# tavildar/Polar

Hardware: AMD Instinct MI355X
Metric: codewords/s (N=2048 K=1024 L=32 LLR-SCL) (higher is better)
Workload: dtype f64

## Files before the change

### include/polar_amd_debug.h

```cpp
#ifndef POLAR_AMD_DEBUG_H
#define POLAR_AMD_DEBUG_H
#include "polar_amd.h"
#ifdef __cplusplus
extern "C" {
#endif

int polar_debug_set(polar_code_t *h, const char *key, long value);
long polar_debug_get(const polar_code_t *h, const char *key);
long polar_debug_fallback_rows(polar_code_t *h, uint32_t *rows, long cap);
int polar_debug_comm_inits(void);
int polar_debug_weak_leaves(const polar_code_t *h);
void *polar_debug_scratch_ptr(polar_code_t *h);

#ifdef __cplusplus
}
#endif
#endif
```

### polar_amd/__init__.py

```python
import ctypes as C
import os

import numpy as np

try:
    import torch
except Exception:
    torch = None

_HERE = os.path.dirname(os.path.abspath(__file__))
LIB_PATH = os.environ.get("POLAR_AMD_LIB") or os.path.join(_HERE, "libpolar_amd.so")

_dp = C.POINTER(C.c_double)
_u8p = C.POINTER(C.c_uint8)
_u16p = C.POINTER(C.c_uint16)
_u64p = C.POINTER(C.c_uint64)


ASK4_GRAY, ASK8_GRAY, ASK16_GRAY, BPSK = 1, 2, 3, 4
ASK4_SP, ASK8_SP, ASK16_SP = 5, 6, 7
CONSTELLATION_NAMES = {"bpsk": BPSK, "ask4-gray": ASK4_GRAY, "ask8-gray": ASK8_GRAY, "ask16-gray": ASK16_GRAY,
                       "ask4-sp": ASK4_SP, "ask8-sp": ASK8_SP, "ask16-sp": ASK16_SP}
_NBITS = {BPSK: 1, ASK4_GRAY: 2, ASK4_SP: 2, ASK8_GRAY: 3, ASK8_SP: 3, ASK16_GRAY: 4, ASK16_SP: 4}
RX_MLC = 0x100
RECEIVERS = ("bicm", "mlc")


LLR_F64, LLR_F32, LLR_F16, LLR_BF16 = 0, 1, 2, 3
LLR_FORMATS = {"f64": LLR_F64, "f32": LLR_F32, "f16": LLR_F16, "bf16": LLR_BF16}
LS_RUN, LS_ERR, LS_MISS, LS_UNDET, LS_ML, LS_N = 0, 1, 2, 3, 4, 5
AD_RUN, AD_ERR, AD_UNDET, AD_STAGE0 = 0, 1, 2, 3
AD_MAX_STAGES = 8
FL_RUN, FL_ERR, FL_UNDET, FL_FIRST, FL_FLIPPED, FL_DECODES, FL_N = 0, 1, 2, 3, 4, 5, 6
FLIP_MAX = 64


def _llr_fmt_code(fmt):
    if isinstance(fmt, str):
        if fmt not in LLR_FORMATS:
            raise PolarError(f"unknown LLR format {fmt!r} (supported: {sorted(LLR_FORMATS)})")
        return LLR_FORMATS[fmt]
    return int(fmt)


def _llr_rows(llr, fmt):
    if fmt is not None:
        code = _llr_fmt_code(fmt)
        if code >= LLR_F16:
            ok = (np.uint16, np.float16) if code == LLR_F16 else (np.uint16,)
            if not (isinstance(llr, np.ndarray) and llr.dtype in ok):
                raise PolarError("fmt=%r takes the 16-bit patterns as a uint16 array%s" %
                                 (fmt, " (or the values as float16)" if code == LLR_F16 else ""))
            a = np.ascontiguousarray(llr)
        else:
            a = np.ascontiguousarray(llr, np.float32 if code == LLR_F32 else np.float64)
    elif isinstance(llr, np.ndarray) and llr.dtype == np.float32:
        code, a = LLR_F32, np.ascontiguousarray(llr)
    elif isinstance(llr, np.ndarray) and llr.dtype == np.float16:
        code, a = LLR_F16, np.ascontiguousarray(llr)
    else:
        code, a = LLR_F64, np.ascontiguousarray(llr, np.float64)
    return code, a


def _rx_flag(receiver):
    if receiver not in RECEIVERS:
        raise PolarError(f"unknown receiver {receiver!r} (supported: {RECEIVERS})")
    return RX_MLC if receiver == "mlc" else 0


def _constellation_id(c):
    if isinstance(c, str):
        if c not in CONSTELLATION_NAMES:
            raise PolarError(f"unsupported constellation {c!r} (supported: {sorted(CONSTELLATION_NAMES)})")
        return CONSTELLATION_NAMES[c]
    return int(c)


class PolarError(RuntimeError):
    pass


class PolarWeakLeavesWarning(UserWarning):
    """polar_create_explicit returned POLAR_W_WEAK_LEAVES (include/polar_amd.h)."""


POLAR_W_WEAK_LEAVES = 1


_lib = None


def lib():
    global _lib
    if _lib is None:
        if not os.path.exists(LIB_PATH):
            raise PolarError(
                f"{LIB_PATH} not found: build it with `python -m polar_amd.build` "
                "(the HIP extension is mandatory; there is no CPU fallback)")
        L = C.CDLL(LIB_PATH)
        L.polar_last_error.restype = C.c_char_p
        L.polar_snr_sqrt_linear.restype = C.c_double
        L.polar_snr_sqrt_linear.argtypes = [C.c_void_p, C.c_double]
        _lib = L
    return _lib


def use_library(path=None):
    global _lib, LIB_PATH
    LIB_PATH = path or os.environ.get("POLAR_AMD_LIB") or os.path.join(_HERE, "libpolar_amd.so")
    _lib = None
    return lib()


def _check(rc):
    if rc < 0:
        raise PolarError(f"polar_amd error {rc}: {lib().polar_last_error().decode()}")
    return rc


def _p(a, t):
    return a.ctypes.data_as(t)


def _stream_ptr(stream):
    if stream is None:
        if torch is not None and torch.cuda.is_available():
            return C.c_void_p(torch.cuda.current_stream().cuda_stream)
        return C.c_void_p(0)
    if hasattr(stream, "cuda_stream"):
        return C.c_void_p(stream.cuda_stream)
    return C.c_void_p(int(stream))


class Constellation:

    def __init__(self, name):
        self.id = _constellation_id(name)
        if self.id not in _NBITS:
            raise PolarError(f"unknown constellation {name!r} (supported: {sorted(CONSTELLATION_NAMES)})")
        self.name = name if isinstance(name, str) else {v: k for k, v in CONSTELLATION_NAMES.items()}[self.id]
        self.n_bits = _NBITS[self.id]
        self.n_sym = 1 << self.n_bits
        labels = ((np.arange(self.n_sym)[:, None] >> np.arange(self.n_bits)[None, :]) & 1).astype(np.uint8)
        self.points = self.modulate(labels.reshape(-1))

    def modulate(self, bits):
        a = np.ascontiguousarray(bits, np.uint8)
        if a.ndim not in (1, 2) or a.shape[-1] < 1:
            raise PolarError(f"modulate: bits must be [N] or [B][N], got shape {a.shape}")
        single = a.ndim == 1
        a2 = a.reshape(1, -1) if single else a
        out = np.zeros((a2.shape[0], a2.shape[1] // self.n_bits), np.float64)
        _check(lib().polar_modulate(C.c_int(self.id), _p(a2, _u8p), C.c_int(a2.shape[1]), C.c_long(a2.shape[0]), _p(out, _dp)))
        return out[0] if single else out

    def compute_llr_bicm(self, y, n0, block_length=None):
        f32 = isinstance(y, np.ndarray) and y.dtype == np.float32
        a = np.ascontiguousarray(y) if f32 else np.ascontiguousarray(y, np.float64)
        if a.ndim not in (1, 2):
            raise PolarError(f"compute_llr_bicm: y must be [M] or [B][M], got shape {a.shape}")
        single = a.ndim == 1
        a2 = a.reshape(1, -1) if single else a
        B, M = a2.shape
        N = M * self.n_bits if block_length is None else int(block_length)
        if N < 1 or N // self.n_bits != M:
            raise PolarError(f"compute_llr_bicm: rows of {M} symbols do not make rows of {N} positions at {self.n_bits} bits per symbol")
        p1, llr = np.zeros((B, N)), np.zeros((B, N))
        f = lib().polar_demap_bicm_f32 if f32 else lib().polar_demap_bicm
        _check(f(C.c_int(self.id), _p(a2, C.POINTER(C.c_float) if f32 else _dp), C.c_int(N), C.c_long(B), C.c_double(n0),
                 _p(llr, _dp), _p(p1, _dp)))
        return (p1[0], llr[0]) if single else (p1, llr)

    def compute_llr_bicm_dev(self, y_ptr, block_length, B, n0, llr_ptr=0, p1_ptr=0, stream=None, f32=False):
        f = lib().polar_demap_bicm_dev_f32 if f32 else lib().polar_demap_bicm_dev
        _check(f(C.c_int(self.id), C.c_void_p(y_ptr), C.c_int(block_length), C.c_long(B), C.c_double(n0),
                 C.c_void_p(llr_ptr), C.c_void_p(p1_ptr), _stream_ptr(stream)))


class PolarCode:

    def __init__(self, num_layers, info_length, epsilon, crc_size=0, _handle=None):
        L = self._L = lib()
        self._h = C.c_void_p()
        if _handle is not None:
            self._h = _handle
        else:
            self._chk(L.polar_create(C.c_int(num_layers), C.c_int(info_length), C.c_double(epsilon),
                                  C.c_int(crc_size), C.byref(self._h)))
        n, N, K, crc = C.c_int(), C.c_int(), C.c_int(), C.c_int()
        self._chk(L.polar_get_params(self._h, C.byref(n), C.byref(N), C.byref(K), C.byref(crc)))
        self.n, self.block_length, self.info_length, self.crc_size = n.value, N.value, K.value, crc.value
        self.N, self.K = self.block_length, self.info_length

    @property
    def weak_leaves(self):
        return int(self._L.polar_get_weak_leaves(self._h))

    def debug_set(self, key, value):
        self._chk(self._L.polar_debug_set(self._h, key.encode(), C.c_long(int(value))))

    def debug_get(self, key):
        f = self._L.polar_debug_get
        f.restype = C.c_long
        return int(f(self._h, key.encode()))

    def debug_fallback_rows(self):
        f = self._L.polar_debug_fallback_rows
        f.restype = C.c_long
        f.argtypes = [C.c_void_p, C.POINTER(C.c_uint32), C.c_long]
        n = int(f(self._h, None, 0))
        if n == -1:
            return None
        if n < 0:
            raise PolarError(f"polar_debug_fallback_rows: HIP status {-n - 1}")
        rows = np.zeros(max(n, 1), np.uint32)
        if int(f(self._h, _p(rows, C.POINTER(C.c_uint32)), n)) != n:
            raise PolarError("polar_debug_fallback_rows: the count changed between two reads")
        return np.sort(rows[:n])

    @classmethod
    def from_block_length(cls, block_length, info_length, design_epsilon, crc_size=0):
        n = int(round(np.log2(block_length)))
        if (1 << n) != block_length:
            raise PolarError("block_length must be a power of two")
        return cls(n, info_length, design_epsilon, crc_size)

    @classmethod
    def from_tables(cls, num_layers, info_length, crc_size, frozen, order, crc_matrix=None):
        frozen = np.ascontiguousarray(frozen, np.uint8)
        order = np.ascontiguousarray(order, np.uint16)
        N = 1 << num_layers
        if frozen.shape != (N,) or order.shape != (N,):
            raise PolarError("frozen/order must have N entries")
        cm = None
        if crc_size:
            cm = np.ascontiguousarray(crc_matrix, np.uint8)
            if cm.shape != (crc_size, info_length):
                raise PolarError("crc_matrix must be crc x K")
        h = C.c_void_p()
        status = _check(lib().polar_create_explicit(C.c_int(num_layers), C.c_int(info_length), C.c_int(crc_size),
                                                    _p(frozen, _u8p), _p(order, _u16p),
                                                    _p(cm, _u8p) if cm is not None else None, C.byref(h)))
        code = cls(num_layers, info_length, float("nan"), crc_size, _handle=h)
        if status == POLAR_W_WEAK_LEAVES:
            import warnings
            warnings.warn(f"polar_amd: {lib().polar_last_error().decode()}", PolarWeakLeavesWarning, stacklevel=2)
        return code

    @classmethod
    def from_construction_file(cls, path, info_length, crc_size=0, crc_matrix=None):
        return cls.from_counts(np.loadtxt(path).reshape(-1), info_length, crc_size, crc_matrix)

    @classmethod
    def from_counts(cls, counts, info_length, crc_size=0, crc_matrix=None):
        counts = np.asarray(counts).reshape(-1)
        N = counts.size
        n = int(round(np.log2(N)))
        if (1 << n) != N:
            raise PolarError("the count table must hold a power-of-two number of entries")
        order = np.argsort(counts, kind="stable").astype(np.uint16)
        frozen = np.ones(N, np.uint8)
        frozen[order[: info_length + crc_size]] = 0
        return cls.from_tables(n, info_length, crc_size, frozen, order, crc_matrix)

    @classmethod
    def from_monte_carlo(cls, block_length, info_length, design_snr_db, crc_size=0, num_runs=100000,
                         constellation_name="bpsk", receiver_algo="bicm", seed=1, crc_matrix=None, data_dir=None):
        _rx_flag(receiver_algo)
        path = None
        if data_dir is not None:
            path = os.path.join(data_dir, "MC_block_length_" + construction_unique_string(
                block_length, info_length + crc_size, design_snr_db, constellation_name, receiver_algo, num_runs) + ".txt")
        if path is not None and os.path.exists(path):
            counts = np.loadtxt(path).reshape(-1)
        else:
            n = int(round(np.log2(block_length)))
            if (1 << n) != block_length:
                raise PolarError("block_length must be a power of two")
            counts = mc_construction(n, design_snr_db, num_runs, constellation_name, seed=seed, receiver=receiver_algo)
            if path is not None:
                write_construction_file(path, counts)
        if crc_size and crc_matrix is None:
            crc_matrix = np.random.default_rng(seed).integers(0, 2, (crc_size, info_length)).astype(np.uint8)
        code = cls.from_counts(counts, info_length, crc_size, crc_matrix)
        code.construction_counts = np.asarray(counts)
        code.bler_estimate = float(np.sort(np.asarray(counts, np.float64), kind="stable")[: info_length + crc_size].sum() / num_runs)
        return code

    def monte_carlo_code_construction(self, design_snr_db, num_runs=100000, constellation_name="bpsk",
                                      receiver_algo="bicm", seed=1, data_dir=None):
        cm = self.crc_matrix if self.crc_size else None
        new = PolarCode.from_monte_carlo(self.block_length, self.info_length, design_snr_db, self.crc_size, num_runs,
                                         constellation_name, receiver_algo, seed, cm, data_dir)
        self.close()
        self._h, new._h = new._h, None
        self.construction_counts, self.bler_estimate = new.construction_counts, new.bler_estimate
        return self.bler_estimate

    @classmethod
    def from_gauss_approx(cls, block_length, info_length, design_snr_db, constellation_name="bpsk", receiver_algo="bicm",
                          crc_size=0, crc_matrix=None, phi_dx=1e-5, seed=1, capacity=None):
        n = int(round(np.log2(block_length)))
        if (1 << n) != block_length:
            raise PolarError("block_length must be a power of two")
        cap = None if capacity is None else np.asarray(capacity, np.float64).reshape(1, -1)
        ch, order, pre = ga_construction(n, [design_snr_db], constellation_name, receiver_algo, phi_dx, seed, cap)
        k = info_length + crc_size
        if not 0 < k <= block_length:
            raise PolarError("info_length + crc_size must lie in [1, block_length]")
        frozen = np.ones(block_length, np.uint8)
        frozen[order[0, :k]] = 0
        if crc_size and crc_matrix is None:
            crc_matrix = np.random.default_rng(seed).integers(0, 2, (crc_size, info_length)).astype(np.uint8)
        code = cls.from_tables(n, info_length, crc_size, frozen, order[0], crc_matrix)
        code.channels = ch[0]
        code.bler_estimate = float(pre[0, k - 1])
        return code

    def ga_code_construction(self, design_snr_db, constellation_name="bpsk", receiver_algo="bicm", phi_dx=1e-5, seed=1,
                             capacity=None):
        cm = self.crc_matrix if self.crc_size else None
        new = PolarCode.from_gauss_approx(self.block_length, self.info_length, design_snr_db, constellation_name,
                                          receiver_algo, self.crc_size, cm, phi_dx, seed, capacity)
        self.close()
        self._h, new._h = new._h, None
        self.channels, self.bler_estimate = new.channels, new.bler_estimate
        return self.bler_estimate

    def _chk(self, rc):
        if rc < 0:
            raise PolarError(f"polar_amd error {rc}: {self._L.polar_last_error().decode()}")
        return rc

    def close(self):
        if getattr(self, "_h", None):
            self._L.polar_destroy(self._h)
            self._h = None

    def __del__(self):
        try:
            self.close()
        except Exception:
            pass

    @property
    def frozen_bits(self):
        a = np.zeros(self.N, np.uint8)
        self._chk(self._L.polar_get_frozen(self._h, _p(a, _u8p)))
        return a

    @property
    def channel_order_descending(self):
        a = np.zeros(self.N, np.uint16)
        self._chk(self._L.polar_get_order(self._h, _p(a, _u16p)))
        return a

    @property
    def bit_rev_order(self):
        a = np.zeros(self.N, np.uint16)
        self._chk(self._L.polar_get_bitrev(self._h, _p(a, _u16p)))
        return a

    @property
    def crc_matrix(self):
        a = np.zeros((self.crc_size, self.K), np.uint8)
        if self.crc_size:
            self._chk(self._L.polar_get_crc_matrix(self._h, _p(a, _u8p)))
        return a

    @crc_matrix.setter
    def crc_matrix(self, m):
        m = np.ascontiguousarray(m, np.uint8)
        if m.shape != (self.crc_size, self.K):
            raise PolarError("crc_matrix must be crc x K")
        if self.crc_size:
            self._chk(self._L.polar_set_crc_matrix(self._h, _p(m, _u8p)))

    def reserve(self, B, list_size):
        self._chk(self._L.polar_reserve(self._h, C.c_long(B), C.c_int(list_size)))

    def set_tuning(self, waves_per_cu=0, lds_log=0):
        self._chk(self._L.polar_set_tuning(self._h, C.c_int(waves_per_cu), C.c_int(lds_log)))

    def set_mode(self, mode=0):
        self._chk(self._L.polar_set_mode(self._h, C.c_int(mode)))

    def snr_sqrt_linear(self, ebno_db):
        return self._L.polar_snr_sqrt_linear(self._h, C.c_double(ebno_db))

    def encode(self, info_bits):
        info = np.ascontiguousarray(info_bits, np.uint8)
        single = info.ndim == 1
        info2 = info.reshape(-1, self.K)
        out = np.zeros((info2.shape[0], self.N), np.uint8)
        self._chk(self._L.polar_encode_batch(self._h, _p(info2, _u8p), C.c_long(info2.shape[0]), _p(out, _u8p)))
        return out[0] if single else out

    def decode_scl_llr(self, llr, list_size, out=None, fmt=None):
        code, a = _llr_rows(llr, fmt)
        single = a.ndim == 1
        a2 = a.reshape(-1, self.N)
        if out is None:
            out = np.zeros((a2.shape[0], self.K), np.uint8)
        elif out.dtype != np.uint8 or out.shape != (a2.shape[0], self.K) or not out.flags.c_contiguous:
            raise PolarError("out must be a C-contiguous uint8 array of shape [B, K]")
        self._chk(self._L.polar_decode_scl_llr_batch_fmt(self._h, C.c_void_p(a2.ctypes.data), C.c_int(code), C.c_long(a2.shape[0]),
                                                    C.c_int(list_size), _p(out, _u8p)))
        return out[0] if single else out

    def decode_scl_llr_list(self, llr, list_size, fmt=None):
        code, a = _llr_rows(llr, fmt)
        a2 = a.reshape(-1, self.N)
        B, L = a2.shape[0], int(list_size)
        if not 1 <= L <= 64:
            raise PolarError("list size %d out of range [1, 64]" % L)
        cand = np.zeros((B, L, self.K), np.uint8)
        pm = np.zeros((B, L), np.float64)
        crc_ok = np.zeros((B, L), np.uint8)
        n_active = np.zeros(B, np.int32)
        winner = np.zeros(B, np.int32)
        self._chk(self._L.polar_decode_scl_llr_list_batch(
            self._h, C.c_void_p(a2.ctypes.data), C.c_int(code), C.c_long(B), C.c_int(L), C.c_void_p(cand.ctypes.data),
            C.c_void_p(pm.ctypes.data), C.c_void_p(crc_ok.ctypes.data), C.c_void_p(n_active.ctypes.data),
            C.c_void_p(winner.ctypes.data)))
        return cand, pm, crc_ok, n_active, winner

    def decode_scl_llr_list_dev(self, llr_ptr, fmt, B, list_size, cand_ptr, pm_ptr=0, crc_ok_ptr=0, n_active_ptr=0, winner_ptr=0,
                                stream=None):
        self._chk(self._L.polar_decode_scl_llr_list_batch_dev(
            self._h, C.c_void_p(llr_ptr), C.c_int(_llr_fmt_code(fmt)), C.c_long(B), C.c_int(list_size), C.c_void_p(cand_ptr),
            C.c_void_p(pm_ptr), C.c_void_p(crc_ok_ptr), C.c_void_p(n_active_ptr), C.c_void_p(winner_ptr), _stream_ptr(stream)))

    def list_find_dev(self, cand_ptr, n_active_ptr, info_ptr, B, list_size, rank_ptr, stream=None):
        self._chk(self._L.polar_list_find_dev(self._h, C.c_void_p(cand_ptr), C.c_void_p(n_active_ptr), C.c_void_p(info_ptr),
                                              C.c_long(B), C.c_int(list_size), C.c_void_p(rank_ptr), _stream_ptr(stream)))

    def path_metric(self, llr, info, fmt=None):
        code, a = _llr_rows(llr, fmt)
        a2 = a.reshape(-1, self.N)
        B = a2.shape[0]
        w = np.ascontiguousarray(info, np.uint8)
        if w.ndim == 1 and B == 1:
            w = w.reshape(1, -1)
        if w.ndim not in (2, 3) or w.shape[0] != B or w.shape[-1] != self.K:
            raise PolarError(f"path_metric: info must be [B, K] or [B, R, K] with B = {B}, K = {self.K}, got shape {w.shape}")
        R = 1 if w.ndim == 2 else w.shape[1]
        if not 1 <= R <= 64:
            raise PolarError("path_metric: %d words per row out of range [1, 64]" % R)
        pm = np.zeros((B,) if w.ndim == 2 else (B, R), np.float64)
        self._chk(self._L.polar_path_metric_batch(self._h, C.c_void_p(a2.ctypes.data), C.c_int(code), C.c_void_p(w.ctypes.data),
                                                  C.c_long(B), C.c_int(R), C.c_void_p(pm.ctypes.data)))
        return pm

    def path_metric_dev(self, llr_ptr, fmt, info_ptr, B, R, pm_ptr, stream=None):
        self._chk(self._L.polar_path_metric_batch_dev(self._h, C.c_void_p(llr_ptr), C.c_int(_llr_fmt_code(fmt)), C.c_void_p(info_ptr),
                                                      C.c_long(B), C.c_int(R), C.c_void_p(pm_ptr), _stream_ptr(stream)))

    def mc_batch_list(self, seed, t0, T, stride, axis, list_size_vec, enabled, stats, constellation=0):
        Ls = np.ascontiguousarray(list_size_vec, np.uint8)
        self._mc_batch_cells(self._L.polar_mc_batch_list, seed, t0, T, stride, axis, Ls, enabled, stats, constellation, LS_N, True)

    def _mc_batch_cells(self, fn, seed, t0, T, stride, axis, Ls, enabled, stats, constellation, cols, per_L):
        ax = np.ascontiguousarray(axis, np.float64)
        enabled = np.ascontiguousarray(enabled, np.uint8)
        cells, txt = (len(Ls) * len(ax), ("len(L)", "len(axis)")) if per_L else (len(ax), ("len(axis)",))
        if stats.dtype != np.uint64 or stats.size != cells * cols or not stats.flags.c_contiguous:
            raise PolarError("stats must be a C-contiguous uint64 array [%s, %d]" % (", ".join(txt), cols))
        if enabled.size != cells:
            raise PolarError("enabled must have %s entries" % " * ".join(txt))
        self._chk(fn(self._h, C.c_int(_constellation_id(constellation)), C.c_uint64(seed), C.c_uint64(t0), C.c_long(T), C.c_long(stride),
                     _p(ax, _dp), C.c_int(len(ax)), _p(Ls, _u8p), C.c_int(len(Ls)), _p(enabled, _u8p), _p(stats, _u64p)))

    @staticmethod
    def _stat_rounds(who, batch_fn, stats, err_col, run_col, max_runs, max_err, batch):
        if max_runs < 1 or batch < 0:
            raise PolarError(who + ": max_runs must be positive and batch non-negative")
        done, step = 0, int(batch) if batch else max(256, 2 * int(max_err))
        while done < max_runs:
            enabled = ((stats[..., err_col] <= max_err) & (stats[..., run_col] < max_runs)).astype(np.uint8)
            if not enabled.any():
                break
            T = min(step, max_runs - done)
            batch_fn(done, T, enabled)
            done += T
            if not batch:
                step = min(2 * step, 262144)

    def list_stats(self, axis, list_size_vec, max_runs=1000, max_err=100, seed=0, batch=0, constellation=0):
        ax = np.ascontiguousarray(axis, np.float64)
        Ls = np.ascontiguousarray(list_size_vec, np.uint8)
        stats = np.zeros((len(Ls), len(ax), LS_N), np.uint64)
        self._stat_rounds("list_stats", lambda t0, T, enabled: self.mc_batch_list(seed, t0, T, 1, ax, Ls, enabled, stats, constellation),
                          stats, LS_ERR, LS_RUN, max_runs, max_err, batch)
        run = np.maximum(stats[:, :, LS_RUN], 1).astype(np.float64)
        res = {"stats": stats}
        for name, col in (("bler", LS_ERR), ("miss_rate", LS_MISS), ("undetected_rate", LS_UNDET), ("ml_bound", LS_ML)):
            res[name] = stats[:, :, col] / run
        return res

    @staticmethod
    def _schedule(schedule):
        v = [int(x) for x in np.atleast_1d(np.asarray(schedule)).tolist()]
        if any(not 0 <= x <= 255 for x in v):
            raise PolarError("list size out of range [1, 64] in schedule %r" % (v,))
        return np.array(v, np.uint8)

    def decode_scl_llr_adaptive(self, llr, schedule=(1, 4, 32), fmt=None):
        code, a = _llr_rows(llr, fmt)
        a2 = a.reshape(-1, self.N)
        B, Ls = a2.shape[0], self._schedule(schedule)
        out = np.zeros((B, self.K), np.uint8)
        pm = np.zeros(B, np.float64)
        stage = np.zeros(B, np.uint8)
        crc_ok = np.zeros(B, np.uint8)
        self._chk(self._L.polar_decode_scl_llr_adaptive_batch(
            self._h, C.c_void_p(a2.ctypes.data), C.c_int(code), C.c_long(B), _p(Ls, _u8p), C.c_int(len(Ls)), _p(out, _u8p),
            C.c_void_p(pm.ctypes.data), C.c_void_p(stage.ctypes.data), C.c_void_p(crc_ok.ctypes.data)))
        return out, pm, stage, crc_ok

    def decode_scl_llr_adaptive_dev(self, llr_ptr, fmt, B, schedule, out_ptr, pm_ptr=0, stage_ptr=0, crc_ok_ptr=0, stream=None):
        Ls = self._schedule(schedule)
# ... 469 lines not shown
```

### polar_amd/build.py

```python
import os
import shutil
import subprocess
import sys

HERE = os.path.dirname(os.path.abspath(__file__))
ROOT = os.path.dirname(HERE)
CSRC = os.path.join(HERE, "csrc")
INC = os.path.join(ROOT, "include")
LIB = os.path.join(HERE, "libpolar_amd.so")
BUILD = os.path.join(HERE, "_build")
FLAGS_LIST32 = ["-mllvm", "-amdgpu-sched-strategy=max-memory-clause", "-mllvm", "-amdgpu-use-amdgpu-trackers"] + \
               os.environ.get("POLAR_LIST32_FLAGS", "").split()
FLAGS_LAT = os.environ.get("POLAR_LAT_FLAGS", "").split()
SOURCES = [("polar_kernels.hip", ["POLAR_ED_TU=0"], "", []), ("polar_kernels.hip", ["POLAR_ED_TU=1"], ".ed", []),
           ("polar_kernels.hip", ["POLAR_ED_TU=2"], ".ed32", FLAGS_LIST32), ("polar_kernels.hip", ["POLAR_ED_TU=3"], ".lat", FLAGS_LAT),
           ("polar_kernels.hip", ["POLAR_ED_TU=4"], ".list", []),
           ("polar_kernels.hip", ["POLAR_ED_TU=5"], ".headA", []), ("polar_kernels.hip", ["POLAR_ED_TU=6"], ".headB", FLAGS_LIST32),
           ("polar_kernels.hip", ["POLAR_ED_TU=7"], ".adapt", []),
           ("polar_kernels_sc.hip", [], "", []), ("polar_kernels_p1.hip", [], "", []), ("polar_channel.hip", [], "", []),
           ("polar_construct.hip", [], "", []), ("polar_kernels_mlc.hip", [], "", []), ("polar_kernels_ga.hip", [], "", []),
           ("polar_kernels_metric.hip", [], "", []), ("polar_kernels_adapt.hip", [], "", []),
           ("polar_kernels_flip.hip", [], "", [])] + \
          [(f, [], "", []) for f in ("polar_handle.cpp", "polar_decode.cpp", "polar_hostpipe.cpp", "polar_montecarlo.cpp", "polar_multi.cpp",
                                     "polar_debug.cpp", "polar_ga.cpp", "polar_bicm.cpp", "polar_list.cpp", "polar_mlc.cpp", "polar_adaptive.cpp", "polar_flip.cpp")]
TEST_HOOK_SOURCES = ("polar_montecarlo.cpp", "polar_debug.cpp")
LIB_TEST = os.path.join(HERE, "libpolar_amd_test.so")
KNOWN_DEFS = {"POLAR_MARGIN", "POLAR_SLOTHIST", "SCLAT_PROF", "POLAR_DEV_GS32", "POLAR_DEV_ONE", "POLAR_NO_FIXED_N",
              "POLAR_NO_GUARD_INT", "POLAR_NO_COLD_HINTS", "OCC", "ED_NR"}
ARCH = os.environ.get("POLAR_ARCH", "gfx950")
_flags_ok = {}


def _probe_flags(flags):
    key = tuple(flags)
    if key not in _flags_ok:
        import tempfile
        ok = list(flags)
        with tempfile.TemporaryDirectory() as d:
            src = os.path.join(d, "probe.hip")
            open(src, "w").write("#include <hip/hip_runtime.h>\n__global__ void probe_kernel() {}\n")
            pairs = [flags[i:i + 2] for i in range(0, len(flags), 2)]
            ok = []
            for pr in pairs:
                r = subprocess.run([_hipcc(), "--offload-arch=" + ARCH, "-c", src, "-o", os.path.join(d, "probe.o")] + pr,
                                   stdout=subprocess.DEVNULL, stderr=subprocess.PIPE, text=True)
                if r.returncode == 0 or "Unknown command line argument" not in r.stderr:
                    ok += pr
                else:
                    print("polar_amd.build: this compiler rejects %s (%s); building without it" %
                          (" ".join(pr), (r.stderr.strip().splitlines() or ["?"])[-1][:120]), file=sys.stderr)
        _flags_ok[key] = ok
    return _flags_ok[key]


def _hipcc():
    return shutil.which("hipcc") or "/opt/rocm/bin/hipcc"


def _torch_lib():
    try:
        import torch
        d = os.path.join(os.path.dirname(torch.__file__), "lib")
        if os.path.exists(os.path.join(d, "libamdhip64.so")):
            return d
    except Exception:
        pass
    return None


def _newer(target, deps):
    if not os.path.exists(target):
        return True
    t = os.path.getmtime(target)
    return any((not os.path.exists(d)) or os.path.getmtime(d) > t for d in deps)


def _fingerprint(cmd, files):
    import hashlib
    root = os.path.realpath(ROOT)

    def rel(x):
        rx = os.path.realpath(x) if os.path.isabs(x) else x
        return "<root>" + rx[len(root):] if os.path.isabs(rx) and rx.startswith(root) else x
    h = hashlib.sha256(" ".join(rel(c) for c in cmd[1:]).encode())
    for f in sorted(set(files), key=rel):
        try:
            h.update(rel(f).encode()); h.update(open(f, "rb").read())
        except OSError:
            h.update(b"<missing>")
    return h.hexdigest()


def _deps(obj, fallback):
    d = obj + ".d"
    if not os.path.exists(d):
        return fallback
    txt = open(d).read().replace("\\\n", " ")
    parts = txt.split(":", 1)
    if len(parts) < 2:
        return fallback
    out = []
    for x in parts[1].split():
        for anchor in ("/polar_amd/csrc/", "/include/"):
            k = x.rfind(anchor)
            if k >= 0 and not x.startswith("/opt/") and not x.startswith("/usr/"):
                cand = os.path.join(ROOT, x[k + 1:])
                if os.path.exists(cand):
                    out.append(cand)
                break
    return out


def build(force=False, verbose=False, profile=False, bless=False, test_hooks=False):
    global LIB
    os.makedirs(BUILD, exist_ok=True)
    lib_out = os.path.join(HERE, "libpolar_amd_prof.so") if profile else (LIB_TEST if test_hooks else LIB)
    tag = ".prof" if profile else ""
    if os.environ.get("POLAR_BUILD_TAG"):
        tag = "." + os.environ["POLAR_BUILD_TAG"]
        lib_out = os.path.join(HERE, "libpolar_amd_%s%s.so" % (os.environ["POLAR_BUILD_TAG"], "_test" if test_hooks else ""))
    extra_defs = os.environ.get("POLAR_DEFS", "").split()
    dev_build = profile or bool(extra_defs)
    if extra_defs:
        unknown = [d for d in extra_defs if d.split("=")[0] not in KNOWN_DEFS]
        if unknown:
            raise SystemExit("polar_amd.build: POLAR_DEFS names unknown macro(s) %s (known: %s)" % (unknown, sorted(KNOWN_DEFS)))
        if not os.environ.get("POLAR_BUILD_TAG"):
            raise SystemExit("polar_amd.build: POLAR_DEFS=%r without POLAR_BUILD_TAG: development builds never take the product "
                             "library's name (libpolar_amd.so)" % os.environ["POLAR_DEFS"])
    headers = [os.path.join(INC, f) for f in os.listdir(INC)] + \
              [os.path.join(CSRC, f) for f in os.listdir(CSRC) if f.endswith((".h", ".inc"))]
    objs = []
    jobs = []
    for s, defs, otag, xflags in SOURCES:
        src = os.path.join(CSRC, s)
        if test_hooks and s in TEST_HOOK_SOURCES:
            defs, otag = defs + ["POLAR_TEST_HOOKS"], otag + ".th"
        obj = os.path.join(BUILD, s + otag + tag + ".o")
        objs.append(obj)
        cmd = [_hipcc(), "--offload-arch=" + ARCH, "-O3", "-std=c++17", "-fPIC", "-ffp-contract=off",
               "-Wall", "-Wno-unused-function", "-x", "hip", "-I", INC, "-I", CSRC, "-MD", "-MF", obj + ".d",
               "-c", src, "-o", obj]
        if profile:
            cmd.insert(1, "-DPOLAR_PROFILE")
        for d in defs + extra_defs + (["POLAR_DEV_BUILD"] if dev_build else []):
            cmd.insert(1, "-D" + d)
        cmd[1:1] = (_probe_flags(xflags) if xflags else []) + os.environ.get("POLAR_HIPCC_FLAGS", "").split()
        fp = _fingerprint(cmd, [src] + _deps(obj, headers))
        stamp = obj + ".sha"
        have = open(stamp).read().strip() if os.path.exists(stamp) and os.path.exists(obj) else None
        if bless and os.path.exists(obj):
            if have != fp:
                print("polar_amd.build --bless: WARNING: stamping %s as current WITHOUT compiling it; use only on a tree "
                      "whose objects you know to be built from these sources" % os.path.basename(obj), file=sys.stderr)
            open(stamp, "w").write(fp)
            continue
        if force or have != fp:
            if verbose:
                print(" ".join(cmd))
            jobs.append((cmd, stamp, obj, src, headers))
    if jobs:
        from concurrent.futures import ThreadPoolExecutor

        def run(job):
            cmd, stamp, obj, src, hdrs = job
            subprocess.check_call(cmd)
            open(stamp, "w").write(_fingerprint(cmd, [src] + _deps(obj, hdrs)))
        with ThreadPoolExecutor(max_workers=min(len(jobs), os.cpu_count() or 1)) as ex:
            list(ex.map(run, jobs))
    import hashlib
    link_fp = hashlib.sha256("".join(open(o + ".sha").read() if os.path.exists(o + ".sha") else "?" for o in objs).encode()).hexdigest()
    link_stamp = os.path.join(BUILD, os.path.basename(lib_out) + ".sha")
    have_link = open(link_stamp).read().strip() if os.path.exists(link_stamp) and os.path.exists(lib_out) else None
    if bless and os.path.exists(lib_out):
        open(link_stamp, "w").write(link_fp)
        have_link = link_fp
    if force or jobs or have_link != link_fp:
        tl = _torch_lib()
        vs = os.path.join(BUILD, "exports.map")
        open(vs, "w").write("{ global: polar_*; local: *; };\n")
        cmd = [_hipcc(), "-shared", "-fPIC", "-Wl,--version-script=" + vs, "-o", lib_out] + objs
        if tl:
            clang = "/opt/rocm/lib/llvm/bin/clang++"
            cmd = [clang, "-shared", "-fPIC", "-Wl,--version-script=" + vs, "-o", lib_out] + objs + \
                  ["-L" + tl, "-lamdhip64", "-Wl,-rpath," + tl, "-Wl,-rpath,/opt/rocm/lib", "-lstdc++", "-lm"]
        if verbose:
            print(" ".join(cmd))
        subprocess.check_call(cmd)
        open(link_stamp, "w").write(link_fp)
    return lib_out


def build_test(force=False):
    return build(force=force, test_hooks=True)


def build_cli(force=False):
    lib = build()
    exe = os.path.join(BUILD, "polar_main")
    src = os.path.join(HERE, "cpp", "main.cpp")
    hdr = os.path.join(HERE, "cpp", "PolarCode.hpp")
    if force or _newer(exe, [src, hdr, lib]):
        subprocess.check_call(["g++", "-std=c++17", "-O2", "-I", INC, "-I", os.path.join(HERE, "cpp"), src, "-o", exe,
                               "-L", HERE, "-lpolar_amd", "-Wl,-rpath," + HERE,
                               "-Wl,-rpath," + (_torch_lib() or "/opt/rocm/lib"), "-Wl,-rpath,/opt/rocm/lib"])
    return exe


if __name__ == "__main__":
    if "--bless" in sys.argv and not os.environ.get("POLAR_DEV"):
        raise SystemExit("polar_amd.build: --bless stamps existing objects as current without compiling them; it is a "
                         "development aid and needs POLAR_DEV=1 in the environment")
    print(build(force="--force" in sys.argv, verbose=True, profile="--profile" in sys.argv, bless="--bless" in sys.argv))
```

### polar_amd/csrc/polar_debug.cpp

```cpp
#include "polar_multi.h"
#include "polar_amd_debug.h"
#ifdef POLAR_TEST_HOOKS
#include "polar_head_plan.h"
#endif

extern "C" {

int polar_debug_weak_leaves(const polar_code_t *h) { return polar_get_weak_leaves(h); }

int polar_debug_set(polar_code_t *h, const char *key, long value) {
    if (!h || !key) return fail(POLAR_E_ARG, "NULL argument");
    polar_code::Knobs &k = h->knobs;
    const std::string s(key);
    if (s == "mode_override") { if (value < -1 || value > 2) return fail(POLAR_E_ARG, "mode_override must be -1 (none), 0, 1 or 2"); k.mode_override = (int)value; }
    else if (s == "sc_no_fold") k.sc_no_fold = value != 0;
    else if (s == "no_tables") k.no_tables = value != 0;
    else if (s == "no_head") k.no_head = value != 0;
    else if (s == "head_min_b") { if (value < 0) return fail(POLAR_E_ARG, "head_min_b must be >= 0 (0 = default)"); k.head_min_b = value; }
    else if (s == "no_fuse_front") k.no_fuse_front = value != 0;
    else if (s == "no_prefix") h->prefix_on = (value == 0);
    else if (s == "no_rccl") { k.no_rccl = value != 0; multi_release(h, false); }
    else if (s == "force_rccl") { k.force_rccl = value != 0; multi_release(h, false); }
#ifdef POLAR_TEST_HOOKS
    else if (s == "host_fail_alloc") k.host_fail_alloc = value;
    else if (s == "share_device") { k.share_device = value != 0; multi_release(h, false); }
    else if (s == "fail_device") k.fail_device = (int)value;
    else if (s == "fail_collective") k.fail_collective = (int)value;
#endif
    else if (s == "lat_max_b") k.lat_max_b = value;
    else if (s == "lat_grid") { if (value < 0) return fail(POLAR_E_ARG, "lat_grid must be >= 0 (0 = default)"); k.lat_grid = value; }
    else if (s == "lane_grid") { if (value < 0) return fail(POLAR_E_ARG, "lane_grid must be >= 0 (0 = default)"); k.lane_grid = value; }
    else if (s == "list_chunk_cw") { if (value < 0) return fail(POLAR_E_ARG, "list_chunk_cw must be >= 0"); k.list_chunk_cw = value; }
    else if (s == "host_pipe_min_bytes") k.host_pipe_min_bytes = value;
    else if (s == "host_chunk_bytes") k.host_chunk_bytes = value;
    else if (s == "host_lanes") { if (value < 0 || value > HostPipe::kMaxLanes) return fail(POLAR_E_ARG, "host_lanes must be 0 (default) or 1 .. %d", HostPipe::kMaxLanes); k.host_lanes = value; }
    else if (s == "host_ramp") k.host_ramp = value;
    else if (s == "host_prefault") { if (value < -1 || value > 16) return fail(POLAR_E_ARG, "host_prefault must be -1 (none), 0 (default) or 1 .. 16 threads"); k.host_prefault = value; }
    else if (s == "host_threads") { if (value < 0) return fail(POLAR_E_ARG, "host_threads must be >= 0"); k.host_threads = value; }
    else if (s == "multi_grace_s") { if (value < 0) return fail(POLAR_E_ARG, "multi_grace_s must be >= 0"); k.multi_grace_s = value; }
#ifdef POLAR_TEST_HOOKS
    else if (s == "force_workers") { k.force_workers = value != 0; multi_release(h, false); }
    else if (s == "stall_device") k.stall_device = (int)value;
    else if (s == "stall_ms") { if (value < 0) return fail(POLAR_E_ARG, "stall_ms must be >= 0"); k.stall_ms = value; }
#endif
    else if (s == "multi_timeout_s") { if (value < 0) return fail(POLAR_E_ARG, "multi_timeout_s must be >= 0 (0 = no watchdog)"); k.multi_timeout_s = value; }
    else return fail(POLAR_E_ARG, "polar_debug_set: unknown key '%s'", key);
    drop_clones(h);
    return POLAR_OK;
}
void *polar_debug_scratch_ptr(polar_code_t *h) { return h ? (void *)h->d_llr_scr.p : nullptr; }
long polar_debug_get(const polar_code_t *h, const char *key) {
    if (!key) return -1;
    const std::string s(key);
    if (s == "allocs") return (long)g_allocs.load();
    if (s == "comm_inits") return (long)polar_debug_comm_inits();
    if (!h) return -1;
    if (s == "test_hooks") {
#ifdef POLAR_TEST_HOOKS
        return 1;
#else
        return 0;
#endif
    }
    if (s == "weak_leaves") return h->weak_leaves;
    if (s == "mode_override") return h->knobs.mode_override;
    if (s == "head_phi") return h->last_head_phi;
    if (s == "lat_waves") return h->last_lat_waves;
    if (s == "lane_waves") return h->last_lane_waves;
#ifdef POLAR_TEST_HOOKS
    if (s == "head_check") {
        if (!h->last_head_phi || h->last_head_b <= 0 || !h->d_head_rec.p) return -2;
        int P = 0;
        while (P < h->N && h->frozen[P]) ++P;
        const int Q = P >= 256 ? 256 : (P < 33 ? 0 : (P < 64 ? 64 : (P < 128 ? 128 : 256)));
        const HeadPlan hp = head_plan(h->frozen.data(), h->n, Q, std::min(P, Q), h->N / 2);
        if (hp.phi_h != h->last_head_phi) return -3;
        std::vector<unsigned long long> rows2((size_t)h->last_head_b * 4);
        const size_t pitch = hp.record_words() * sizeof(unsigned long long);
        if (hipMemcpy2D(rows2.data(), 32, h->d_head_rec.p + 2 * 4, pitch, 32, (size_t)h->last_head_b, hipMemcpyDeviceToHost) != hipSuccess) return -4;
        long bad = 0;
        for (long b = 0; b < h->last_head_b; ++b) {
            unsigned long long r[4];
            for (int a = 0; a < 4; ++a) r[a] = rows2[(size_t)b * 4 + a];
            bad += head_record_ok(hp, r) ? 0 : 1;
        }
        return bad;
    }
#endif
    if (s == "last_rounds") return h->last_rounds;
    if (s == "last_round_max_per_device") return h->last_round_max_per_device;
    if (s == "worker_threads_started") return h->worker_threads_started;
    if (s.compare(0, 9, "round_us_") == 0) {
        if (h->round_us.empty()) return 0;
        std::vector<long> v(h->round_us);
        if (s == "round_us_count") return (long)v.size();
        if (s == "round_us_first") return v.front();
        std::sort(v.begin(), v.end());
        if (s == "round_us_min") return v.front();
        if (s == "round_us_max") return v.back();
        if (s == "round_us_median") return v[v.size() / 2];
        return -1;
    }
    if (s == "multi_poisoned") return h->multi_poisoned ? 1 : 0;
    if (s == "host_chunks") return h->hpipe ? h->hpipe->last_chunks : 0;
    if (s == "host_chunk_cw") return h->hpipe ? h->hpipe->last_chunk_cw : 0;
    if (s == "host_lanes") return h->hpipe ? h->hpipe->last_lanes : 0;
    if (s == "host_threads") return h->hpipe ? h->hpipe->last_threads : 0;
    if (s == "host_us_copy_in") return h->hpipe ? h->hpipe->us_copy_in : 0;
    if (s == "host_us_wait") return h->hpipe ? h->hpipe->us_wait : 0;
    if (s == "host_us_copy_out") return h->hpipe ? h->hpipe->us_copy_out : 0;
    if (s == "host_us_total") return h->hpipe ? h->hpipe->us_total : 0;
    return -1;
}
int polar_debug_comm_inits(void) { return g_comm_inits.load(); }

long polar_debug_fallback_rows(polar_code_t *h, uint32_t *rows, long cap) {
    if (!h || !h->fb_count) return -1;
    DevGuard dg_;
    if (ensure_device(h, dg_)) return -1;
    hipError_t e = hipStreamSynchronize((hipStream_t)h->fb_stream);
    unsigned int count = 0;
    if (e == hipSuccess) e = hipMemcpy(&count, h->fb_count, sizeof count, hipMemcpyDeviceToHost);
    if (e == hipSuccess && (long)count > h->fb_b) return -(long)hipErrorInvalidValue - 1;
    const long n = std::min<long>(count, cap);
    if (e == hipSuccess && rows && n > 0) e = hipMemcpy(rows, h->fb_list, (size_t)n * sizeof(uint32_t), hipMemcpyDeviceToHost);
    return e == hipSuccess ? (long)count : -(long)e - 1;
}

}
```

### polar_amd/csrc/polar_decode.cpp

```cpp
#include "polar_host.h"
#include "polar_head_plan.h"

namespace {

int effective_mode(const polar_code *h) { return h->knobs.mode_override >= 0 ? h->knobs.mode_override : h->mode; }
long lat_resident(const polar_code *h, int gs) {
    const size_t lds = polar_decode_lat_lds_bytes(h->N, gs, h->W);
    return lds <= h->lds_per_block ? (long)h->num_cu * std::min<long>(4, (long)(h->lds_per_block / lds)) : 0;
}
bool use_sc_lat(const polar_code *h, long B) {
    return h->n <= polar_sc_lat_max_log() && polar_sc_lat_lds_bytes(h->N, (int)h->sc_lat_ops.size()) <= h->lds_per_block &&
           h->knobs.lat_max_b >= 0 && B <= (h->knobs.lat_max_b ? h->knobs.lat_max_b : 2048);
}

struct Call {
    polar_code *h;
    const void *d_llr; int llr_fmt; long B; const unsigned int *n_dev; int L; uint8_t *d_out; double *d_pm;
    hipStream_t st; void *ev_start, *ev_stop; int phase; Deferred *deferred;
    BatchGeometry g; PolarDecodeParams p;
};

int batch_setup(polar_code *h, long B, int L, BatchGeometry &g) {
    if (!batch_geometry(h, B, L, true, g)) return fail(POLAR_E_ARG, "lds_log %d does not fit the LDS", g.lds_log);
    if ((size_t)g.grid * g.big * 64 + 64 > h->d_llr_scr.cap) {
        const size_t per_wave = g.big * 64 * sizeof(double) + 1;
        const long cap = (long)(scratch_budget(h) / per_wave);
        if (g.grid > cap) g.grid = (int)std::max<long>(g.wpb, (cap / g.wpb) * g.wpb);
    }
    return ensure_batch_scratch(h, g);
}

int fallback_pass(const PolarDecodeParams &p, const BatchGeometry &g, const uint32_t *list, const unsigned int *count, unsigned int *work, int max_grid, hipStream_t st) {
    PolarDecodeParams pf = p;
    pf.prefix_q = 0; pf.prefix_len = 0; pf.pre = nullptr;
    if (work) pf.work = work;
    else HIP_TRY(hipMemsetAsync(pf.work, 0, sizeof(unsigned int), st));
    pf.cw_list = list; pf.cw_count = count; pf.n_dev = nullptr;
    HIP_TRY(polar_launch_decode_llr(pf, g.gs, g.lds_log, g.pipe, std::min(g.grid, max_grid), false, st));
    return POLAR_OK;
}

int decode_sc8(Call &c, bool lat) {
    polar_code *h = c.h; const BatchGeometry &g = c.g;
    const long B = c.B;
    int rc;
    const int sgrid = (int)std::min<long>((B + 7) / 8, (long)h->num_cu * polar_sc8_waves_per_cu(h->N));
    const bool in_place = lat || (h->sc_fold && !h->knobs.sc_no_fold && ((uintptr_t)c.d_llr & 15u) == 0);
    if (!in_place && (rc = h->d_ech.ensure((size_t)B * h->N))) return rc;
    if ((rc = h->d_list.ensure((size_t)B))) return rc;
    const size_t nfw = (size_t)(B + 31) / 32 + 1;
    if ((rc = h->d_flag_words.ensure(4 + nfw))) return rc;
    unsigned int *ctrl = h->d_flag_words.p, *fwords = h->d_flag_words.p + 4;
    if ((rc = h->d_llr_scr.ensure(std::max((size_t)sgrid * polar_sc8_scratch_doubles_per_wave(h->N) + 64, (size_t)g.grid * g.big * 64 + 64)))) return rc;
    c.p.llr_scr = h->d_llr_scr.p;
    if (c.phase != 2) {
        HIP_TRY(hipMemsetAsync(ctrl, 0, (4 + nfw) * sizeof(unsigned int), c.st));
        if (!in_place) HIP_TRY(polar_launch_sc8_front(c.d_llr, c.llr_fmt, h->d_ech.p, fwords, h->d_tabs.p, h->n, B, c.n_dev, c.st));
        PolarScParams sp;
        sp.n = h->n; sp.N = h->N; sp.K = h->K; sp.B = B;
        sp.llr = in_place ? c.d_llr : nullptr; sp.llr_fmt = c.llr_fmt;
        sp.ech_t = in_place ? nullptr : h->d_ech.p; sp.out = c.d_out;
        sp.ops = lat ? h->d_sc_lat_ops.p : h->d_sc_ops.p; sp.n_ops = (int)(lat ? h->sc_lat_ops.size() : h->sc_ops.size());
        sp.order = h->d_order.p; sp.tabs = h->d_tabs.p; sp.a_scr = h->d_llr_scr.p;
        sp.flag_words = fwords; sp.work = ctrl; sp.n_dev = c.n_dev;
        sp.flag_bytes = lat ? h->lat_flag_bytes : nullptr;
        if (c.ev_start) HIP_TRY(hipEventRecord((hipEvent_t)c.ev_start, c.st));
        HIP_TRY(lat ? polar_launch_sc_lat(sp, lat_grid(h, std::min<long>(B, (long)h->num_cu * 4)), c.st) : polar_launch_sc8_decode(sp, sgrid, c.st));
        if (c.ev_stop) HIP_TRY(hipEventRecord((hipEvent_t)c.ev_stop, c.st));
        if (c.phase == 1 && lat && c.deferred) { *c.deferred = Deferred::FlagWords; return POLAR_OK; }
    }
    HIP_TRY(polar_launch_sc_collect(fwords, B, c.n_dev, h->d_list.p, ctrl + 1, c.st));
    h->note_fallback(ctrl + 1, h->d_list.p, c.st, B);
    return fallback_pass(c.p, g, h->d_list.p, ctrl + 1, ctrl + 2, 16 * g.wpb, c.st);
}

int decode_list_lat(const Call &c) {
    polar_code *h = c.h;
    const int gs = pow2ceil(c.L);
    const bool ed = effective_mode(h) != 1 && !(gs == 2 && c.d_pm);
    const long resident = lat_resident(h, gs);
    int rc;
    if (ed) {
        const size_t cap = (size_t)std::max<long>(c.B, 2 * resident);
        if ((rc = h->d_flags.ensure(cap))) return rc;
        if ((rc = h->d_list.ensure(cap))) return rc;
        if ((rc = h->d_count.ensure(1))) return rc;
    }
    const PolarDecodeParams &p = c.p;
    if (c.phase != 2) {
        PolarDecodeParams pl = p;
        if (ed) pl.flags = h->d_flags.p;
        HIP_TRY(hipMemsetAsync(p.work, 0, sizeof(unsigned int), c.st));
        if (c.ev_start) HIP_TRY(hipEventRecord((hipEvent_t)c.ev_start, c.st));
        HIP_TRY(polar_launch_decode_lat(pl, gs, ed, lat_grid(h, std::min<long>(c.B, resident)), c.st));
        if (c.ev_stop) HIP_TRY(hipEventRecord((hipEvent_t)c.ev_stop, c.st));
        if (ed && c.phase == 1 && c.deferred) { *c.deferred = Deferred::FlagBytes; return POLAR_OK; }
    }
    if (!ed) return POLAR_OK;
    HIP_TRY(hipMemsetAsync(h->d_count.p, 0, sizeof(unsigned int), c.st));
    HIP_TRY(polar_launch_ed_collect(h->d_flags.p, c.B, c.n_dev, h->d_list.p, h->d_count.p, c.st));
    h->note_fallback(h->d_count.p, h->d_list.p, c.st, c.B);
    return fallback_pass(p, c.g, h->d_list.p, h->d_count.p, nullptr, 64 * c.g.wpb, c.st);
}

int decode_batch_llr(Call &c) {
    polar_code *h = c.h; const BatchGeometry &g = c.g;
    PolarDecodeParams &p = c.p;
    if (int rc = prefix_params(h, g.gs, p)) return rc;
    HIP_TRY(hipMemsetAsync(p.work, 0, sizeof(unsigned int), c.st));
    if (p.prefix_q) HIP_TRY(polar_launch_prefix(p, false, nullptr, c.st));
    if (c.ev_start) HIP_TRY(hipEventRecord((hipEvent_t)c.ev_start, c.st));
    HIP_TRY(polar_launch_decode_llr(p, g.gs, g.lds_log, g.pipe, g.grid, false, c.st));
    if (c.ev_stop) HIP_TRY(hipEventRecord((hipEvent_t)c.ev_stop, c.st));
    return POLAR_OK;
}

int decode_batch_ed(Call &c) {
    polar_code *h = c.h; const BatchGeometry &g = c.g;
    PolarDecodeParams &p = c.p;
    const long B = c.B;
    int rc;
    if ((rc = prefix_params(h, g.gs, p))) return rc;
    HIP_TRY(hipMemsetAsync(p.work, 0, 2 * sizeof(unsigned int), c.st));
    if ((rc = h->d_ech.ensure((size_t)B * h->N))) return rc;
    if ((rc = h->d_flags.ensure((size_t)B))) return rc;
    if ((rc = h->d_list.ensure((size_t)B))) return rc;
    if ((rc = h->d_count.ensure(1))) return rc;
    HIP_TRY(hipMemsetAsync(h->d_count.p, 0, sizeof(unsigned int), c.st));
    const bool fuse_front = p.prefix_q > 0 && polar_prefix_is_staged(h->N) && !h->knobs.no_fuse_front;
    if (!fuse_front) HIP_TRY(polar_launch_ed_front(c.d_llr, c.llr_fmt, h->d_ech.p, h->d_flags.p, h->d_tabs.p, h->N, B, c.n_dev, c.st));
    PolarDecodeParams pe = p;
    pe.llr = h->d_ech.p; pe.llr_fmt = POLAR_LLR_F64; pe.flags = h->d_flags.p;
    if (g.gs == 32 && !g.pipe && h->N >= 1024 && p.prefix_q > 0 && !h->knobs.no_tables) {
        if ((rc = h->d_tab_scr.ensure((size_t)g.grid * g.G * 3 * h->N + 64))) return rc;
        if ((rc = h->d_var_scr.ensure((size_t)g.grid * (h->N / 32) * 64 + 64))) return rc;
        pe.tab_scr = h->d_tab_scr.p; pe.var_scr = h->d_var_scr.p;
    }
    if (pe.prefix_q && fuse_front) {
        PolarDecodeParams pp = pe;
        pp.llr = (const double *)c.d_llr; pp.llr_fmt = c.llr_fmt;
        HIP_TRY(polar_launch_prefix(pp, true, h->d_ech.p, c.st));
    } else if (pe.prefix_q) HIP_TRY(polar_launch_prefix(pe, true, nullptr, c.st));
    HeadPlan hp;
    if (g.gs == 32 && p.prefix_q > 0) hp = head_plan(h->frozen.data(), h->n, p.prefix_q, p.prefix_len, h->N / 2);
    const long head_min_b = h->knobs.head_min_b ? h->knobs.head_min_b : (long)h->num_cu * 16 * 16;
    const bool two_phase = head_use(hp, g.lds_log == 3 && !g.pipe, B, head_min_b, h->knobs.no_head);
    h->last_head_phi = two_phase ? hp.phi_h : 0;
    h->last_head_b = two_phase && !c.n_dev ? B : 0;
    PolarHeadParams ph;
    if (two_phase) {
        if ((rc = h->d_head_rec.ensure((size_t)B * hp.record_words()))) return rc;
        static_cast<PolarDecodeParams &>(ph) = pe;
        ph.head_rec = h->d_head_rec.p; ph.head_phi = hp.phi_h; ph.head_t = hp.t; ph.head_rows = hp.rows();
        ph.head_llr_mask = hp.llr_mask; ph.head_c_mask = hp.c_mask;
    }
    if (c.ev_start) HIP_TRY(hipEventRecord((hipEvent_t)c.ev_start, c.st));
    if (two_phase) {
        PolarHeadParams pa = ph;
        pa.L = HeadPlan::kPaths; pa.work = p.work + 1; pa.tab_scr = nullptr; pa.var_scr = nullptr; pa.out = nullptr; pa.pm_out = nullptr;
        const long waves_a = (B + 15) / 16;
        const int grid_a = (int)std::min<long>(g.grid, ((waves_a + g.wpb - 1) / g.wpb) * g.wpb);
        HIP_TRY(polar_launch_decode_head_export(pa, grid_a, c.st));
        HIP_TRY(polar_launch_decode_head_import(ph, g.grid, c.st));
    } else
    HIP_TRY(polar_launch_decode_llr(pe, g.gs, g.lds_log, g.pipe, g.grid, true, c.st));
    if (c.ev_stop) HIP_TRY(hipEventRecord((hipEvent_t)c.ev_stop, c.st));
    HIP_TRY(polar_launch_ed_collect(h->d_flags.p, B, c.n_dev, h->d_list.p, h->d_count.p, c.st));
    h->note_fallback(h->d_count.p, h->d_list.p, c.st, B);
    return fallback_pass(p, g, h->d_list.p, h->d_count.p, nullptr, h->weak_leaves ? g.grid : 64 * g.wpb, c.st);
}

}

Family polar_host::choose_family(const polar_code *h, long B, int L, bool want_pm) {
    const int mode = effective_mode(h), gs = pow2ceil(L);
    if (L == 1 && mode != 1 && !want_pm) return use_sc_lat(h, B) ? Family::ScLat : Family::Sc8;
    const bool ed = gs >= 4 && mode != 1;
    const long resident = lat_resident(h, gs);
    if ((gs == 2 || (ed && (gs == 4 || gs == 8))) && h->knobs.lat_max_b >= 0 && resident > 0 &&
        B <= (h->knobs.lat_max_b ? h->knobs.lat_max_b : 2 * resident)) return Family::ListLat;
    return ed ? Family::BatchEd : Family::BatchLlr;
}

int polar_host::prefix_params(polar_code *h, int gs, PolarDecodeParams &p) {
    int P = 0;
    while (P < h->N && h->frozen[P]) ++P;
    int Q = 0;
    if (gs >= 4 && h->prefix_on) {
        if (P >= 256) Q = 256;
        else { Q = 64; while (Q <= P) Q <<= 1; if (P < 33) Q = 0; }
        if (Q > h->N / 2) Q = 0;
    }
    p.prefix_q = Q; p.prefix_len = Q ? std::min(P, Q) : 0;
    if (!Q) return POLAR_OK;
    if (int rc = h->d_pre.ensure((size_t)p.B * (size_t)(h->N - Q + 1))) return rc;
    p.pre = h->d_pre.p;
    return POLAR_OK;
}

bool polar_host::batch_geometry(const polar_code *h, long B, int L, bool tuned, BatchGeometry &g) {
    g.gs = pow2ceil(L); g.G = 64 / g.gs;
    const long groups = (B + g.G - 1) / g.G;
    g.wpc = tuned && h->waves_per_cu ? h->waves_per_cu : 16;
    int lds_log = tuned ? h->lds_log : 3;
    if (tuned && !h->waves_per_cu && !h->lds_log && g.gs >= 16 && groups <= (long)h->num_cu * 4 &&
        polar_decode_lds_bytes(5, 1) <= h->lds_per_block) { g.wpc = 4; lds_log = 5; }
    g.pipe = (g.wpc > 8) ? 0 : 1;
    g.lds_log = lds_log ? lds_log : (g.pipe ? 4 : 3);
    g.wpb = polar_decode_waves_per_block(g.pipe);
    const int max_blocks_by_lds = (int)(h->lds_per_block / polar_decode_lds_bytes(g.lds_log, g.pipe));
    if (max_blocks_by_lds < 1) return false;
    if (g.wpc > max_blocks_by_lds * g.wpb) g.wpc = max_blocks_by_lds * g.wpb;
    g.grid = (int)std::min(groups, (long)h->num_cu * g.wpc);
    g.grid = ((g.grid + g.wpb - 1) / g.wpb) * g.wpb;
    g.big = polar_decode_big(h->N, g.lds_log);
    g.cwords = polar_decode_cwords(h->N);
    return true;
}

int polar_host::ensure_batch_scratch(polar_code *h, const BatchGeometry &g) {
    int rc;
    if ((rc = h->d_llr_scr.ensure((size_t)g.grid * g.big * 64 + 64))) return rc;
    if ((rc = h->d_c_scr.ensure((size_t)g.grid * 2 * g.cwords * 64 + 64))) return rc;
    return h->d_hist_scr.ensure((size_t)g.grid * 3 * h->W * 64 + 64);
}

int polar_host::default_scratch(polar_code *h, BatchGeometry *g, int n) {
    BatchGeometry gm = *std::max_element(g, g + n, [](const BatchGeometry &a, const BatchGeometry &b) { return a.grid < b.grid; });
    int rc;
    while ((rc = ensure_batch_scratch(h, gm)) == POLAR_E_NOMEM && gm.grid > gm.wpb) {
        (void)hipGetLastError();
        gm.grid = std::max(gm.wpb, (gm.grid / 2 / gm.wpb) * gm.wpb);
    }
    for (int s = 0; s < n && !rc; ++s) g[s].grid = std::min(g[s].grid, gm.grid);
    return rc;
}

void polar_host::base_params(const polar_code *h, int L, long B, PolarDecodeParams &p) {
    p.n = h->n; p.N = h->N; p.K = h->K; p.crc = h->crc; p.L = L; p.W = h->W; p.B = B;
    p.prefix_q = 0; p.prefix_len = 0; p.pre = nullptr;
    p.llr = nullptr; p.llr_fmt = POLAR_LLR_F64; p.p0 = nullptr; p.out = nullptr; p.pm_out = nullptr;
    p.frozen = h->d_frozen.p; p.info_rank = h->d_info_rank.p; p.crc_mask = h->d_crc_mask.p; p.tabs = h->d_tabs.p;
    p.ctl = h->d_ctl.p; p.work = h->d_work.p; p.llr_scr = h->d_llr_scr.p; p.c_scr = h->d_c_scr.p; p.hist_scr = h->d_hist_scr.p;
    p.flags = nullptr; p.cw_list = nullptr; p.cw_count = nullptr; p.n_dev = nullptr; p.tab_scr = nullptr; p.var_scr = nullptr;
}

void polar_host::fill_enc(const polar_code *h, PolarEncodeParams &p) {
    memset(&p, 0, sizeof p);
    p.n = h->n; p.N = h->N; p.K = h->K; p.crc = h->crc;
    p.order = h->d_order.p; p.crcm = h->d_crcm.p;
    p.stride = 1;
    p.info_block_div = 100;
}

int polar_host::decode_impl(polar_code *h, const void *d_llr, int llr_fmt, long B, const unsigned int *n_dev, int L, uint8_t *d_out,
                            double *d_pm, void *stream, void *ev_start, void *ev_stop, int phase, Deferred *deferred) {
    if (deferred) *deferred = Deferred::None;
    int rc = check_args(h && d_llr && d_out, L, B);
    if (rc || B == 0) return rc;
    DevGuard dg_;
    if ((rc = ensure_device(h, dg_))) return rc;
    if ((rc = h->d_work.ensure(2))) return rc;
    h->last_head_phi = 0; h->last_head_b = 0;
    if (phase != 2) h->last_lane_waves = 0;
    if (phase != 2) h->last_lat_waves = 0;
    if (phase != 2) h->note_fallback(nullptr, nullptr, nullptr, 0);
    const Family fam = choose_family(h, B, L, d_pm != nullptr);
    Call c{h, d_llr, llr_fmt, B, n_dev, L, d_out, d_pm, (hipStream_t)stream, ev_start, ev_stop, phase, deferred, {}, {}};
    if (!(fam == Family::ListLat && effective_mode(h) == 1) && (rc = batch_setup(h, B, L, c.g))) return rc;
    base_params(h, L, B, c.p);
    c.p.llr = (const double *)d_llr; c.p.llr_fmt = llr_fmt; c.p.out = d_out; c.p.pm_out = d_pm; c.p.n_dev = n_dev;
    switch (fam) {
        case Family::Sc8: case Family::ScLat: return decode_sc8(c, fam == Family::ScLat);
        case Family::ListLat: return decode_list_lat(c);
        case Family::BatchLlr: return decode_batch_llr(c);
        case Family::BatchEd: break;
    }
    return decode_batch_ed(c);
}

extern "C" {

int polar_decode_scl_llr_batch_dev(polar_code_t *h, const double *d_llr, long B, int L, uint8_t *d_out,
                                   double *d_pm, void *stream) {
    return polar_decode_scl_llr_batch_dev_fmt(h, d_llr, POLAR_LLR_F64, B, L, d_out, d_pm, stream);
}

int polar_decode_scl_llr_batch_dev_ev(polar_code_t *h, const double *d_llr, long B, int L, uint8_t *d_out,
                                      double *d_pm, void *stream, void *ev_start, void *ev_stop) {
    return decode_impl(h, d_llr, 0, B, nullptr, L, d_out, d_pm, stream, ev_start, ev_stop);
}

int polar_decode_scl_llr_batch_dev_f32(polar_code_t *h, const float *d_llr, long B, int L, uint8_t *d_out,
                                       double *d_pm, void *stream) {
    return polar_decode_scl_llr_batch_dev_fmt(h, d_llr, POLAR_LLR_F32, B, L, d_out, d_pm, stream);
}
int polar_decode_scl_llr_batch_dev_fmt(polar_code_t *h, const void *d_llr, int fmt, long B, int L, uint8_t *d_out,
                                       double *d_pm, void *stream) {
    int rc = llr_fmt_check(fmt, d_llr);
    if (rc) return rc;
    return decode_impl(h, d_llr, fmt, B, nullptr, L, d_out, d_pm, stream, nullptr, nullptr);
}

int polar_decode_scl_p1_batch(polar_code_t *h, const double *p1, const double *p0, long B, int L, uint8_t *out) {
    int rc = check_args(h && p1 && p0 && out, L, B);
    if (rc || B == 0) return rc;
    DevGuard dg_;
    if ((rc = ensure_device(h, dg_))) return rc;
    const int N = h->N;
    const int gs = pow2ceil(L), G = 64 / gs;
    long groups = (B + G - 1) / G;
    if ((rc = h->d_in.ensure((size_t)B * N * 2))) return rc;
    if ((rc = h->d_out.ensure((size_t)B * h->K))) return rc;
    int grid = 1;
    h->last_lat_waves = 0; h->last_lane_waves = 0;
    rc = grid_that_fits(h, lane_grid(h, std::min<long>(groups, (long)h->num_cu * 16)), (size_t)N * 64 * 2 * sizeof(double), [&](int g) {
        int r = h->d_llr_scr.ensure((size_t)g * N * 64 * 2 + 64);
        if (!r) r = h->d_c_scr.ensure((size_t)g * 2 * polar_decode_cwords(N) * 64 + 64);
        if (!r) r = h->d_hist_scr.ensure((size_t)g * h->W * 64 + 64);
        return r;
    }, &grid);
    if (rc) return rc;
    HIP_TRY(hipMemcpy(h->d_in.p, p1, (size_t)B * N * sizeof(double), hipMemcpyHostToDevice));
    HIP_TRY(hipMemcpy(h->d_in.p + (size_t)B * N, p0, (size_t)B * N * sizeof(double), hipMemcpyHostToDevice));
    PolarDecodeParams p;
    base_params(h, L, B, p);
    p.ctl = nullptr; p.work = nullptr;
    p.llr = h->d_in.p; p.p0 = h->d_in.p + (size_t)B * N; p.out = h->d_out.p;
    HIP_TRY(polar_launch_decode_p1(p, gs, grid, nullptr));
    h->last_lane_waves = grid;
    HIP_TRY(hipDeviceSynchronize());
    HIP_TRY(hipMemcpy(out, h->d_out.p, (size_t)B * h->K, hipMemcpyDeviceToHost));
    return POLAR_OK;
}
int polar_decode_scl_p1(polar_code_t *h, const double *p1, const double *p0, int L, uint8_t *out) {
    return polar_decode_scl_p1_batch(h, p1, p0, 1, L, out);
}

int polar_decode_sc_p1_batch(polar_code_t *h, const double *p1, long B, double *out) {
    int rc = check_args(h && p1 && out, kNoList, B);
    if (rc || B == 0) return rc;
    DevGuard dg_;
    if ((rc = ensure_device(h, dg_))) return rc;
    const int N = h->N;
    h->last_lat_waves = 0; h->last_lane_waves = 0;
    if ((rc = h->d_in.ensure((size_t)B * N + (size_t)B * h->K))) return rc;
    PolarScP1Params p;
    p.n = h->n; p.N = N; p.K = h->K; p.B = B;
    p.p1 = h->d_in.p; p.out = h->d_in.p + (size_t)B * N;
    p.frozen = h->d_frozen.p; p.order = h->d_order.p; p.scr = nullptr;
    HIP_TRY(hipMemcpy(h->d_in.p, p1, (size_t)B * N * sizeof(double), hipMemcpyHostToDevice));
    const long lat_waves = polar_sc_p1_lat_lds_bytes(N) <= h->lds_per_block ? (long)h->num_cu * std::max<long>(1, (long)(h->lds_per_block / polar_sc_p1_lat_lds_bytes(N))) : 0;
    const long lat_max = h->knobs.lat_max_b < 0 ? 0 : (h->knobs.lat_max_b ? h->knobs.lat_max_b : lat_waves * 4);
    if (lat_waves > 0 && B <= lat_max) {
        HIP_TRY(polar_launch_sc_p1_lat(p, lat_grid(h, std::min<long>(B, lat_waves)), nullptr));
    } else {
        int grid = 1;
        rc = grid_that_fits(h, lane_grid(h, std::min<long>((B + 63) / 64, (long)h->num_cu * 16)), (size_t)N * 64 * 4 * sizeof(double),
                            [&](int g) { return h->d_llr_scr.ensure((size_t)g * 4 * N * 64 + 64); }, &grid);
        if (rc) return rc;
        p.scr = h->d_llr_scr.p;
        HIP_TRY(polar_launch_sc_p1(p, grid, nullptr));
        h->last_lane_waves = grid;
    }
    HIP_TRY(hipDeviceSynchronize());
    HIP_TRY(hipMemcpy(out, p.out, (size_t)B * h->K * sizeof(double), hipMemcpyDeviceToHost));
    return POLAR_OK;
}
int polar_decode_sc_p1(polar_code_t *h, const double *p1, double *out) { return polar_decode_sc_p1_batch(h, p1, 1, out); }

int polar_encode_batch_dev(polar_code_t *h, const uint8_t *d_info, long B, uint8_t *d_coded, void *stream) {
    int rc = check_args(h && d_info && d_coded, kNoList, B);
    if (rc || B == 0) return rc;
    DevGuard dg_;
    if ((rc = ensure_device(h, dg_))) return rc;
    PolarEncodeParams p;
    fill_enc(h, p);
    p.B = B; p.info = d_info; p.coded = d_coded;
    HIP_TRY(polar_launch_encode(p, (hipStream_t)stream));
    return POLAR_OK;
}

int polar_encode_batch(polar_code_t *h, const uint8_t *info, long B, uint8_t *coded) {
    int rc = check_args(h && info && coded, kNoList, B);
    if (rc || B == 0) return rc;
    DevGuard dg_;
    if ((rc = ensure_device(h, dg_))) return rc;
    if ((rc = h->d_bytes_a.ensure((size_t)B * h->K))) return rc;
    if ((rc = h->d_bytes_b.ensure((size_t)B * h->N))) return rc;
    HIP_TRY(hipMemcpy(h->d_bytes_a.p, info, (size_t)B * h->K, hipMemcpyHostToDevice));
    if ((rc = polar_encode_batch_dev(h, h->d_bytes_a.p, B, h->d_bytes_b.p, nullptr))) return rc;
    HIP_TRY(hipDeviceSynchronize());
    HIP_TRY(hipMemcpy(coded, h->d_bytes_b.p, (size_t)B * h->N, hipMemcpyDeviceToHost));
    return POLAR_OK;
}
int polar_encode(polar_code_t *h, const uint8_t *info, uint8_t *coded) { return polar_encode_batch(h, info, 1, coded); }

int polar_synth_llr_dev(polar_code_t *h, uint64_t seed, uint64_t trial0, long B, double s,
                        double *d_llr, uint8_t *d_info, void *stream) {
    int rc = check_args(h && d_llr, kNoList, B);
    if (rc || B == 0) return rc;
    DevGuard dg_;
    if ((rc = ensure_device(h, dg_))) return rc;
    PolarEncodeParams p;
    fill_enc(h, p);
    p.B = B; p.seed = seed; p.trial0 = trial0; p.s = s; p.llr = d_llr; p.info_out = d_info;
    HIP_TRY(polar_launch_synth(p, (hipStream_t)stream));
    return POLAR_OK;
}

int polar_reserve(polar_code_t *h, long B, int L) {
    if (!h) return fail(POLAR_E_ARG, "NULL handle");
    int rc = check_args(true, L, B);
    if (rc || B == 0) return rc;
    DevGuard dg_;
    if ((rc = ensure_device(h, dg_))) return rc;
    DevBuf<double> llr, pm;
    DevBuf<uint8_t> out;
    if ((rc = llr.ensure((size_t)B * h->N + 1)) || (rc = out.ensure((size_t)B * h->K)) || (rc = pm.ensure((size_t)B))) { llr.release(); out.release(); pm.release(); return rc; }
    rc = polar_synth_llr_dev(h, 1, 0, B, polar_snr_sqrt_linear(h, 2.0), llr.p, nullptr, nullptr);
    const int top = std::min(pow2ceil(L), POLAR_MAX_LIST);
    for (int l = 1; l <= top && !rc; l <<= 1) {
        rc = polar_decode_scl_llr_batch_dev(h, llr.p, B, l, out.p, nullptr, nullptr);
        if (!rc && l <= 8) rc = polar_decode_scl_llr_batch_dev(h, llr.p, 1, l, out.p, nullptr, nullptr);
        if (!rc && l == 1) rc = polar_decode_scl_llr_batch_dev(h, llr.p, B, l, out.p, pm.p, nullptr);
        if (!rc && l == 1) rc = polar_decode_scl_llr_batch_dev(h, llr.p + 1, B, l, out.p, nullptr, nullptr);
    }
    if (!rc && top >= 32) {
        PolarDecodeParams pp;
        base_params(h, 32, B, pp);
        if (!(rc = prefix_params(h, 32, pp)) && pp.prefix_q > 0) {
            const HeadPlan hp = head_plan(h->frozen.data(), h->n, pp.prefix_q, pp.prefix_len, h->N / 2);
            if (hp.phi_h > 0 && hp.window >= kHeadMinWindow) rc = h->d_head_rec.ensure((size_t)B * hp.record_words());
        }
    }
    hipError_t e = hipDeviceSynchronize();
    llr.release(); out.release(); pm.release();
    if (!rc && e != hipSuccess) return fail(POLAR_E_DEVICE, "polar_reserve: %s", hipGetErrorString(e));
    return rc;
}

int polar_count_errors_dev(polar_code_t *h, const uint8_t *d_a, const uint8_t *d_b, long B,
                           unsigned long long *d_err_count, void *stream) {
    int rc = check_args(h && d_a && d_b && d_err_count, kNoList, B);
    if (rc || B == 0) return rc;
    DevGuard dg_;
    if ((rc = ensure_device(h, dg_))) return rc;
    HIP_TRY(polar_launch_count_errors(d_a, d_b, B, h->K, d_err_count, nullptr, (hipStream_t)stream));
    return POLAR_OK;
}

}
```

### polar_amd/csrc/polar_handle.cpp

```cpp
#include "polar_host.h"

namespace polar_host {

thread_local std::string g_err;

int fail(int code, const char *fmt, ...) {
    char buf[512];
    va_list ap;
    va_start(ap, fmt);
    vsnprintf(buf, sizeof buf, fmt, ap);
    va_end(ap);
    g_err = buf;
    return code;
}

std::atomic<unsigned long> g_allocs{0};

int usable_cpus() {
    int n = (int)std::thread::hardware_concurrency();
    cpu_set_t set;
    if (sched_getaffinity(0, sizeof set, &set) == 0) n = CPU_COUNT(&set);
    if (FILE *f = fopen("/sys/fs/cgroup/cpu.max", "r")) {
        char q[32]; long per = 0;
        if (fscanf(f, "%31s %ld", q, &per) == 2 && strcmp(q, "max") != 0 && per > 0) n = std::min<long>(n, std::max<long>(1, atol(q) / per));
        fclose(f);
    }
    return std::max(1, n);
}

void make_bitrev(polar_code *h) {
    h->bitrev.resize(h->N);
    for (int i = 0; i < h->N; ++i) {
        unsigned r = 0;
        for (int b = 0; b < h->n; ++b) r |= ((unsigned(i) >> b) & 1u) << (h->n - 1 - b);
        h->bitrev[i] = (uint16_t)r;
    }
}

int derive_tables(polar_code *h) {
    const int N = h->N, K = h->K, crc = h->crc, E = K + crc;
    std::vector<int> rank(N, -1);
    int t = 0;
    for (int i = 0; i < N; ++i) if (!h->frozen[i]) rank[i] = t++;
    if (t != E) return fail(POLAR_E_ARG, "frozen mask has %d unfrozen positions, expected K+crc = %d", t, E);
    std::vector<uint8_t> seen(N, 0);
    h->info_rank.assign(E, 0);
    for (int b = 0; b < E; ++b) {
        int pos = h->order[b];
        if (pos >= N || rank[pos] < 0 || seen[pos])
            return fail(POLAR_E_ARG, "order[%d] = %d is frozen, duplicate or out of range", b, pos);
        seen[pos] = 1;
        h->info_rank[b] = (uint16_t)rank[pos];
    }
    h->W = (E + 31) / 32;
    if (h->W == 0) h->W = 1;
    h->sched.assign(N, 0);
    if (h->n >= 4) {
        for (int phi = 0; phi < N;) {
            auto allf = [&](int z) { if (phi % z || phi + z > N) return false; for (int i = 0; i < z; ++i) if (!h->frozen[phi + i]) return false; return true; };
            if (allf(8)) { h->sched[phi] = 3; phi += 8; }
            else if (allf(4)) { h->sched[phi] = 2; phi += 4; }
            else ++phi;
        }
    }
    h->sc_ops.clear();
    {
        auto emit = [&](int type, int S, int base) {
            int sh = 0; while ((1 << sh) < S) ++sh;
            h->sc_ops.push_back((uint32_t)type | ((uint32_t)sh << 3) | ((uint32_t)base << 8));
        };
        struct Rec {
            polar_code *h; decltype(emit) &em; int N;
            void go(int lo, int S) {
                bool allf = true, nonef = true;
                for (int i = lo; i < lo + S; ++i) { if (h->frozen[i]) nonef = false; else allf = false; }
                if (allf) { if (S < N) em(6, S, lo); }
                else if (nonef) em(3, S, lo);
                else {
                    const int hS = S / 2;
                    em(0, hS, lo); go(lo, hS);
                    em(1, hS, lo); go(lo + hS, hS);
                    em(4, hS, lo);
                }
            }
        } rec{h, emit, N};
        rec.go(0, N);
        h->sc_lat_ops.clear();
        {
            auto emit2 = [&](int type, int S, int base, uint32_t hi) {
                int sh = 0; while ((1 << sh) < S) ++sh;
                h->sc_lat_ops.push_back((uint32_t)type | ((uint32_t)sh << 3) | ((uint32_t)base << 8) | (hi << 24));
            };
            struct Rec2 {
                polar_code *h; decltype(emit2) &em; int N;
                void go(int lo, int S) {
                    bool allf = true, nonef = true;
                    for (int i = lo; i < lo + S; ++i) { if (h->frozen[i]) nonef = false; else allf = false; }
                    if (allf) { if (S < N) em(6, S, lo, 0u); }
                    else if (nonef) em(3, S, lo, 0u);
                    else if (S == 8) {
                        uint32_t pat = 0;
                        for (int i = 0; i < 8; ++i) pat |= (uint32_t)(h->frozen[lo + i] ? 1u : 0u) << i;
                        em(7, S, lo, pat);
                    } else {
                        const int hS = S / 2;
                        em(0, hS, lo, 0u); go(lo, hS);
                        em(1, hS, lo, 0u); go(lo + hS, hS);
                        uint32_t &last = h->sc_lat_ops.back();
                        if ((last & 7u) == 7u) last += 1u << 3;
                        else last += 1u << 24;
                    }
                }
            } rec2{h, emit2, N};
            rec2.go(0, N);
            for (uint32_t &w : h->sc_lat_ops) if ((w & 7u) == 7u) w -= 3u << 3;
        }
        std::vector<uint32_t> fused;
        for (size_t i = 0; i < h->sc_ops.size(); ++i) {
            uint32_t op = h->sc_ops[i];
            const int type = (int)(op & 7u), sh = (int)((op >> 3) & 15u);
            if (type <= 1 && N <= 65536) {
                int extra = 0;
                while (extra < 2 && i + 1 < h->sc_ops.size()) {
                    const uint32_t nx = h->sc_ops[i + 1];
                    if ((nx & 7u) != 0u || (int)((nx >> 3) & 15u) != sh - 1 - extra || sh - 1 - extra < polar_sc8_min_global_log() - 1 || sh - extra < polar_sc8_min_global_log()) break;
                    ++extra; ++i;
                }
                op |= (uint32_t)extra << 24;
            }
            fused.push_back(op);
        }
        h->sc_ops.swap(fused);
        h->sc_fold = h->n >= polar_sc8_fold_min_log();
        for (uint32_t op : h->sc_ops) {
            const int type = (int)(op & 7u), sh = (int)((op >> 3) & 15u), extra = (int)((op >> 24) & 3u);
            if (sh == h->n) h->sc_fold = false;
            if (type <= 1 && sh == h->n - 1 && extra != 2) h->sc_fold = false;
        }
    }
    h->ctl.resize(N);
    for (int i = 0; i < N; ++i) h->ctl[i] = (uint32_t)(h->frozen[i] ? 1u : 0u) | ((uint32_t)h->sched[i] << 1);
    h->weak_leaves = 0;
    {
        std::vector<double> z(1, 0.5), om(1, 0.5), z2, om2;
        for (int l = 0; l < h->n; ++l) {
            z2.resize(2 * z.size()); om2.resize(2 * z.size());
            for (size_t i = 0; i < z.size(); ++i) {
                z2[2 * i] = 2 * z[i] - z[i] * z[i]; om2[2 * i] = om[i] * om[i];
                z2[2 * i + 1] = z[i] * z[i];        om2[2 * i + 1] = om[i] * (1.0 + z[i]);
            }
            z.swap(z2); om.swap(om2);
        }
        for (int i = 0; i < N; ++i)
            if (!h->frozen[i] && om[i] < 1e-3) { h->ctl[i] |= 0x100u; ++h->weak_leaves; }
    }
    h->crc_mask.assign((size_t)crc * h->W, 0u);
    for (int i = 0; i < crc; ++i) {
        uint32_t *m = &h->crc_mask[(size_t)i * h->W];
        for (int j = 0; j < K; ++j)
            if (h->crcm[(size_t)i * K + j] & 1) m[h->info_rank[j] >> 5] ^= 1u << (h->info_rank[j] & 31);
        int r = h->info_rank[K + i];
        m[r >> 5] ^= 1u << (r & 31);
    }
    return POLAR_OK;
}

int ensure_device(polar_code *h, DevGuard &dg) {
    if (h->ctx_stuck) return fail(POLAR_E_DEVICE, "an earlier multi-device round of this handle never returned: the handle accepts no further calls (create a new one)");
    int cur = -1;
    if (hipGetDevice(&cur) == hipSuccess && h->device >= 0 && cur != h->device) dg.prev = cur;
    if (h->dev_ready) {
        HIP_TRY(hipSetDevice(h->device));
        return POLAR_OK;
    }
    int cnt = 0;
    hipError_t e = hipGetDeviceCount(&cnt);
    if (e != hipSuccess || cnt <= 0)
        return fail(POLAR_E_DEVICE, "no HIP device available (%s); this library has no CPU decode path",
                    e == hipSuccess ? "device count 0" : hipGetErrorString(e));
    if (h->device < 0) HIP_TRY(hipGetDevice(&h->device));
    HIP_TRY(hipSetDevice(h->device));
    hipDeviceProp_t prop;
    HIP_TRY(hipGetDeviceProperties(&prop, h->device));
    h->num_cu = prop.multiProcessorCount;
    {
        int v = 0;
        h->lds_per_block = (hipDeviceGetAttribute(&v, hipDeviceAttributeMaxSharedMemoryPerBlock, h->device) == hipSuccess && v > 0) ? (size_t)v : (size_t)64 * 1024;
    }
    int rc;
    if ((rc = upload(h->d_frozen, h->frozen))) return rc;
    if ((rc = upload(h->d_ctl, h->ctl))) return rc;
    if ((rc = upload(h->d_sc_ops, h->sc_ops))) return rc;
    if ((rc = upload(h->d_sc_lat_ops, h->sc_lat_ops))) return rc;
    if ((rc = upload(h->d_order, h->order))) return rc;
    if ((rc = upload(h->d_info_rank, h->info_rank))) return rc;
    if ((rc = upload(h->d_crc_mask, h->crc_mask))) return rc;
    if ((rc = upload(h->d_crcm, h->crcm))) return rc;
    {
        std::vector<double> t(322);
        for (int j = 0; j < 64; ++j) t[j] = j ? 2.0 * std::exp2(-(double)(64 - j) / 64.0) : 1.0;
        for (int j = 0; j <= 128; ++j) {
            t[64 + j] = 1.0 / (1.0 + (double)j / 128.0);
            t[64 + 129 + j] = std::log1p((double)j / 128.0);
        }
        if ((rc = upload(h->d_tabs, t))) return rc;
    }
    h->dev_ready = true;
    return POLAR_OK;
}

int read_env_knobs(polar_code *h) {
    auto on = [](const char *name) { const char *e = getenv(name); return e && *e && strcmp(e, "0") != 0; };
    if (const char *e = getenv("POLAR_MODE")) {
        if (!(e[0] >= '0' && e[0] <= '2' && e[1] == 0)) return fail(POLAR_E_ARG, "POLAR_MODE=%s: must be 0, 1 or 2", e);
        h->knobs.mode_override = e[0] - '0';
    }
    h->knobs.sc_no_fold = on("POLAR_SC_NO_FOLD");
    h->knobs.no_tables = on("POLAR_NO_TABLES");
    h->knobs.no_head = on("POLAR_NO_HEAD");
    h->knobs.no_rccl = on("POLAR_NO_RCCL");
    h->knobs.force_rccl = on("POLAR_FORCE_RCCL");
    return POLAR_OK;
}

void drop_clones(polar_code *h) {
    if (h->multi_poisoned) return;
    for (polar_code *c : h->clones) polar_destroy(c);
    h->clones.clear();
    if (h->hpipe) for (polar_code *&c : h->hpipe->ctx) if (c) { polar_destroy(c); c = nullptr; }
}

}

extern "C" {

const char *polar_last_error(void) { return g_err.c_str(); }
int polar_version(void) { return 200; }

int polar_create(int n, int K, double eps, int crc, polar_code_t **out) {
    if (!out) return fail(POLAR_E_ARG, "out is NULL");
    if (n < 1 || n > POLAR_MAX_N_LOG2) return fail(POLAR_E_ARG, "n = %d out of range [1, %d]", n, POLAR_MAX_N_LOG2);
    const int N = 1 << n;
    if (K < 1 || crc < 0 || crc > POLAR_MAX_CRC || K + crc > N)
        return fail(POLAR_E_ARG, "need 1 <= K, 0 <= crc <= %d, K + crc <= N (K=%d crc=%d N=%d)", POLAR_MAX_CRC, K, crc, N);
    polar_code *h = new polar_code;
    h->n = n; h->N = N; h->K = K; h->crc = crc; h->eps = eps;
    make_bitrev(h);
    std::vector<double> z(N, eps);
    for (int it = 0; it < n; ++it) {
        const int inc = 1 << it;
        for (int j = 0; j < inc; ++j)
            for (int i = 0; i < N; i += 2 * inc) {
                double c1 = z[i + j], c2 = z[i + j + inc];
                z[i + j] = c1 + c2 - c1 * c2;
                z[i + j + inc] = c1 * c2;
            }
    }
    h->order.resize(N);
    std::iota(h->order.begin(), h->order.end(), (uint16_t)0);
    const std::vector<uint16_t> &br = h->bitrev;
    std::sort(h->order.begin(), h->order.end(), [&](int i1, int i2) { return z[br[i1]] < z[br[i2]]; });
    h->frozen.assign(N, 1);
    for (int i = 0; i < K + crc; ++i) h->frozen[h->order[i]] = 0;
    h->crcm.resize((size_t)crc * K);
    for (int b = 0; b < crc; ++b)
        for (int j = 0; j < K; ++j) h->crcm[(size_t)b * K + j] = (uint8_t)(rand() % 2);
    int rc = derive_tables(h);
    if (!rc) rc = read_env_knobs(h);
    if (rc) { delete h; return rc; }
    (void)hipGetDevice(&h->device);
    *out = h;
    return POLAR_OK;
}

int polar_create_explicit(int n, int K, int crc, const uint8_t *frozen, const uint16_t *order,
                          const uint8_t *crc_matrix, polar_code_t **out) {
    if (!out || !frozen || !order) return fail(POLAR_E_ARG, "NULL argument");
    if (n < 1 || n > POLAR_MAX_N_LOG2) return fail(POLAR_E_ARG, "n = %d out of range", n);
    const int N = 1 << n;
    if (K < 1 || crc < 0 || crc > POLAR_MAX_CRC || K + crc > N) return fail(POLAR_E_ARG, "bad K/crc");
    if (crc > 0 && !crc_matrix) return fail(POLAR_E_ARG, "crc_matrix is NULL with crc = %d", crc);
    polar_code *h = new polar_code;
    h->n = n; h->N = N; h->K = K; h->crc = crc; h->eps = NAN;
    make_bitrev(h);
    h->frozen.assign(frozen, frozen + N);
    h->order.assign(order, order + N);
    h->crcm.assign((size_t)crc * K, 0);
    if (crc) memcpy(h->crcm.data(), crc_matrix, (size_t)crc * K);
    int rc = derive_tables(h);
    if (!rc) rc = read_env_knobs(h);
    if (rc) { delete h; return rc; }
    (void)hipGetDevice(&h->device);
    *out = h;
    if (h->weak_leaves) { g_err = "explicit table leaves " + std::to_string(h->weak_leaves) + " unfrozen leaves in channels of BEC(1/2) capacity below 1e-3"; return POLAR_W_WEAK_LEAVES; }
    return POLAR_OK;
}

void polar_destroy(polar_code_t *h) {
    if (!h) return;
    if (h->multi_poisoned) return;
    multi_release(h, false);
    for (polar_code *c : h->clones) polar_destroy(c);
    h->clones.clear();
    hostpipe_release(h);
    DevGuard dg_;
    {
        int cur = -1;
        if (h->dev_ready && hipGetDevice(&cur) == hipSuccess && cur != h->device) dg_.prev = cur;
    }
    if (h->dev_ready) (void)hipSetDevice(h->device);
    h->d_frozen.release(); h->d_ctl.release(); h->d_crcm.release(); h->d_order.release(); h->d_info_rank.release();
    h->d_crc_mask.release(); h->d_tabs.release(); h->d_pre.release(); h->d_llr_scr.release(); h->d_c_scr.release(); h->d_hist_scr.release();
    h->d_in.release(); h->d_f32.release(); h->d_out.release(); h->d_bytes_a.release(); h->d_bytes_b.release();
    h->d_counter.release(); h->d_sel.release(); h->d_work.release();
    h->d_ech.release(); h->d_flags.release(); h->d_list.release(); h->d_count.release(); h->d_bicm_llr.release(); h->d_list_out.release(); h->d_metric_scr.release(); h->d_adapt_ctl.release();
    h->d_alive[0].release(); h->d_alive[1].release(); h->d_nalive.release(); h->d_mc_ctr.release();
    for (auto &sl : h->mc_slots) { sl.list[0].release(); sl.list[1].release(); }
    h->d_slot_n.release();
    if (h->pin_in) (void)hipHostFree(h->pin_in);
    if (h->pin_out) (void)hipHostFree(h->pin_out);
    h->d_flip_ops.release(); h->d_flip_i32.release(); h->d_sc_ops.release(); h->d_sc_lat_ops.release(); h->d_flag_words.release(); h->d_var_scr.release(); h->d_tab_scr.release(); h->d_head_rec.release();
    delete h;
}

int polar_get_params(const polar_code_t *h, int *n, int *N, int *K, int *crc) {
    if (!h) return fail(POLAR_E_ARG, "NULL handle");
    if (n) *n = h->n;
    if (N) *N = h->N;
    if (K) *K = h->K;
    if (crc) *crc = h->crc;
    return POLAR_OK;
}
int polar_get_frozen(const polar_code_t *h, uint8_t *o) {
    if (!h || !o) return fail(POLAR_E_ARG, "NULL argument");
    memcpy(o, h->frozen.data(), h->N); return POLAR_OK;
}
int polar_get_order(const polar_code_t *h, uint16_t *o) {
    if (!h || !o) return fail(POLAR_E_ARG, "NULL argument");
    memcpy(o, h->order.data(), 2 * (size_t)h->N); return POLAR_OK;
}
int polar_get_bitrev(const polar_code_t *h, uint16_t *o) {
    if (!h || !o) return fail(POLAR_E_ARG, "NULL argument");
    memcpy(o, h->bitrev.data(), 2 * (size_t)h->N); return POLAR_OK;
}
int polar_get_weak_leaves(const polar_code_t *h) { return h ? h->weak_leaves : -1; }
int polar_get_crc_matrix(const polar_code_t *h, uint8_t *m) {
    if (!h || (!m && h->crc)) return fail(POLAR_E_ARG, "NULL argument");
    if (h->crc) memcpy(m, h->crcm.data(), (size_t)h->crc * h->K);
    return POLAR_OK;
}

int polar_set_crc_matrix(polar_code_t *h, const uint8_t *m) {
    if (!h || (!m && h->crc)) return fail(POLAR_E_ARG, "NULL argument");
    drop_clones(h);
    if (h->crc) memcpy(h->crcm.data(), m, (size_t)h->crc * h->K);
    int rc = derive_tables(h);
    if (rc) return rc;
    if (h->dev_ready) {
        if ((rc = upload(h->d_crc_mask, h->crc_mask))) return rc;
        if ((rc = upload(h->d_crcm, h->crcm))) return rc;
    }
    return POLAR_OK;
}

int polar_set_tuning(polar_code_t *h, int waves_per_cu, int lds_log) {
    if (!h) return fail(POLAR_E_ARG, "NULL handle");
    if (waves_per_cu < 0 || waves_per_cu > 32) return fail(POLAR_E_ARG, "waves_per_cu out of range");
    if (lds_log != 0 && (lds_log < 2 || lds_log > 5)) return fail(POLAR_E_ARG, "lds_log must be 0 or 2..5");
    if (lds_log == 2 && waves_per_cu != 0 && waves_per_cu <= 8)
        return fail(POLAR_E_ARG, "lds_log = 2 exists only for the 4-wave-block kernels (waves_per_cu > 8)");
    h->waves_per_cu = waves_per_cu;
    h->lds_log = lds_log;
    drop_clones(h);
    return POLAR_OK;
}

int polar_set_mode(polar_code_t *h, int mode) {
    if (!h) return fail(POLAR_E_ARG, "NULL handle");
    if (mode < 0 || mode > 2) return fail(POLAR_E_ARG, "mode must be 0 (auto), 1 (LLR-domain) or 2 (exp-domain)");
    h->mode = mode;
    drop_clones(h);
    return POLAR_OK;
}

double polar_snr_sqrt_linear(const polar_code_t *h, double ebno_db) {
    if (!h) return NAN;
    return std::pow(10.0f, ebno_db / 20) * std::sqrt(((double)h->K) / ((double)h->N));
}

}
```

### polar_amd/csrc/polar_host.h

```cpp
#pragma once
#include <hip/hip_runtime.h>

#include <dlfcn.h>
#include <sched.h>
#include <sys/mman.h>
#include <unistd.h>

#include <algorithm>
#include <atomic>
#include <chrono>
#include <condition_variable>
#include <memory>
#include <mutex>
#include <thread>
#include <cmath>
#include <cstdarg>
#include <cstdio>
#include <cstdlib>
#include <cstring>
#include <functional>
#include <numeric>
#include <string>
#include <vector>

#include "polar_amd.h"
#include "polar_kernels.h"
#include "polar_synth.h"

namespace polar_host {

extern thread_local std::string g_err;
int fail(int code, const char *fmt, ...);

#define HIP_TRY(expr)                                                                      \
    do {                                                                                   \
        hipError_t e_ = (expr);                                                            \
        if (e_ != hipSuccess)                                                              \
            return fail(POLAR_E_DEVICE, "%s failed: %s (%s:%d)", #expr, hipGetErrorString(e_), __FILE__, __LINE__); \
    } while (0)

extern std::atomic<unsigned long> g_allocs;

template <typename T>
struct DevBuf {
    T *p = nullptr;
    size_t cap = 0;
    int ensure(size_t n) {
        if (n <= cap) return POLAR_OK;
        if (p) (void)hipFree(p);
        p = nullptr; cap = 0;
        ++g_allocs;
        hipError_t e = hipMalloc((void **)&p, n * sizeof(T));
        if (e != hipSuccess) return fail(POLAR_E_NOMEM, "hipMalloc(%zu bytes) failed: %s", n * sizeof(T), hipGetErrorString(e));
        cap = n;
        return POLAR_OK;
    }
    void release() { if (p) (void)hipFree(p); p = nullptr; cap = 0; }
};

int usable_cpus();

struct CopyPool {
    std::vector<std::thread> threads;
    std::mutex m;
    std::condition_variable cv_job, cv_done;
    unsigned gen = 0;
    bool quit = false;
    char *dst = nullptr; const char *src = nullptr; size_t bytes = 0;
    std::atomic<size_t> next{0};
    int pending = 0;
    static constexpr size_t kSlice = (size_t)1 << 20;
    void work() {
        for (;;) {
            const size_t off = next.fetch_add(kSlice);
            if (off >= bytes) return;
            memcpy(dst + off, src + off, std::min(kSlice, bytes - off));
        }
    }
    void start(int n) {
        for (int i = 0; i < n; ++i)
            threads.emplace_back([this] {
                unsigned seen = 0;
                for (;;) {
                    {
                        std::unique_lock<std::mutex> lk(m);
                        cv_job.wait(lk, [&] { return quit || gen != seen; });
                        if (quit) return;
                        seen = gen;
                    }
                    work();
                    std::lock_guard<std::mutex> lk(m);
                    if (--pending == 0) cv_done.notify_all();
                }
            });
    }
    void copy(void *d, const void *s, size_t n) {
        if (threads.empty() || n < 2 * kSlice) { memcpy(d, s, n); return; }
        {
            std::lock_guard<std::mutex> lk(m);
            dst = (char *)d; src = (const char *)s; bytes = n; next = 0; pending = (int)threads.size(); ++gen;
        }
        cv_job.notify_all();
        work();
        std::unique_lock<std::mutex> lk(m);
        cv_done.wait(lk, [&] { return pending == 0; });
    }
    ~CopyPool() {
        { std::lock_guard<std::mutex> lk(m); quit = true; }
        cv_job.notify_all();
        for (auto &t : threads) t.join();
    }
};

struct PrefaultPool {
    std::vector<std::thread> threads;
    std::mutex m;
    std::condition_variable cv_job, cv_done;
    unsigned gen = 0;
    bool quit = false;
    uintptr_t lo = 0, hi = 0, pg = 4096;
    std::atomic<uintptr_t> next{0};
    int pending = 0;
    static constexpr uintptr_t kStep = (uintptr_t)2 << 20;
    void work() {
        for (;;) {
            const uintptr_t q = next.fetch_add(kStep);
            if (q >= hi) return;
            const size_t len = (size_t)std::min(kStep, hi - q);
#ifdef MADV_POPULATE_WRITE
            if (madvise((void *)q, len, MADV_POPULATE_WRITE) == 0) continue;
#endif
            for (uintptr_t r = q; r < q + len; r += pg) __atomic_fetch_add((volatile unsigned char *)r, (unsigned char)0, __ATOMIC_RELAXED);
        }
    }
    void start_threads(int n) {
        pg = (uintptr_t)sysconf(_SC_PAGESIZE);
        for (int i = 0; i < n; ++i)
            threads.emplace_back([this] {
                unsigned seen = 0;
                for (;;) {
                    {
                        std::unique_lock<std::mutex> lk(m);
                        cv_job.wait(lk, [&] { return quit || gen != seen; });
                        if (quit) return;
                        seen = gen;
                    }
                    work();
                    std::lock_guard<std::mutex> lk(m);
                    if (--pending == 0) cv_done.notify_all();
                }
            });
    }
    void start(void *p, size_t bytes) {
        const uintptr_t a = ((uintptr_t)p + pg - 1) & ~(pg - 1), b = ((uintptr_t)p + bytes) & ~(pg - 1);
        if (threads.empty() || b <= a + 64 * pg) return;
        {
            std::lock_guard<std::mutex> lk(m);
            lo = a; hi = b; next = a; pending = (int)threads.size(); ++gen;
        }
        cv_job.notify_all();
    }
    void wait() {
        std::unique_lock<std::mutex> lk(m);
        cv_done.wait(lk, [&] { return pending == 0; });
    }
    ~PrefaultPool() {
        { std::lock_guard<std::mutex> lk(m); quit = true; }
        cv_job.notify_all();
        for (auto &t : threads) t.join();
    }
};

}
using namespace polar_host;

struct HostPipe {
    static constexpr int kMaxLanes = 8, kMaxSlots = kMaxLanes + 2;
    int R = 0;
    hipStream_t copy = nullptr, lane[kMaxLanes] = {};
    hipEvent_t h2d[kMaxSlots] = {}, done[kMaxSlots] = {};
    void *pin_in[kMaxSlots] = {}; uint8_t *pin_out[kMaxSlots] = {};
    void *d_in[kMaxSlots] = {}; uint8_t *d_out[kMaxSlots] = {};
    size_t in_cap = 0, out_cap = 0;
    polar_code *ctx[kMaxLanes] = {};
    std::unique_ptr<CopyPool> pool;
    std::unique_ptr<PrefaultPool> prefault;
    long last_chunks = 0, last_chunk_cw = 0, last_lanes = 0, last_threads = 0;
    long us_copy_in = 0, us_wait = 0, us_copy_out = 0, us_total = 0;
};

struct polar_code {
    int n = 0, N = 0, K = 0, crc = 0;
    double eps = 0.0;
    std::vector<uint8_t> frozen;
    std::vector<uint16_t> order;
    std::vector<uint16_t> bitrev;
    std::vector<uint8_t> crcm;
    int W = 0;
    std::vector<uint16_t> info_rank;
    std::vector<uint32_t> crc_mask;
    std::vector<uint8_t> sched;
    std::vector<uint32_t> ctl;
    int weak_leaves = 0;
    std::vector<uint32_t> sc_ops;
    std::vector<uint32_t> sc_lat_ops;
    bool sc_fold = false;
    bool dev_ready = false;
    int device = -1, num_cu = 0;
    size_t lds_per_block = 0;
    DevBuf<uint8_t> d_frozen, d_crcm;
    DevBuf<uint16_t> d_order, d_info_rank;
    DevBuf<uint32_t> d_crc_mask, d_ctl, d_sc_ops, d_sc_lat_ops, d_var_scr;
    DevBuf<double> d_tab_scr;
    DevBuf<unsigned long long> d_head_rec;
    int last_head_phi = 0;
    long last_head_b = 0;
    long last_lat_waves = 0;
    long last_lane_waves = 0;
    const unsigned int *fb_count = nullptr;
    const uint32_t *fb_list = nullptr;
    void *fb_stream = nullptr;
    long fb_b = 0;
    void note_fallback(const unsigned int *count, const uint32_t *list, void *st, long B) { fb_count = count; fb_list = list; fb_stream = st; fb_b = B; }
    DevBuf<unsigned int> d_flag_words;
    DevBuf<double> d_llr_scr, d_tabs, d_pre;
    DevBuf<uint32_t> d_c_scr, d_hist_scr;
    DevBuf<double> d_in;
    DevBuf<float> d_f32;
    DevBuf<uint8_t> d_out, d_bytes_a, d_bytes_b;
    DevBuf<unsigned long long> d_counter;
    DevBuf<unsigned int> d_work;
    DevBuf<uint64_t> d_sel;
    DevBuf<double> d_ech;
    DevBuf<uint8_t> d_flags;
    DevBuf<uint32_t> d_list;
    DevBuf<unsigned int> d_count;
    DevBuf<double> d_list_out;
    DevBuf<double> d_metric_scr;
    DevBuf<unsigned int> d_adapt_ctl;
    std::vector<uint32_t> flip_ops;
    DevBuf<uint32_t> d_flip_ops;
    DevBuf<int32_t> d_flip_i32;
    DevBuf<double> d_bicm_llr;
    int mode = 0;
    struct Knobs {
        int mode_override = -1;
        bool sc_no_fold = false;
        bool no_tables = false;
        bool no_head = false;
        long head_min_b = 0;
        bool no_fuse_front = false;
        bool no_rccl = false;
        bool force_rccl = false;
        bool share_device = false;
        int fail_device = -1;
        int fail_collective = -1;
        long multi_timeout_s = 1800;
        long multi_grace_s = 10;
        bool force_workers = false;
        int stall_device = -1;
        long stall_ms = 0;
        long lat_max_b = 0;
        long host_pipe_min_bytes = 0;
        long host_chunk_bytes = 0;
        long host_lanes = 0;
        long host_threads = 0;
        long host_ramp = 0;
        long host_fail_alloc = 0;
        long lat_grid = 0;
        long lane_grid = 0;
        long list_chunk_cw = 0;
        long host_prefault = 0;
    } knobs;
    DevBuf<uint64_t> d_alive[2];
    DevBuf<unsigned int> d_nalive;
    DevBuf<unsigned long long> d_mc_ctr;
    struct McSlot { DevBuf<uint64_t> list[2]; int cur = 0; long cnt = 0; };
    std::vector<McSlot> mc_slots;
    DevBuf<unsigned int> d_slot_n;
    std::vector<unsigned int> h_slot_n;
    std::vector<polar_code *> clones;
    struct MultiCtx *multi = nullptr;
    bool multi_poisoned = false;
    bool ctx_stuck = false;
    void *pin_in = nullptr, *pin_in_dev = nullptr;
    uint8_t *pin_out = nullptr, *pin_out_dev = nullptr;
    size_t pin_in_cap = 0, pin_out_cap = 0;
    uint8_t *lat_flag_bytes = nullptr;
    struct HostPipe *hpipe = nullptr;
    long last_rounds = 0, last_round_max_per_device = 0, worker_threads_started = 0;
    std::vector<long> round_us;
    int waves_per_cu = 0, lds_log = 0, pipe = -1;
    bool prefix_on = true;
};

namespace polar_host {

struct DevGuard {
    int prev = -1;
    ~DevGuard() { if (prev >= 0) (void)hipSetDevice(prev); }
};

inline int pow2ceil(int v) { int p = 1; while (p < v) p <<= 1; return p; }
inline bool is_ask_constellation(int c) { return c >= POLAR_CONST_ASK4_GRAY && c <= POLAR_CONST_ASK16_SP; }
inline bool is_ask_not_bpsk(int c) { return is_ask_constellation(c) && c != POLAR_CONST_BPSK; }
inline double sigma_of_snr_db(double snr_db) { return std::sqrt(1.0 / 2) * std::pow(10.0, -snr_db / 20); }

int derive_tables(polar_code *h);
int ensure_device(polar_code *h, DevGuard &dg);
void drop_clones(polar_code *h);
template <typename T>
int upload(DevBuf<T> &d, const std::vector<T> &v) {
    size_t n = v.size() ? v.size() : 1;
    int rc = d.ensure(n);
    if (rc) return rc;
    if (v.size()) HIP_TRY(hipMemcpy(d.p, v.data(), v.size() * sizeof(T), hipMemcpyHostToDevice));
    return POLAR_OK;
}
inline int stage_rows(polar_code *h, const void *rows, int fmt, long B) {
    const size_t bytes = (size_t)B * h->N * polar_llr_esz(fmt);
    if (int rc = h->d_in.ensure((bytes + 7) / 8)) return rc;
    HIP_TRY(hipMemcpy(h->d_in.p, rows, bytes, hipMemcpyHostToDevice));
    return POLAR_OK;
}
template <typename T>
int copy_back(T *dst, size_t at, const T *d_src, size_t n) {
    if (dst) HIP_TRY(hipMemcpy(dst + at, d_src, n * sizeof(T), hipMemcpyDeviceToHost));
    return POLAR_OK;
}
inline int lat_grid(polar_code *h, long grid) {
    if (h->knobs.lat_grid > 0) grid = std::min<long>(grid, h->knobs.lat_grid);
    h->last_lat_waves = grid;
    return (int)grid;
}
inline long lane_grid(const polar_code *h, long want) {
    return h->knobs.lane_grid > 0 ? std::min<long>(want, h->knobs.lane_grid) : want;
}
inline long chunk_len(const polar_code *h, long T, size_t budget, size_t per) {
    return std::min<long>(T, h->knobs.list_chunk_cw > 0 ? h->knobs.list_chunk_cw : std::max<long>(1, (long)(budget / per)));
}
constexpr int kNoList = 1;
inline int check_args(bool ptrs_set, int L, long B, const std::function<int()> &mid = nullptr) {
    if (!ptrs_set) return fail(POLAR_E_ARG, "NULL argument");
    if (int rc = mid ? mid() : POLAR_OK) return rc;
    if (L < 1 || L > POLAR_MAX_LIST) return fail(POLAR_E_ARG, "list size %d out of range [1, %d]", L, POLAR_MAX_LIST);
    return B < 0 ? fail(POLAR_E_ARG, "negative batch") : POLAR_OK;
}
inline size_t scratch_budget(const polar_code *h) {
    size_t budget = (size_t)24 << 30, free_b = 0, total_b = 0;
    if (hipMemGetInfo(&free_b, &total_b) == hipSuccess) budget = std::min(budget, (free_b + h->d_llr_scr.cap * sizeof(double)) / 2);
    return std::max(budget, (size_t)64 << 20);
}
template <typename Ensure>
int grid_that_fits(const polar_code *h, long want, size_t per_wave, Ensure ensure, int *grid_out) {
    long grid = want;
    if ((size_t)want * per_wave > h->d_llr_scr.cap * sizeof(double)) grid = std::max<long>(1, std::min<long>(want, (long)(scratch_budget(h) / per_wave)));
    for (;;) {
        const int rc = ensure((int)grid);
        if (rc != POLAR_E_NOMEM || grid <= 64) { *grid_out = (int)grid; return rc; }
        (void)hipGetLastError();
        grid /= 2;
    }
}

enum class Family { Sc8, ScLat, ListLat, BatchLlr, BatchEd };
Family choose_family(const polar_code *h, long B, int L, bool want_pm);
enum class Deferred { None, FlagWords, FlagBytes };
int decode_impl(polar_code *h, const void *d_llr, int llr_fmt, long B, const unsigned int *n_dev, int L, uint8_t *d_out,
                double *d_pm, void *stream, void *ev_start, void *ev_stop, int phase = 0, Deferred *deferred = nullptr);
struct BatchGeometry { int gs, G, wpc, lds_log, pipe, wpb, grid; size_t big, cwords; };
bool batch_geometry(const polar_code *h, long B, int L, bool tuned, BatchGeometry &g);
int ensure_batch_scratch(polar_code *h, const BatchGeometry &g);
int default_scratch(polar_code *h, BatchGeometry *g, int n);
void base_params(const polar_code *h, int L, long B, PolarDecodeParams &p);
int prefix_params(polar_code *h, int gs, PolarDecodeParams &p);
static_assert(POLAR_LLR_F64 == 0 && POLAR_LLR_F32 == 1 && POLAR_LLR_F16 == 2 && POLAR_LLR_BF16 == 3, "POLAR_LLR_* codes");
int llr_fmt_check(int fmt, const void *rows);
void fill_enc(const polar_code *h, PolarEncodeParams &p);
int mlc_check(const polar_code *h, int constellation, int *cid);
void fill_mlc(const polar_code *h, int cid, double snr_db, PolarMlcParams &p);
int mlc_decode_launch(polar_code *h, int cid, const double *d_y, double n0, long B, const unsigned int *n_dev, double *d_out,
                      uint8_t *d_out_bytes, hipStream_t st);
int bicm_check(int constellation, double n0);
void fill_demap(int cid, int N, double n0, PolarDemapParams &p);
int bicm_front(polar_code *c, int cid, double n0, const void *d_y, int y_f32, long B, hipStream_t st, const double **d_llr);
void fill_channel(const polar_code *h, PolarEncodeParams &p, int constellation, double snr_point);
struct Sweep { polar_code *h; int cid; uint64_t seed, t0; long T, stride; const double *axis; uint64_t *stats; DevGuard dg; };
struct SweepCell { int point; long chunk; size_t ctr; int width; };
int sweep_begin(Sweep &sw, polar_code *h, bool ptrs_set, const char *what, int constellation, uint64_t seed, uint64_t t0, long T,
                long stride, const double *axis, bool sizes_ok, uint64_t *stats, const std::function<int()> &own);
int sweep_walk(Sweep &sw, const std::vector<SweepCell> &cells, size_t n_ctr, const std::function<int(const SweepCell &, long)> &body);
struct SymRows { int cid, M; double n0; };
int host_decode(polar_code *h, const void *rows, int rows_fmt, const SymRows *sym, long B, int L, uint8_t *out);
void hostpipe_release(polar_code *h);
void multi_release(polar_code *h, bool abort_comms);
polar_code *copy_ctx(polar_code *h, int dev);
polar_code *clone_on_device(polar_code *h, int dev, bool fresh = false);

}
```

### polar_amd/csrc/polar_kernels.hip

```cpp
#include <hip/hip_runtime.h>
#include <stdint.h>
#include <type_traits>

#include "polar_kernels.h"
#include "polar_device.h"
#include "polar_edom.h"

#ifdef POLAR_PROFILE
#define PROF_DECL u64 prof_acc[24] = {0,0,0,0,0,0,0,0,0,0,0,0,0,0,0,0,0,0,0,0,0,0,0,0}; u64 prof_t = __builtin_readcyclecounter();
#define PROF(i) { u64 t_ = __builtin_readcyclecounter(); prof_acc[i] += t_ - prof_t; prof_t = t_; }
#define PROF_OUT if (lane == 0 && p.pm_out) { for (int i_ = 0; i_ < 24; ++i_) atomicAdd((u64 *)p.pm_out + i_, prof_acc[i_]); }
#define PROF_CNT(i, v) { prof_acc[i] += (u64)(v); }
#define PROF_HEAD_DECL const int prof_head_phi = p.pm_out ? (int)((const u64 *)p.pm_out)[32] : 0; const u64 prof_head_t0 = prof_t; bool prof_head_open = prof_head_phi > 0;
#define PROF_HEAD(phi_) if (prof_head_open && (phi_) >= prof_head_phi) { prof_acc[22] += __builtin_readcyclecounter() - prof_head_t0; prof_head_open = false; }
#define PROF_HEAD_END prof_acc[23] += __builtin_readcyclecounter() - prof_head_t0;
#else
#define PROF_HEAD_DECL
#define PROF_HEAD(phi_)
#define PROF_HEAD_END
#define PROF_DECL
#define PROF(i)
#define PROF_CNT(i, v)
#define PROF_OUT
#endif

#include "polar_llr_nodes.h"

template <bool NARROW16>
__device__ __forceinline__ const double *ch_row(const PolarDecodeParams &p, size_t cw, int N) {
    if constexpr (NARROW16) {
        if (p.llr_fmt >= POLAR_LLR_F16) return reinterpret_cast<const double *>(reinterpret_cast<const uint16_t *>(p.llr) + cw * (size_t)N);
    }
    return p.llr_fmt ? reinterpret_cast<const double *>(reinterpret_cast<const float *>(p.llr) + cw * (size_t)N)
                     : p.llr + cw * (size_t)N;
}
template <bool NARROW16>
__device__ __forceinline__ double ch_narrow(const double *row, size_t i, int fmt) {
    if constexpr (NARROW16) return llr_load_narrow(row, i, fmt);
    else return (double)reinterpret_cast<const float *>(row)[i];
}
#define CH(row, i) (p.llr_fmt ? ch_narrow<CH_N16>(row, i, p.llr_fmt) : (row)[i])

#ifndef FU
#define FU 4
#endif
#ifndef POLAR_SKIP_L1
#define POLAR_SKIP_L1 1
#endif
#define POLAR_SADDR 1
#ifndef OCC
#define OCC 4
#endif
#define LANE_CTX                                   \
    const int lane = LAT ? lane_k : lane_id_opaque();    \
    const int lig = lane & (GS - 1);               \
    const int gbase = lane & ~(GS - 1);            \
    (void)lig; (void)gbase;
#if defined(POLAR_ED_TU) && POLAR_ED_TU == 4
#define POLAR_LIST_OUT 1
#define scl_decode_llr_kernel scl_decode_llr_list_kernel
#define POLAR_KPARAMS PolarListParams
#elif defined(POLAR_ED_TU) && POLAR_ED_TU == 7
#define POLAR_ADAPT_OUT 1
#define scl_decode_llr_kernel scl_decode_llr_adapt_kernel
#define POLAR_KPARAMS PolarAdaptParams
#elif defined(POLAR_ED_TU) && (POLAR_ED_TU == 5 || POLAR_ED_TU == 6)
#define POLAR_HEAD (POLAR_ED_TU == 5 ? 1 : 2)
#define scl_decode_llr_kernel scl_decode_llr_head_kernel
#define POLAR_KPARAMS PolarHeadParams
#else
#define POLAR_KPARAMS PolarDecodeParams
#endif
#ifndef POLAR_HEAD
#define POLAR_HEAD 0
#endif
template <int GS, int LDS_LOG, int PIPE, bool ED, int NL = 0, int LAT = 0>
__global__ __launch_bounds__(PIPE ? 64 : 256, PIPE ? 2 : OCC) void scl_decode_llr_kernel(POLAR_KPARAMS p) {
    constexpr int WPB = PIPE ? 1 : 4;
    constexpr bool CH_N16 = !ED;
    constexpr int G = LAT ? 1 : 64 / GS;
    constexpr int EL = 64 / GS;
    constexpr int CST = LAT ? GS : 64;
#define POLAR_CL (LAT ? lig : lane)
#define POLAR_CGB (LAT ? 0 : gbase)
    constexpr int SL = 1 << LDS_LOG;
    const int lane = threadIdx.x & 63;
    const int wib = __builtin_amdgcn_readfirstlane((int)(threadIdx.x >> 6));
    const int wave_id = blockIdx.x * WPB + wib;
    const int nwaves = gridDim.x * WPB;
    const int lane_k = lane;
    (void)lane_k;
    const int lig = lane & (GS - 1);
    const int gbase = lane & ~(GS - 1);
    const int grp = LAT ? 0 : lane / GS;
    const int n = NL ? NL : p.n, N = NL ? (1 << NL) : p.N, K = p.K, L = p.L;
    const u64 gmask = (GS == 64) ? ~0ull : ((1ull << GS) - 1ull);

    extern __shared__ __attribute__((aligned(16))) unsigned char smem[];
    double *tabs = reinterpret_cast<double *>(smem);
    constexpr size_t WAVE_LDS = (size_t)(2 * SL - 1) * 64 * 8 + 128 * 8 + 128;
    unsigned char *wbase = smem + 324 * 8 + (size_t)wib * WAVE_LDS;
    double *lds_llr = reinterpret_cast<double *>(wbase);
    double *sortbuf = lds_llr + (LAT ? 0 : (size_t)(2 * SL - 1) * 64);
    unsigned char *stackv = reinterpret_cast<unsigned char *>(sortbuf + 128);
    unsigned char *srcof = stackv + 64;
    for (int i = threadIdx.x; i < 322; i += WPB * 64) tabs[i] = p.tabs[i];
    if (WPB > 1) __syncthreads();
    const Tabs tb = {tabs, tabs + 64, tabs + 64 + 129};
    u64 guard = 0;
    double gacc = __builtin_inf();
    auto FN = [&](double a, double b) -> double {
        if constexpr (ED) return f_node_e_acc(a, b, gacc); else return f_node(a, b, tb);
    };
    auto GN = [&](double a, double b, uint32_t cw_, int bi) -> double {
        if constexpr (ED) return g_node_e(a, b, cw_ << (31 - bi), tb); else return g_node(a, b, (cw_ >> bi) & 1u);
    };
    const long Bv = p.cw_count ? (long)*p.cw_count : (p.n_dev ? ((long)*p.n_dev < p.B ? (long)*p.n_dev : p.B) : p.B);

    const size_t big_elems = (N > 2 * SL) ? (size_t)(N - 2 * SL) : 0;
    double *g_llr = LAT ? nullptr : p.llr_scr + (size_t)wave_id * big_elems * 64;
    const int cwords = (N >= 128) ? (N / 32 - 2) : 0;
    double *lat_ch = reinterpret_cast<double *>(stackv + 128);
    double *lat_a = lat_ch + N;
    uint32_t *lat_w = reinterpret_cast<uint32_t *>(lat_a + (size_t)N * GS);
    uint32_t *g_cl = LAT ? lat_w : p.c_scr + (size_t)wave_id * 2 * (size_t)cwords * 64;
    uint32_t *g_cr = g_cl + (size_t)cwords * CST;
    uint32_t *g_hist = LAT ? g_cr + (size_t)cwords * CST : p.hist_scr + (size_t)wave_id * 3 * (size_t)p.W * 64;
    uint32_t *g_horg = g_hist + (size_t)p.W * CST;
    uint32_t *g_tb = g_horg + (size_t)p.W * CST;
    const int S1 = N / 2, S2 = N / 4;
    const bool tbl = ED && !PIPE && GS == 32 && N >= 1024 && p.tab_scr != nullptr && p.prefix_q > 0;
    double *tab_w = tbl ? p.tab_scr + (size_t)wave_id * G * (size_t)(3 * N) : nullptr;
    uint32_t *g_v = tbl ? p.var_scr + (size_t)wave_id * (size_t)(S2 / 8) * 64 : nullptr;

    for (long g0 = (long)wave_id * G; g0 < Bv;) {
        const long cwi = g0 + grp;
        const bool valid = (cwi < Bv);
        const long cw = (p.cw_list && valid) ? (long)p.cw_list[cwi] : cwi;
        guard = 0;
        gacc = __builtin_inf();
        auto cw_of_lane = [&](int ln) -> size_t {
            const long i = g0 + (LAT ? 0 : ln / GS);
            return p.cw_list ? (size_t)p.cw_list[i < Bv ? i : Bv - 1] : (size_t)i;
        };
        auto FN2 = [&](double a0_, double b0_, double a1_, double b1_, double &r0_, double &r1_) {
            if constexpr (ED) { r0_ = f_node_e_acc(a0_, b0_, gacc); r1_ = f_node_e_acc(a1_, b1_, gacc); }
            else f_node2(a0_, b0_, a1_, b1_, tb, r0_, r1_);
        };

        bool active = valid && (lig == L - 1);
        u64 actw = __ballot(active);
        double pm = 0.0;
        int sp = L - 1;
        if (lig < L - 1) stackv[gbase + lig] = (unsigned char)lig;
        P16 pL = {0, 0};
        P16 pC = {0, 0};
        u64 clsmall = 0;
        uint32_t hword = 0;
        int origin = lig;
        unsigned t = 0;
        if constexpr (LAT) {
            bool any = false, sized = false;
            const size_t row = (size_t)(valid ? cw : 0) * (size_t)N;
            for (int i0 = 0; i0 < N; i0 += 64 * 8) {
                double x[8];
#pragma unroll
                for (int k = 0; k < 8; ++k) {
                    const int i = i0 + 64 * k + lane;
                    x[k] = (i < N) ? (p.llr_fmt ? llr_load_narrow(p.llr, row + i, p.llr_fmt) : p.llr[row + i]) : 1.0;
                }
#pragma unroll
                for (int k = 0; k < 8; ++k) {
                    const int i = i0 + 64 * k + lane;
                    double v = x[k];
                    if constexpr (ED) { bool f; v = ed_from_channel(x[k], tb, f); any |= f; sized |= i < N && fabs(x[k]) >= 0.1; }
                    if (i < N) lat_ch[__brev((unsigned)i) >> (32 - n)] = v;
                }
            }
            if constexpr (ED) { if (wave_any(any) || !wave_any(sized)) guard = ~0ull; }
        }
        wave_mem_fence();

        int phi_start = 0, forced_top = 0;
#if POLAR_HEAD == 2
        {
            static_assert(GS == 32 && ED && !LAT && !PIPE && LDS_LOG == 3, "import exists for the list of 32 in its default tuning");
            const int la = lig - (L - 4);
            const bool mine = valid && la >= 0 && lig < L;
            const u64 *rec = p.head_rec + (size_t)(valid ? cw : 0) * (size_t)p.head_rows * 4 + (mine ? la : 0);
            const u64 st_ = mine ? rec[8] : 0ull;
            active = (st_ >> 63) != 0;
            actw = __ballot(active);
            sp = L - __popcll((actw >> gbase) & gmask);
            if (active) {
                pm = __longlong_as_double((long long)rec[0]);
                clsmall = rec[4];
                hword = (uint32_t)st_;
                int r = 3;
                for (int s = 6; s < n; ++s) {
                    if (!((p.head_c_mask >> s) & 1u)) continue;
                    const int nwd = (1 << s) / 32;
                    uint32_t *dst = g_cl + (size_t)(nwd - 2) * 64 + lane;
#pragma unroll 1
                    for (int w = 0; w < nwd; w += 2) {
                        const u64 x0 = rec[(size_t)(r + w) * 4], x1 = rec[(size_t)(r + w + 1) * 4];
                        dst[(size_t)w * 64] = (uint32_t)x0; dst[(size_t)(w + 1) * 64] = (uint32_t)x1;
                    }
                    pC.set(s, lig);
                    r += nwd;
                }
                for (int s = 5; s < n; ++s) {
                    if (!((p.head_llr_mask >> s) & 1u)) continue;
                    const int T = 1 << s;
                    double *dst = g_llr + (size_t)(T - 2 * SL) * 64 + lane;
#pragma unroll 1
                    for (int j = 0; j < T; j += 4) {
                        u64 x[4];
#pragma unroll
                        for (int k = 0; k < 4; ++k) x[k] = rec[(size_t)(r + j + k) * 4];
#pragma unroll
                        for (int k = 0; k < 4; ++k) dst[(size_t)(j + k) * 64] = __longlong_as_double((long long)x[k]);
                    }
                    pL.set(s, lig);
                    r += T;
                }
            }
            t = (unsigned)p.head_t;
            wave_mem_fence();
            phi_start = p.head_phi;
        }
#else
        const double *pre_cw = nullptr;
        if (!LAT && p.prefix_q > 0) {
            const int Q = p.prefix_q, Pe = p.prefix_len;
            pre_cw = p.pre + (size_t)(valid ? cw : 0) * (size_t)(N - Q + 1);
            if (active) {
                pm = pre_cw[0];
                for (int S = 64; S <= Q && S <= N / 2; S <<= 1) {
                    uint32_t *cz = g_cl + (size_t)(S / 32 - 2) * 64 + lane;
                    for (int w = 0; w < S / 32; ++w) cz[(size_t)w * 64] = 0u;
                    pC.set(__builtin_ctz((unsigned)S), lig);
                }
            }
            wave_mem_fence();
            phi_start = Pe;
            if (Pe < Q) forced_top = n - __builtin_ctz((unsigned)Q) + 1;
        }
#endif

        PROF_DECL
        PROF_HEAD_DECL
#ifdef POLAR_MARGIN
        double mingap = __builtin_inf();
#endif
        typedef const uint32_t __attribute__((address_space(4))) *kconst_u32;
        const kconst_u32 ctlp = (kconst_u32)(uintptr_t)p.ctl;
        uint32_t ctlv = 0, ctlv_n = 0;
        double lat_x[4] = {0.0, 0.0, 0.0, 0.0}, lat_y0 = 0.0, lat_y1 = 0.0;
        bool lat_yv = false;
        (void)lat_x; (void)lat_y0; (void)lat_y1; (void)lat_yv;
        auto ctl_window = [&](int w0) -> uint32_t { const int i_ = w0 + lane_id_opaque(); return p.ctl[i_ < N ? i_ : 0]; };
        uint32_t ctl_next;
        if constexpr (LAT) {
            ctlv = ctl_window(phi_start & ~63);
            ctlv_n = ctl_window((phi_start & ~63) + 64);
            ctl_next = (uint32_t)__builtin_amdgcn_readlane((int)ctlv, phi_start & 63);
        } else ctl_next = ctlp[phi_start];
#if POLAR_HEAD == 1
        for (int phi = phi_start; phi < p.head_phi; ++phi) {
#else
        for (int phi = phi_start; phi < N; ++phi) {
#endif
            PROF_HEAD(phi)
            PROF(0)
            const uint32_t ctl = ctl_next;
            auto update_c = [&](int S, uint32_t X, int ph) {
                LANE_CTX
                if constexpr (LAT) {
                    if (S == 1 && N >= 128) {
                        uint32_t lo = (uint32_t)clsmall, hi = (uint32_t)(clsmall >> 32);
                        bool done = false;
                        auto level = [&](auto SC_) {
                            constexpr int Sc = decltype(SC_)::value;
                            if (done) return;
                            const uint32_t cl = (Sc == 16) ? (lo >> 16) : ((lo >> Sc) & ((1u << Sc) - 1u));
                            const uint32_t nw = (cl ^ X) | (X << Sc);
                            if (!((ph >> 1) & 1)) {
                                if constexpr (Sc == 16) hi = nw;
                                else if constexpr (Sc == 8) lo = (lo & 0x0000FFFFu) | (nw << 16);
                                else lo = (lo & ~(((1u << (2 * Sc)) - 1u) << (2 * Sc))) | (nw << (2 * Sc));
                                done = true;
                            } else { X = nw; ph >>= 1; }
                        };
                        level(std::integral_constant<int, 1>{}); level(std::integral_constant<int, 2>{}); level(std::integral_constant<int, 4>{});
                        level(std::integral_constant<int, 8>{}); level(std::integral_constant<int, 16>{});
                        if (done) {
                            if (active) clsmall = ((u64)hi << 32) | lo;
                            return;
                        }
                        S = 32;
                    }
                }
                for (;;) {
                    if (4 * S > N) break;
                    const int psi = ph >> 1;
                    const bool to_right = (psi & 1);
                    const int sh = __builtin_ctz((unsigned)S);
                    if (S <= 16) {
                        uint32_t cl = (uint32_t)(clsmall >> S) & ((1u << S) - 1u);
                        uint32_t nw = (cl ^ X) | (X << S);
                        if (!to_right) {
                            const int S2 = 2 * S;
                            const u64 m = ((S2 == 32) ? 0xFFFFFFFFull : ((1ull << S2) - 1ull)) << S2;
                            if (active) clsmall = (clsmall & ~m) | ((u64)nw << S2);
                        }
                        X = nw;
                    } else if (S == 32) {
                        uint32_t cl = (uint32_t)(clsmall >> 32);
                        uint32_t *dst = (to_right ? g_cr : g_cl) + (size_t)0 * CST + POLAR_CL;
                        if (active) { dst[0] = cl ^ X; dst[CST] = X; }
                        if (!to_right && active) pC.set(sh + 1, lig);
                    } else {
                        const int nwd = S / 32;
                        const uint32_t *cl = g_cl + (size_t)(nwd - 2) * CST + POLAR_CGB + pC.get(sh);
                        const uint32_t *cr = g_cr + (size_t)(nwd - 2) * CST + POLAR_CL;
                        uint32_t *dst = (to_right ? g_cr : g_cl) + (size_t)(2 * nwd - 2) * CST + POLAR_CL;
                        if (active) {
                            auto chunk = [&](auto CH_) {
                                constexpr int CH = decltype(CH_)::value;
                                for (int w = 0; w < nwd; w += CH) {
                                    uint32_t r[CH], l[CH];
#pragma unroll
                                    for (int i = 0; i < CH; ++i) { r[i] = cr[(size_t)(w + i) * CST]; l[i] = cl[(size_t)(w + i) * CST]; }
#pragma unroll
                                    for (int i = 0; i < CH; ++i) { dst[(size_t)(w + i) * CST] = l[i] ^ r[i]; dst[(size_t)(w + i + nwd) * CST] = r[i]; }
                                }
                            };
                            if (nwd >= 8) chunk(std::integral_constant<int, 8>{});
                            else if (nwd == 4) chunk(std::integral_constant<int, 4>{});
                            else chunk(std::integral_constant<int, 2>{});
                            if (!to_right) pC.set(sh + 1, lig);
                        }
                    }
                    wave_mem_fence();
                    if (!to_right) break;
                    S *= 2;
                    ph = psi;
                }
            };
            const int zb = (int)(ctl >> 1) & 0x7F;
            {
                const int nphi = phi + (1 << zb);
                if constexpr (LAT) {
                    if (POLAR_UNLIKELY2(((nphi ^ phi) & ~63) != 0)) { ctlv = ctlv_n; ctlv_n = ctl_window((nphi & ~63) + 64); }
                    ctl_next = (uint32_t)__builtin_amdgcn_readlane((int)ctlv, nphi & 63);
                } else ctl_next = ctlp[nphi < N ? nphi : 0];
            }
            const int lam_stop = n - zb;
#include "polar_scl_visits.inc"
#include "polar_scl_leaf.inc"
        }
        PROF_HEAD_END
        PROF_OUT

#if POLAR_HEAD == 1
        {
            static_assert(GS == 4 && ED && !LAT && !PIPE && LDS_LOG == 3, "export exists for the groups of 4 lanes in the default tuning");
            (void)K; (void)g_tb;
            if (valid) {
                u64 *rec = p.head_rec + (size_t)cw * (size_t)p.head_rows * 4 + lig;
                rec[0] = active ? (u64)__double_as_longlong(pm) : 0ull;
                rec[4] = clsmall;
                rec[8] = (u64)hword | ((u64)t << 32) | ((u64)(active ? 1 : 0) << 63);
                if (active) {
                    int r = 3;
                    for (int s = 6; s < n; ++s) {
                        if (!((p.head_c_mask >> s) & 1u)) continue;
                        const int nwd = (1 << s) / 32;
                        const uint32_t *src = g_cl + (size_t)(nwd - 2) * 64 + gbase + pC.get(s);
                        for (int w = 0; w < nwd; w += 2) {
                            const uint32_t x0 = src[(size_t)w * 64], x1 = src[(size_t)(w + 1) * 64];
                            rec[(size_t)(r + w) * 4] = x0; rec[(size_t)(r + w + 1) * 4] = x1;
                        }
                        r += nwd;
                    }
                    for (int s = 5; s < n; ++s) {
                        if (!((p.head_llr_mask >> s) & 1u)) continue;
                        const int T = 1 << s;
                        const double *src = g_llr + (size_t)(T - 2 * SL) * 64 + gbase + pL.get(s);
                        for (int j = 0; j < T; j += 8) {
                            double x[8];
#pragma unroll
                            for (int k = 0; k < 8; ++k) x[k] = src[(size_t)(j + k) * 64];
#pragma unroll
                            for (int k = 0; k < 8; ++k) rec[(size_t)(r + j + k) * 4] = (u64)__double_as_longlong(x[k]);
                        }
                        r += T;
                    }
                }
            }
            guard |= __ballot(gacc <= ED_GACC_FLAG);
            if (valid && lig == 0 && ((guard >> gbase) & gmask) != 0) p.flags[cw] = 1;
            wave_mem_fence();
        }
#else
#include "polar_scl_finish.inc"
#endif
        if (p.work) {
            unsigned nxt = 0;
            if (lane == 0) nxt = atomicAdd(p.work, 1u);
            g0 = ((long)nwaves + (long)__builtin_amdgcn_readfirstlane((int)nxt)) * G;
        } else {
            g0 += (long)nwaves * G;
        }
    }
}

template <bool ED>
__global__ __launch_bounds__(256) void prefix_kernel(PolarDecodeParams p, int staged, double *ech_out) {
    __shared__ double tabs[324];
    extern __shared__ double pstage[];

    for (int i = threadIdx.x; i < 322; i += 256) tabs[i] = p.tabs[i];
    __syncthreads();
    const Tabs tb = {tabs, tabs + 64, tabs + 64 + 129};
    u64 guard = 0;
    auto FN = [&](double a, double b) -> double {
        if constexpr (ED) return f_node_e(a, b, guard); else return f_node(a, b, tb);
    };
    auto GN0 = [&](double a, double b) -> double {
        if constexpr (ED) return g_node_e(a, b, 0u, tb); else return g_node(a, b, 0u);
    };
    constexpr bool CH_N16 = true;
    const int lane = threadIdx.x & 63, lig = lane & 31, gbase = lane & 32;
    const int n = p.n, N = p.N, Q = p.prefix_q, Pe = p.prefix_len;
    const int R = Q >> 5;
    const long per_block = 8;
    const long Bv = p.n_dev ? ((long)*p.n_dev < p.B ? (long)*p.n_dev : p.B) : p.B;
    for (long c0 = (long)blockIdx.x * per_block; c0 < Bv; c0 += (long)gridDim.x * per_block) {
        const long cw = c0 + (threadIdx.x >> 5);
        const bool valid = cw < Bv;
        const double *in0 = ch_row<CH_N16>(p, (size_t)(valid ? cw : 0), N);
        double *pre = const_cast<double *>(p.pre) + (size_t)(valid ? cw : 0) * (size_t)(N - Q + 1);
        double x[8] = {0, 0, 0, 0, 0, 0, 0, 0};
        bool bad_in = false;
        for (int S = N / 2; S >= Q; S >>= 1) {
            if (valid && staged && 2 * S == N) {
                double *stg = pstage + (size_t)(threadIdx.x >> 5) * (size_t)S;
                double *outp = pre + 1;
                if (ED && ech_out) {
                    double *erow = ech_out + (size_t)cw * (size_t)N;
                    bool any = false, sized = false;
                    int m = lig;
                    for (; m + 96 < S; m += 128) {
                        double x0[4], x1[4];
#pragma unroll
                        for (int k = 0; k < 4; ++k) { x0[k] = CH(in0, 2 * (m + 32 * k)); x1[k] = CH(in0, 2 * (m + 32 * k) + 1); }
#pragma unroll
                        for (int k = 0; k < 4; ++k) {
                            const int mk = m + 32 * k;
                            bool f0, f1;
                            const double a = ed_from_channel(x0[k], tb, f0), b = ed_from_channel(x1[k], tb, f1);
                            any |= f0 | f1;
                            sized |= (fabs(x0[k]) >= 0.1) | (fabs(x1[k]) >= 0.1);
                            erow[2 * mk] = a; erow[2 * mk + 1] = b;
                            stg[__brev((unsigned)mk) >> (33 - n)] = FN(a, b);
                        }
                    }
                    for (; m < S; m += 32) {
                        const double x0 = CH(in0, 2 * m), x1 = CH(in0, 2 * m + 1);
                        bool f0, f1;
                        const double a = ed_from_channel(x0, tb, f0), b = ed_from_channel(x1, tb, f1);
                        any |= f0 | f1;
                        sized |= (fabs(x0) >= 0.1) | (fabs(x1) >= 0.1);
                        erow[2 * m] = a; erow[2 * m + 1] = b;
                        stg[__brev((unsigned)m) >> (33 - n)] = FN(a, b);
                    }
                    const u64 m_any = __builtin_amdgcn_ballot_w64(any), m_sz = __builtin_amdgcn_ballot_w64(sized);
                    const u64 half = gbase ? 0xFFFFFFFF00000000ull : 0x00000000FFFFFFFFull;
                    bad_in = ((m_any & half) != 0) || ((m_sz & half) == 0);
                } else {
                    for (int m = lig; m < S; m += 32) {
                        const double r = FN(CH(in0, 2 * m), CH(in0, 2 * m + 1));
                        stg[__brev((unsigned)m) >> (33 - n)] = r;
                    }
                }
                wave_mem_fence();
                for (int j = lig; j < S; j += 32) {
                    const double r = stg[j];
                    outp[j] = r;
                    if (S == Q) {
#pragma unroll
                        for (int rr = 0; rr < 8; ++rr) if (rr == (j >> 5)) x[rr] = r;
                    }
                }
                wave_mem_fence();
            } else if (valid && staged) {
                double *stg = pstage + (size_t)(threadIdx.x >> 5) * (size_t)(N / 2);
                double *outp = pre + 1 + (size_t)(N - 2 * S);
                for (int j = lig; j < S; j += 32) {
                    const double r = FN(stg[j], stg[j + S]);
                    stg[j] = r;
                    outp[j] = r;
                    if (S == Q) {
#pragma unroll
                        for (int rr = 0; rr < 8; ++rr) if (rr == (j >> 5)) x[rr] = r;
                    }
                }
                wave_mem_fence();
            } else if (valid) {
                const bool from_ch = (2 * S == N);
                const double *inp = pre + 1 + (size_t)(N - 4 * S);
                double *outp = pre + 1 + (size_t)(N - 2 * S);
                int j = lig;
                for (; j + 96 < S; j += 128) {
                    double a[4], b[4];
#pragma unroll
                    for (int k = 0; k < 4; ++k) {
                        if (from_ch) {
                            const unsigned idx = __brev((unsigned)(j + 32 * k)) >> (32 - n);
                            a[k] = CH(in0, idx); b[k] = CH(in0, idx + 1);
                        } else {
                            a[k] = inp[j + 32 * k]; b[k] = inp[j + 32 * k + S];
                        }
                    }
#pragma unroll
                    for (int k = 0; k < 4; ++k) {
                        const double r = FN(a[k], b[k]);
                        outp[j + 32 * k] = r;
                        if (S == Q) {
#pragma unroll
                            for (int rr = 0; rr < 8; ++rr) if (rr == ((j + 32 * k) >> 5)) x[rr] = r;
                        }
                    }
                }
                for (; j < S; j += 32) {
                    double a, b;
                    if (from_ch) {
                        unsigned idx = __brev((unsigned)j) >> (32 - n);
                        a = CH(in0, idx); b = CH(in0, idx + 1);
                    } else {
                        a = inp[j]; b = inp[j + S];
                    }
                    const double r = FN(a, b);
                    outp[j] = r;
                    if (S == Q) {
#pragma unroll
                        for (int rr = 0; rr < 8; ++rr) if (rr == (j >> 5)) x[rr] = r;
                    }
                }
            }
            wave_mem_fence();
        }
        for (int h = Q / 2; h >= 1; h >>= 1) {
            if (h >= 32) {
                const int hr = h >> 5;
#pragma unroll
                for (int r = 0; r < 8; ++r) {
                    if (r < R && (r & hr) == 0) {
#pragma unroll
                        for (int r2 = 0; r2 < 8; ++r2) {
                            if (r2 == r + hr) {
                                const double lo = x[r], hi = x[r2];
                                x[r] = FN(lo, hi);
                                x[r2] = GN0(lo, hi);
                            }
                        }
                    }
                }
            } else {
#pragma unroll
                for (int r = 0; r < 8; ++r) {
                    if (r < R) {
                        const double mine = x[r];
                        const double other = shfl_d(mine, lane ^ h);
                        x[r] = (lig & h) ? GN0(other, mine) : FN(mine, other);
                    }
                }
            }
        }
        double acc = 0.0;
#pragma unroll
        for (int r = 0; r < 8; ++r) {
            if (r < R && r * 32 < Pe) {
                bool ng; double al, sneg, spos;
                leaf_terms<ED>(x[r], true, __builtin_amdgcn_ballot_w64(true), tb, ng, al, sneg, spos);
                const double spv = ng ? spos : sneg;
                const int cnt = (Pe - r * 32 < 32) ? (Pe - r * 32) : 32;
#pragma unroll
                for (int c = 0; c < 32; ++c) {
                    const double t = shfl_d(spv, gbase + c);
                    acc = (c < cnt) ? acc + t : acc;
                }
            }
        }
        if (valid && lig == 0) pre[0] = acc;
        if constexpr (ED) {
            const bool fl = ((guard >> gbase) & 0xFFFFFFFFull) != 0;
            if (ech_out) { if (valid && lig == 0) p.flags[cw] = (fl || bad_in) ? 1 : 0; }
            else if (valid && lig == 0 && fl) p.flags[cw] = 1;
            guard = 0;
        }
        wave_mem_fence();
    }
}

#ifndef POLAR_ED_TU
#define POLAR_ED_TU 0
#endif
#if POLAR_ED_TU < 2
#if POLAR_ED_TU
hipError_t polar_launch_prefix_ed1(const PolarDecodeParams &p, double *ech_out, hipStream_t st) {
#else
hipError_t polar_launch_prefix_ed0(const PolarDecodeParams &p, double *ech_out, hipStream_t st) {
#endif
    long blocks = (p.B + 7) / 8;
    if (blocks > 8192) blocks = 8192;
    const size_t stage = (size_t)8 * (size_t)(p.N / 2) * sizeof(double);
    const int staged = polar_prefix_is_staged(p.N);
    if (ech_out && !staged) return hipErrorInvalidValue;
    hipLaunchKernelGGL(prefix_kernel<POLAR_ED_TU != 0>, dim3((unsigned)blocks), dim3(256), staged ? stage : 0, st, p, staged, ech_out);
    return hipGetLastError();
}
#endif

#if !POLAR_ED_TU
int polar_prefix_is_staged(int N) { return (N >= 64 && (size_t)8 * (size_t)(N / 2) * sizeof(double) <= 64 * 1024) ? 1 : 0; }
hipError_t polar_launch_prefix(const PolarDecodeParams &p, bool ed, double *ech_out, hipStream_t st) {
    return ed ? polar_launch_prefix_ed1(p, ech_out, st) : polar_launch_prefix_ed0(p, nullptr, st);
}
template <typename TIN>
__global__ __launch_bounds__(256) void ed_front_kernel(const TIN *llr, double *ech, uint8_t *flags, const double *tabs_g, int N, long B, const unsigned *n_dev) {
    if (n_dev && (long)*n_dev < B) B = (long)*n_dev;
    __shared__ double tabs[324];
    for (int i = threadIdx.x; i < 322; i += 256) tabs[i] = tabs_g[i];
    __syncthreads();
    const Tabs tb = {tabs, tabs + 64, tabs + 64 + 129};
    const int lane = threadIdx.x & 63;
    for (long cw = (long)blockIdx.x * 4 + (threadIdx.x >> 6); cw < B; cw += (long)gridDim.x * 4) {
        const TIN *src = llr + (size_t)cw * N;
        double *dst = ech + (size_t)cw * N;
        bool any = false, sized = false;
        for (int i = lane; i < N; i += 64) {
            bool f;
            const double x = llr_widen(src[i]);
            dst[i] = ed_from_channel(x, tb, f);
            any |= f;
            sized |= fabs(x) >= 0.1;
        }
        const bool bad = wave_any(any) || !wave_any(sized);
        if (lane == 0) flags[cw] = bad ? 1 : 0;
    }
}
hipError_t polar_launch_ed_front(const void *llr, int llr_fmt, double *ech, uint8_t *flags, const double *tabs, int N, long B, const unsigned *n_dev, hipStream_t st) {
    long blocks = (B + 3) / 4;
    if (blocks > 16384) blocks = 16384;
    if (llr_fmt == POLAR_LLR_F32) hipLaunchKernelGGL(ed_front_kernel<float>, dim3((unsigned)blocks), dim3(256), 0, st, (const float *)llr, ech, flags, tabs, N, B, n_dev);
    else if (llr_fmt == POLAR_LLR_F16) hipLaunchKernelGGL(ed_front_kernel<polar_f16>, dim3((unsigned)blocks), dim3(256), 0, st, (const polar_f16 *)llr, ech, flags, tabs, N, B, n_dev);
    else if (llr_fmt == POLAR_LLR_BF16) hipLaunchKernelGGL(ed_front_kernel<polar_bf16>, dim3((unsigned)blocks), dim3(256), 0, st, (const polar_bf16 *)llr, ech, flags, tabs, N, B, n_dev);
    else hipLaunchKernelGGL(ed_front_kernel<double>, dim3((unsigned)blocks), dim3(256), 0, st, (const double *)llr, ech, flags, tabs, N, B, n_dev);
    return hipGetLastError();
}
__global__ __launch_bounds__(256) void ed_collect_kernel(const uint8_t *flags, long B, const unsigned *n_dev, uint32_t *list, unsigned *count) {
    if (n_dev && (long)*n_dev < B) B = (long)*n_dev;
    for (long cw = (long)blockIdx.x * 256 + threadIdx.x; cw < B; cw += (long)gridDim.x * 256)
        if (flags[cw]) list[atomicAdd(count, 1u)] = (uint32_t)cw;
}
hipError_t polar_launch_ed_collect(const uint8_t *flags, long B, const unsigned *n_dev, uint32_t *list, unsigned *count, hipStream_t st) {
    long blocks = (B + 255) / 256;
    if (blocks > 1024) blocks = 1024;
    hipLaunchKernelGGL(ed_collect_kernel, dim3((unsigned)blocks), dim3(256), 0, st, flags, B, n_dev, list, count);
    return hipGetLastError();
}

#endif

template <int GS, bool ED>
static hipError_t launch_gs(const PolarDecodeParams &p, int lds_log, int pipe, int grid, hipStream_t st) {
    size_t lds = polar_decode_lds_bytes(lds_log, pipe);
    const int wpb = polar_decode_waves_per_block(pipe);
#define POLAR_LAUNCH(LL, PP) hipLaunchKernelGGL((scl_decode_llr_kernel<GS, LL, PP, ED>), dim3(grid / wpb), dim3(64 * wpb), lds, st, p)
#ifndef POLAR_NO_FIXED_N
    if constexpr (GS == 32 && ED) {
        if (lds_log == 3 && !pipe && (p.n == 11 || p.n == 10)) {
            if (p.n == 11) hipLaunchKernelGGL((scl_decode_llr_kernel<GS, 3, 0, ED, 11>), dim3(grid / wpb), dim3(64 * wpb), lds, st, p);
            else hipLaunchKernelGGL((scl_decode_llr_kernel<GS, 3, 0, ED, 10>), dim3(grid / wpb), dim3(64 * wpb), lds, st, p);
            return hipGetLastError();
        }
    }
#endif
    switch (lds_log * 2 + (pipe ? 1 : 0)) {
        case 6: POLAR_LAUNCH(3, 0); break;
#ifndef POLAR_DEV_ONE
        case 4: POLAR_LAUNCH(2, 0); break;
        case 7: POLAR_LAUNCH(3, 1); break;
        case 8: POLAR_LAUNCH(4, 0); break;
        case 9: POLAR_LAUNCH(4, 1); break;
        case 10: POLAR_LAUNCH(5, 0); break;
        case 11: POLAR_LAUNCH(5, 1); break;
#endif
        default: return hipErrorInvalidValue;
    }
#undef POLAR_LAUNCH
    return hipGetLastError();
}

template <int GS, bool ED>
static hipError_t launch_lat(const PolarDecodeParams &p, int blocks, hipStream_t st) {
    const size_t lds = polar_decode_lat_lds_bytes(p.N, GS, p.W);
    const hipError_t e = hipFuncSetAttribute(reinterpret_cast<const void *>(&scl_decode_llr_kernel<GS, 3, 1, ED, 0, 1>), hipFuncAttributeMaxDynamicSharedMemorySize, (int)lds);
    if (e != hipSuccess) return e;
    hipLaunchKernelGGL((scl_decode_llr_kernel<GS, 3, 1, ED, 0, 1>), dim3(blocks), dim3(64), lds, st, p);
    return hipGetLastError();
}
#if POLAR_ED_TU == 3
hipError_t polar_launch_decode_lat_ed1(const PolarDecodeParams &p, int gs, int blocks, hipStream_t st) {
    switch (gs) {
        case 2: return launch_lat<2, true>(p, blocks, st);
        case 4: return launch_lat<4, true>(p, blocks, st);
        case 8: return launch_lat<8, true>(p, blocks, st);
        default: return hipErrorInvalidValue;
    }
}
#elif POLAR_ED_TU == 0
hipError_t polar_launch_decode_lat_ed1(const PolarDecodeParams &p, int gs, int blocks, hipStream_t st);
hipError_t polar_launch_decode_lat(const PolarDecodeParams &p, int gs, bool ed, int blocks, hipStream_t st) {
    if (ed) return polar_launch_decode_lat_ed1(p, gs, blocks, st);
    if (gs == 2) return launch_lat<2, false>(p, blocks, st);
    return hipErrorInvalidValue;
}
size_t polar_decode_lat_lds_bytes(int N, int gs, int W) {
    return 324 * 8 + (128 * 8 + 128) + (size_t)N * 8 + (size_t)N * gs * 8 + (2 * polar_decode_cwords(N) + (size_t)3 * W) * gs * 4 + 64;
}
#endif

#if POLAR_ED_TU == 4 || POLAR_ED_TU == 7
template <int GS>
static hipError_t launch_finish(const POLAR_KPARAMS &p, int grid, hipStream_t st) {
    const int wpb = polar_decode_waves_per_block(0);
    const size_t lds = polar_decode_lds_bytes(3, 0);
    hipLaunchKernelGGL((scl_decode_llr_kernel<GS, 3, 0, false>), dim3(grid / wpb), dim3(64 * wpb), lds, st, p);
    return hipGetLastError();
}
static hipError_t launch_finish_gs(const POLAR_KPARAMS &p, int gs, int grid, hipStream_t st) {
    switch (gs) {
        case 1: return launch_finish<1>(p, grid, st);
        case 2: return launch_finish<2>(p, grid, st);
        case 4: return launch_finish<4>(p, grid, st);
        case 8: return launch_finish<8>(p, grid, st);
        case 16: return launch_finish<16>(p, grid, st);
        case 32: return launch_finish<32>(p, grid, st);
        case 64: return launch_finish<64>(p, grid, st);
        default: return hipErrorInvalidValue;
    }
}
#if POLAR_ED_TU == 4
hipError_t polar_launch_decode_llr_list(const PolarListParams &p, int gs, int grid, hipStream_t st) {
    if (!p.list_cand || grid < 4 || (grid & 3)) return hipErrorInvalidValue;
    return launch_finish_gs(p, gs, grid, st);
}
#else
hipError_t polar_launch_decode_llr_adapt(const PolarAdaptParams &p, int gs, int grid, hipStream_t st) {
    if (!p.out || !p.ad_retry || grid < 4 || (grid & 3)) return hipErrorInvalidValue;
    return launch_finish_gs(p, gs, grid, st);
}
#endif
#elif POLAR_ED_TU == 5
hipError_t polar_launch_decode_head_export(const PolarHeadParams &p, int grid, hipStream_t st) {
    if (!p.head_rec || p.L != 4 || p.head_phi <= 0 || p.head_phi >= p.N || grid < 4 || (grid & 3)) return hipErrorInvalidValue;
    hipLaunchKernelGGL((scl_decode_llr_kernel<4, 3, 0, true>), dim3(grid / 4), dim3(256), polar_decode_lds_bytes(3, 0), st, p);
    return hipGetLastError();
}
#elif POLAR_ED_TU == 6
hipError_t polar_launch_decode_head_import(const PolarHeadParams &p, int grid, hipStream_t st) {
    if (!p.head_rec || p.L < 17 || p.L > 32 || p.head_phi <= 0 || p.head_phi >= p.N || grid < 4 || (grid & 3)) return hipErrorInvalidValue;
    const size_t lds = polar_decode_lds_bytes(3, 0);
#ifndef POLAR_NO_FIXED_N
    if (p.n == 11) hipLaunchKernelGGL((scl_decode_llr_kernel<32, 3, 0, true, 11>), dim3(grid / 4), dim3(256), lds, st, p);
    else if (p.n == 10) hipLaunchKernelGGL((scl_decode_llr_kernel<32, 3, 0, true, 10>), dim3(grid / 4), dim3(256), lds, st, p);
    else
#endif
    hipLaunchKernelGGL((scl_decode_llr_kernel<32, 3, 0, true>), dim3(grid / 4), dim3(256), lds, st, p);
    return hipGetLastError();
}
#elif POLAR_ED_TU == 2
hipError_t polar_launch_decode_llr_ed1_gs32(const PolarDecodeParams &p, int lds_log, int pipe, int grid, hipStream_t st) {
    return launch_gs<32, true>(p, lds_log, pipe, grid, st);
}
#elif POLAR_ED_TU == 1
hipError_t polar_launch_decode_llr_ed1_gs32(const PolarDecodeParams &p, int lds_log, int pipe, int grid, hipStream_t st);
hipError_t polar_launch_decode_llr_ed1(const PolarDecodeParams &p, int gs, int lds_log, int pipe, int grid, hipStream_t st) {
    switch (gs) {
#ifndef POLAR_DEV_GS32
        case 4: return launch_gs<4, true>(p, lds_log, pipe, grid, st);
        case 8: return launch_gs<8, true>(p, lds_log, pipe, grid, st);
        case 16: return launch_gs<16, true>(p, lds_log, pipe, grid, st);
        case 64: return launch_gs<64, true>(p, lds_log, pipe, grid, st);
#endif
        case 32: return polar_launch_decode_llr_ed1_gs32(p, lds_log, pipe, grid, st);
        default: return hipErrorInvalidValue;
    }
}
#elif POLAR_ED_TU == 0
hipError_t polar_launch_decode_llr_ed0(const PolarDecodeParams &p, int gs, int lds_log, int pipe, int grid, hipStream_t st) {
    switch (gs) {
        case 1: return launch_gs<1, false>(p, lds_log, pipe, grid, st);
#ifndef POLAR_DEV_GS32
        case 2: return launch_gs<2, false>(p, lds_log, pipe, grid, st);
        case 4: return launch_gs<4, false>(p, lds_log, pipe, grid, st);
        case 8: return launch_gs<8, false>(p, lds_log, pipe, grid, st);
        case 16: return launch_gs<16, false>(p, lds_log, pipe, grid, st);
        case 64: return launch_gs<64, false>(p, lds_log, pipe, grid, st);
#endif
        case 32: return launch_gs<32, false>(p, lds_log, pipe, grid, st);
        default: return hipErrorInvalidValue;
    }
}
hipError_t polar_launch_decode_llr(const PolarDecodeParams &p, int gs, int lds_log, int pipe, int grid, bool ed, hipStream_t st) {
    return ed ? polar_launch_decode_llr_ed1(p, gs, lds_log, pipe, grid, st) : polar_launch_decode_llr_ed0(p, gs, lds_log, pipe, grid, st);
}
#endif
```

### polar_amd/csrc/polar_multi.cpp

```cpp
#include "polar_multi.h"

namespace polar_host {

Rccl g_rccl;
std::atomic<int> g_comm_inits{0};

void multi_release(polar_code *h, bool abort_comms) {
    MultiCtx *m = h->multi;
    if (!m) return;
    h->multi = nullptr;
    if (m->stuck) {
        for (auto &t : m->threads) t.detach();
        h->multi_poisoned = true;
        return;
    }
    m->stop_workers();
    int prev = -1;
    (void)hipGetDevice(&prev);
    for (size_t d = 0; d < m->comms.size(); ++d)
        if (void *c = m->take_comm((int)d)) {
            if (abort_comms && g_rccl.CommAbort) (void)g_rccl.CommAbort(c);
            else (void)g_rccl.CommDestroy(c);
        }
    for (size_t d = 0; d < m->streams.size(); ++d)
        if (m->streams[d]) { (void)hipSetDevice(m->devs[d]); (void)hipStreamDestroy(m->streams[d]); }
    if (prev >= 0) (void)hipSetDevice(prev);
    delete m;
}
polar_code *clone_on_device(polar_code *h, int dev, bool fresh) {
    if (!fresh) {
        if (dev == h->device) return h;
        for (polar_code *c : h->clones) if (c->device == dev) return c;
    }
    polar_code *c = copy_ctx(h, dev);
    h->clones.push_back(c);
    return c;
}
polar_code *copy_ctx(polar_code *h, int dev) {
    polar_code *c = new polar_code;
    c->n = h->n; c->N = h->N; c->K = h->K; c->crc = h->crc; c->eps = h->eps;
    c->frozen = h->frozen; c->order = h->order; c->bitrev = h->bitrev; c->crcm = h->crcm;
    c->W = h->W; c->info_rank = h->info_rank; c->crc_mask = h->crc_mask; c->sched = h->sched; c->ctl = h->ctl;
    c->sc_ops = h->sc_ops; c->sc_lat_ops = h->sc_lat_ops; c->sc_fold = h->sc_fold; c->weak_leaves = h->weak_leaves;
    c->device = dev;
    c->waves_per_cu = h->waves_per_cu; c->lds_log = h->lds_log; c->pipe = h->pipe; c->prefix_on = h->prefix_on; c->mode = h->mode;
    c->knobs = h->knobs;
    return c;
}

}
```

### polar_amd/csrc/polar_scl_leaf.inc

```
            if (zb) {
                const int Z = 1 << zb;
                LANE_CTX
                auto block4 = [&](double v0, double v1, double v2, double v3) {
                    double lf[4] = {0, 0, 0, 0};
                    if (active) {
                        double a0, a1;
                        FN2(v0, v2, v1, v3, a0, a1);
                        const double b0 = GN(v0, v2, 0u, 0), b1 = GN(v1, v3, 0u, 0);
                        FN2(a0, a1, b0, b1, lf[0], lf[2]);
                        lf[1] = GN(a0, a1, 0u, 0); lf[3] = GN(b0, b1, 0u, 0);
                    }
                    if constexpr (LAT && ED) {
                        bool ng[4]; double alz[4], sneg[4], spos[4];
                        leaf_terms_ed_block<4>(lf, actw, tb, ng, alz, sneg, spos);
#pragma unroll
                        for (int i = 0; i < 4; ++i)
                            if (active) pm += ng[i] ? spos[i] : sneg[i];
                    } else {
#pragma unroll
                    for (int i = 0; i < 4; ++i) {
                        bool ng; double alz, sneg, spos;
                        leaf_terms<ED>(lf[i], active, actw, tb, ng, alz, sneg, spos);
                        if (active) pm += ng ? spos : sneg;
                    }
                    }
                };
                auto rate0 = [&](const double *yp, auto STR_) {
                    constexpr int YS = decltype(STR_)::value;
                    if (zb == 3) {
                        double a[4] = {0, 0, 0, 0}, b[4] = {0, 0, 0, 0};
                        if (active) {
#pragma unroll
                            for (int j = 0; j < 4; ++j) {
                                const double lo = yp[(size_t)j * YS], hi = yp[(size_t)(j + 4) * YS];
                                a[j] = FN(lo, hi);
                                b[j] = GN(lo, hi, 0u, 0);
                            }
                        }
                        block4(a[0], a[1], a[2], a[3]);
                        block4(b[0], b[1], b[2], b[3]);
                    } else {
                        double y[4] = {0, 0, 0, 0};
                        if (active) {
#pragma unroll
                            for (int j = 0; j < 4; ++j) y[j] = yp[(size_t)j * YS];
                        }
                        block4(y[0], y[1], y[2], y[3]);
                    }
                };
                if constexpr (LAT) rate0(lat_a + (size_t)(Z - 1) * GS + lig, std::integral_constant<int, GS>{});
                else if (Z <= SL) rate0(lds_llr + (size_t)(Z - 1) * 64 + lane, std::integral_constant<int, 64>{});
                else rate0(g_llr + (size_t)(Z - 2 * SL) * 64 + lane, std::integral_constant<int, 64>{});
                const int nu = phi >> zb;
                if ((nu & 1) == 0) {
                    if (active) clsmall &= ~((((u64)1 << Z) - 1ull) << Z);
                } else {
                    update_c(Z, 0u, nu);
                }
                wave_mem_fence();
                PROF(5)
                phi += Z - 1;
                continue;
            }
            LANE_CTX
            const u64 below = (1ull << lig) - 1ull;
            const bool frozen = (ctl & 1u) != 0;
            unsigned ubit = 0;
            if (frozen) {
                bool ng; double alz, sneg, spos;
                if constexpr (LAT && ED) {
                    const double lf1[1] = {leaf}; bool ng1[1]; double al1[1], sn1[1], sp1[1];
                    leaf_terms_ed_block<1>(lf1, actw, tb, ng1, al1, sn1, sp1);
                    ng = ng1[0]; alz = al1[0]; sneg = sn1[0]; spos = sp1[0];
                } else leaf_terms<ED>(leaf, active, actw, tb, ng, alz, sneg, spos);
                if (active) pm += ng ? spos : sneg;
            } else {
                const u64 actm = LAT ? (actw & gmask) : ((actw >> gbase) & gmask);
                const int nact = __popcll(actm);
                const int rho = (2 * nact < L) ? 2 * nact : L;
                bool lneg; double al;
                double gm = -__builtin_inf(), bl = __builtin_inf();
                double sneg, spos;
                if constexpr (LAT && ED) {
                    const double lf1[1] = {leaf}; bool ng1[1]; double al1[1], sn1[1], sp1[1];
                    leaf_terms_ed_block<1>(lf1, actw, tb, ng1, al1, sn1, sp1);
                    lneg = ng1[0]; al = al1[0]; sneg = sn1[0]; spos = sp1[0];
                } else leaf_terms<ED>(leaf, active, actw, tb, lneg, al, sneg, spos);
                if constexpr (ED) {
                    if (POLAR_UNLIKELY2(ctl & 0x100u)) guard |= __ballot(active && fabs(leaf) > 0.99999999 && fabs(leaf) <= 1.0);
                }
                if (active) {
                    gm = pm + sneg;
                    bl = (pm + al) * 0.99999999999909050530;
                }
                bool fast;
                {
                    unsigned gh = active ? (unsigned)__double2hiint(gm) : 0u;
                    unsigned bh = active ? (unsigned)__double2hiint(bl) : 0xFFFFFFFFu;
                    group_max_min_u32<GS>(gh, bh);
                    if constexpr (LAT) {
                        fast = (nact == 0) || (nact == L && ((__builtin_amdgcn_uicmp(gh, bh, 36) | ~group_result_rows<GS>()) == ~0ull));
                    } else {
                    const u64 m_ok = __builtin_amdgcn_sicmp(nact, 0, 32) | (__builtin_amdgcn_sicmp(nact, L, 32) & __builtin_amdgcn_uicmp(gh, bh, 36));
                    fast = ((m_ok | ~group_result_rows<GS>()) == ~0ull);
                    }
                }
                double gmax = 0.0;
                if (!fast) {
                    gmax = group_reduce<GS, true>(gm, lane);
                    const double bmin = group_reduce<GS, false>(bl, lane);
                    fast = wave_all((nact == 0) || (nact == L && gmax < bmin));
                }
                PROF_CNT(8, 1)
                PROF(16)
                if (fast) {
                    PROF_CNT(9, 1)
#ifdef POLAR_MARGIN
                    {
                        const double gx = group_reduce<GS, true>(active ? gm : -__builtin_inf(), lane);
                        const double bx = group_reduce<GS, false>(active ? pm + spos : __builtin_inf(), lane);
                        if (nact == L) mingap = __builtin_fmin(mingap, bx - gx);
                    }
#endif
                    if (active) {
                        ubit = lneg ? 1u : 0u;
                        pm = gm;
                        hword |= ubit << (t & 31);
                    }
                    PROF(17)
                } else {
                double pf0 = __builtin_nan(""), pf1 = __builtin_nan("");
                if (active) {
                    pf0 = -(pm + (lneg ? spos : sneg));
                    pf1 = -(pm + (lneg ? sneg : spos));
                }
                bool c0 = active, c1 = active;
                const bool need = (2 * nact > L);
                const bool full = (nact == L);
                if (POLAR_LIKELY2(!wave_any(need && !full))) {
                    const bool goodbit = lneg;
                    const double mg = goodbit ? -pf1 : -pf0;
                    const double mb = goodbit ? -pf0 : -pf1;
                    const bool cbad = active && full && !(bl > gmax);
                    const u64 cbm = __ballot(cbad);
                    bool sg, sbd;
                    if constexpr (GS == 32) {
                        const u64 actm64 = actw;
                        const u64 gbm = __ballot(goodbit);
                        u64 surv = 0;
                        PROF_CNT(10, 1)
                        PROF_CNT(11, __popcll(cbm))
                        for (u64 mi = cbm; mi; mi &= mi - 1) {
                            const int l_ = __builtin_ctzll(mi);
                            const double s_mb = readlane_d(mb, l_);
                            const u64 grp = 0xFFFFFFFFull << (l_ & 32);
                            const u64 blw = ((1ull << l_) - 1ull) & grp;
                            const u64 self_first = ~gbm & (1ull << l_);
                            const u64 lt_g = __builtin_amdgcn_fcmp(mg, s_mb, 4), eq_g = __builtin_amdgcn_fcmp(mg, s_mb, 1);
                            const u64 lt_b = __builtin_amdgcn_fcmp(mb, s_mb, 4), eq_b = __builtin_amdgcn_fcmp(mb, s_mb, 1);
                            const int r = __popcll((lt_g | (eq_g & (blw | self_first))) & grp & actm64) +
                                          __popcll((lt_b | (eq_b & blw)) & grp & cbm);
                            if (r < L) surv |= 1ull << l_;
                        }
                        PROF(18)
                        int k0 = __popcll(surv & 0xFFFFFFFFull), k1 = __popcll(surv >> 32);
                        u64 alive = actm64;
                        const unsigned khi = (unsigned)__double2hiint(mg) + 1u, klo = (unsigned)__double2loint(mg);
                        auto peel = [&](u64 e, int &k) {
                            const int ne = __popcll(e);
                            if (ne == 0) { k = 0; return; }
                            if (ne <= k) { alive &= ~e; k -= ne; return; }
                            for (; k > 0; --k) {
                                int best = -1; unsigned blo = 0;
                                for (u64 q = e; q; q &= q - 1) {
                                    const int l_ = __builtin_ctzll(q);
                                    const unsigned lo_ = (unsigned)__builtin_amdgcn_readlane((int)klo, l_);
                                    if (best < 0 || lo_ >= blo) { best = l_; blo = lo_; }
                                }
                                e &= ~(1ull << best);
                                alive &= ~(1ull << best);
                            }
                        };
                        while (k0 | k1) {
                            const unsigned h0 = __builtin_amdgcn_inverse_ballot_w64(alive) ? khi : 0u;
                            unsigned h = h0;
                            group_max_u32<GS>(h);
                            const unsigned m0 = (unsigned)__builtin_amdgcn_readlane((int)h, 31), m1 = (unsigned)__builtin_amdgcn_readlane((int)h, 63);
                            const u64 eq = __ballot(h0 == (lane < 32 ? m0 : m1)) & alive;
                            if (k0) peel(eq & 0xFFFFFFFFull, k0);
                            if (k1) peel(eq & 0xFFFFFFFF00000000ull, k1);
                        }
                        sg = __builtin_amdgcn_inverse_ballot_w64(alive);
                        sbd = __builtin_amdgcn_inverse_ballot_w64(surv);
                        PROF_CNT(13, (__popcll(surv & 0xFFFFFFFFull) > __popcll(surv >> 32)) ? __popcll(surv & 0xFFFFFFFFull) : __popcll(surv >> 32))
                        PROF(19)
                    } else {
                        sortbuf[lane] = mg;
                        wave_mem_fence();
                        int rg = 0, rb = 0;
                        const double *sb = sortbuf + gbase;
#pragma unroll 8
                        for (int i = 0; i < GS; ++i) {
                            const double v = sb[i];
                            const u64 below_me = __ballot(lig > i);
                            const u64 lt_g = __builtin_amdgcn_fcmp(v, mg, 4), le_g = __builtin_amdgcn_fcmp(v, mg, 5);
                            const u64 lt_b = __builtin_amdgcn_fcmp(v, mb, 4), le_b = __builtin_amdgcn_fcmp(v, mb, 5);
                            rg += (int)__builtin_amdgcn_inverse_ballot_w64((le_g & below_me) | (lt_g & ~below_me));
                            rb += (int)__builtin_amdgcn_inverse_ballot_w64((le_b & below_me) | (lt_b & ~below_me));
                        }
                        rb += (mg == mb && !goodbit) ? 1 : 0;
                        PROF(18)
                        sortbuf[64 + lane] = mb;
                        wave_mem_fence();
                        const double *sbb = sortbuf + 64 + gbase;
                        u64 any_i = 0;
#pragma unroll
                        for (int g = 0; g < 64 / GS; ++g) any_i |= (cbm >> (g * GS)) & gmask;
                        PROF_CNT(10, 1)
                        PROF_CNT(11, __popcll(any_i))
#ifdef POLAR_PROFILE
                        {
                            const double bmin_true = group_reduce<GS, false>(active ? mb : __builtin_inf(), lane);
                            const u64 cgm = __ballot(active && !(mg < bmin_true));
                            u64 any_g = 0;
                            for (int g = 0; g < 64 / GS; ++g) any_g |= (cgm >> (g * GS)) & gmask;
                            PROF_CNT(12, __popcll(any_g))
                        }
#endif
                        for (u64 mi = any_i; mi; mi &= mi - 1) {
                            const int i = __builtin_ctzll(mi);
                            const double v = sbb[i];
                            const u64 mine = __ballot(((cbm >> gbase) >> i) & 1ull);
                            const u64 below_me = __ballot(lig > i);
                            const u64 lt_g = __builtin_amdgcn_fcmp(v, mg, 4), le_g = __builtin_amdgcn_fcmp(v, mg, 5);
                            const u64 lt_b = __builtin_amdgcn_fcmp(v, mb, 4), le_b = __builtin_amdgcn_fcmp(v, mb, 5);
                            rg += (int)__builtin_amdgcn_inverse_ballot_w64(((le_g & below_me) | (lt_g & ~below_me)) & mine);
                            rb += (int)__builtin_amdgcn_inverse_ballot_w64(((le_b & below_me) | (lt_b & ~below_me)) & mine);
                        }
                        rg += (cbad && mg == mb && goodbit) ? 1 : 0;
                        PROF(19)
#ifdef POLAR_PROFILE
                        {
                            const u64 sbm = __ballot(cbad && rb < L);
                            int kmax = 0, ktot = 0;
                            for (int g = 0; g < 64 / GS; ++g) { const int k_ = __popcll((sbm >> (g * GS)) & gmask); kmax = k_ > kmax ? k_ : kmax; ktot += k_; }
                            PROF_CNT(13, kmax)
                            PROF_CNT(14, kmax <= 4 ? 1 : 0)
                            PROF_CNT(15, kmax == 0 ? 1 : 0)
                        }
#endif
                        sg = active && (rg < L);
                        sbd = cbad && (rb < L);
                    }
                    if (full) {
                        c0 = goodbit ? sbd : sg;
                        c1 = goodbit ? sg : sbd;
                    }
#ifdef POLAR_MARGIN
                    {
                        const double ninf = -__builtin_inf(), pinf = __builtin_inf();
                        const double sv = __builtin_fmax(sg ? mg : ninf, sbd ? mb : ninf);
                        const double kv = __builtin_fmin((active && !sg) ? mg : pinf, (active && !sbd) ? mb : pinf);
                        const double sx = group_reduce<GS, true>(sv, lane), kx = group_reduce<GS, false>(kv, lane);
                        if (full) mingap = __builtin_fmin(mingap, kx - sx);
                    }
#endif
                    wave_mem_fence();
                } else {
                    sortbuf[2 * lane] = pf0;
                    sortbuf[2 * lane + 1] = pf1;
                    wave_mem_fence();
                    int r0 = 0, r1 = 0;
                    const double *sb = sortbuf + 2 * gbase;
                    const int i0 = 2 * lig;
#pragma unroll 4
                    for (int i = 0; i < 2 * GS; ++i) {
                        const double v = sb[i];
                        r0 += (i < i0) ? (v >= pf0) : (v > pf0);
                        r1 += (i <= i0) ? (v >= pf1) : (v > pf1);
                    }
                    if (need) {
                        c0 = active && (r0 < rho);
                        c1 = active && (r1 < rho);
                    }
                    wave_mem_fence();
                }
                const bool kill = active && !c0 && !c1;
                const bool both = c0 && c1;
                const u64 km = (__ballot(kill) >> gbase) & gmask;
                const u64 bm = (__ballot(both) >> gbase) & gmask;
                srcof[lane] = (unsigned char)lig;
                if (POLAR_LIKELY2(wave_all(!active || full))) {
                    if (both) stackv[gbase + __popcll(bm & below)] = (unsigned char)lig;
                    wave_mem_fence();
                    if (kill) srcof[lane] = stackv[gbase + __popcll(km >> 1 >> lig)];
                    wave_mem_fence();
                } else {
                    if (kill) stackv[gbase + sp + __popcll(km & below)] = (unsigned char)lig;
                    sp += __popcll(km);
                    wave_mem_fence();
                    if (both) {
                        int lp = stackv[gbase + sp - 1 - __popcll(bm & below)];
                        srcof[gbase + lp] = (unsigned char)lig;
                    }
                    sp -= __popcll(bm);
                    wave_mem_fence();
                }
                const int src = srcof[lane];
                const bool is_clone = (src != lig);
                PROF(20)
                double pm_new = c0 ? -pf0 : -pf1;
                ubit = c0 ? 0u : 1u;
                if (wave_any(is_clone)) {
                    const int sl = gbase + src;
                    double pm1 = shfl_d(-pf1, sl);
                    u64 a0 = shfl_u64(pL.lo, sl), a1 = shfl_u64(pL.hi, sl);
                    u64 b0 = shfl_u64(pC.lo, sl), b1 = shfl_u64(pC.hi, sl);
                    u64 cs = shfl_u64(clsmall, sl);
                    uint32_t hw = __shfl(hword, sl, 64);
                    int og = __shfl(origin, sl, 64);
                    if (is_clone) {
                        pm_new = pm1; ubit = 1u;
                        pL.lo = a0; pL.hi = a1; pC.lo = b0; pC.hi = b1;
                        clsmall = cs; hword = hw; origin = og;
                    }
                    if constexpr (LAT) {
                        if ((n >= 3) ? ((phi & 1) == 0) : lat_yv) {
                            const double y0_ = shfl_d(lat_y0, sl), y1_ = shfl_d(lat_y1, sl);
                            if (is_clone) { lat_y0 = y0_; lat_y1 = y1_; }
                        }
                        if (n >= 3 && (phi & 3) < 2) {
                            double x_[4];
#pragma unroll
                            for (int k = 0; k < 4; ++k) x_[k] = shfl_d(lat_x[k], sl);
                            if (is_clone) {
#pragma unroll
                                for (int k = 0; k < 4; ++k) lat_x[k] = x_[k];
                            }
                        }
                    }
                }
                active = (active && !kill) || is_clone;
                actw = __ballot(active);
                if (active) {
                    pm = pm_new;
                    hword |= ubit << (t & 31);
                } else {
                    pm = 0.0;
                }
                PROF(21)
                }
                if (POLAR_UNLIKELY2((t & 31) == 31)) {
                    const int w = (int)(t >> 5);
                    if (active) {
                        g_hist[(size_t)w * CST + POLAR_CL] = hword;
                        g_horg[(size_t)w * CST + POLAR_CL] = (uint32_t)origin;
                        origin = lig;
                        hword = 0;
                    }
                    wave_mem_fence();
                }
                ++t;
            }

            PROF(frozen ? 5 : 6)
            if ((phi & 1) == 0) {
                if (active) clsmall = (clsmall & ~2ull) | ((u64)ubit << 1);
            } else {
                update_c(1, ubit, phi);
            }
            PROF(7)
```

Baseline: 1.067 million.

## Add speculative rate-1 leaf group fast path to the L=32 SCL decoder

Marks aligned groups of four consecutive unfrozen, non-weak leaves in a second control table. When the first leaf of such a group takes the fast path, the kernel computes the remaining three leaf LLRs directly from LDS and checks whether every list row would still keep its hard decision. If the check passes it commits all three bits, path metrics and the partial-sum update at once and skips three leaf iterations; otherwise it falls back to the normal per-leaf path. This is meant to cut the per-leaf tree traversal and reduction cost, at the price of extra speculative arithmetic and group reductions on groups that fail the check.

```diff
diff --git a/include/polar_amd_debug.h b/include/polar_amd_debug.h
--- a/include/polar_amd_debug.h
+++ b/include/polar_amd_debug.h
@@ -8,6 +8,7 @@
 int polar_debug_set(polar_code_t *h, const char *key, long value);
 long polar_debug_get(const polar_code_t *h, const char *key);
 long polar_debug_fallback_rows(polar_code_t *h, uint32_t *rows, long cap);
+long polar_debug_ctl_words(polar_code_t *h, uint32_t *words, long cap, int marked);
 int polar_debug_comm_inits(void);
 int polar_debug_weak_leaves(const polar_code_t *h);
 void *polar_debug_scratch_ptr(polar_code_t *h);
diff --git a/polar_amd/__init__.py b/polar_amd/__init__.py
--- a/polar_amd/__init__.py
+++ b/polar_amd/__init__.py
@@ -218,6 +218,16 @@
         if int(f(self._h, _p(rows, C.POINTER(C.c_uint32)), n)) != n:
             raise PolarError("polar_debug_fallback_rows: the count changed between two reads")
         return np.sort(rows[:n])
+
+    def debug_ctl_words(self, marked=True):
+        f = self._L.polar_debug_ctl_words
+        f.restype = C.c_long
+        f.argtypes = [C.c_void_p, C.POINTER(C.c_uint32), C.c_long, C.c_int]
+        words = np.zeros(self.N, np.uint32)
+        n = int(f(self._h, _p(words, C.POINTER(C.c_uint32)), self.N, 1 if marked else 0))
+        if n != self.N:
+            raise PolarError(f"polar_debug_ctl_words: {n}")
+        return words
 
     @classmethod
     def from_block_length(cls, block_length, info_length, design_epsilon, crc_size=0):
diff --git a/polar_amd/build.py b/polar_amd/build.py
--- a/polar_amd/build.py
+++ b/polar_amd/build.py
@@ -24,6 +24,7 @@
           [(f, [], "", []) for f in ("polar_handle.cpp", "polar_decode.cpp", "polar_hostpipe.cpp", "polar_montecarlo.cpp", "polar_multi.cpp",
                                      "polar_debug.cpp", "polar_ga.cpp", "polar_bicm.cpp", "polar_list.cpp", "polar_mlc.cpp", "polar_adaptive.cpp", "polar_flip.cpp")]
 TEST_HOOK_SOURCES = ("polar_montecarlo.cpp", "polar_debug.cpp")
+TEST_HOOK_KERNEL_TAGS = (".ed32", ".headB")
 LIB_TEST = os.path.join(HERE, "libpolar_amd_test.so")
 KNOWN_DEFS = {"POLAR_MARGIN", "POLAR_SLOTHIST", "SCLAT_PROF", "POLAR_DEV_GS32", "POLAR_DEV_ONE", "POLAR_NO_FIXED_N",
               "POLAR_NO_GUARD_INT", "POLAR_NO_COLD_HINTS", "OCC", "ED_NR"}
@@ -134,7 +135,7 @@
     jobs = []
     for s, defs, otag, xflags in SOURCES:
         src = os.path.join(CSRC, s)
-        if test_hooks and s in TEST_HOOK_SOURCES:
+        if test_hooks and (s in TEST_HOOK_SOURCES or (s == "polar_kernels.hip" and otag in TEST_HOOK_KERNEL_TAGS)):
             defs, otag = defs + ["POLAR_TEST_HOOKS"], otag + ".th"
         obj = os.path.join(BUILD, s + otag + tag + ".o")
         objs.append(obj)
diff --git a/polar_amd/csrc/polar_debug.cpp b/polar_amd/csrc/polar_debug.cpp
--- a/polar_amd/csrc/polar_debug.cpp
+++ b/polar_amd/csrc/polar_debug.cpp
@@ -2,6 +2,8 @@
 #include "polar_amd_debug.h"
 #ifdef POLAR_TEST_HOOKS
 #include "polar_head_plan.h"
+hipError_t polar_r1_counts_read_ed32(unsigned long long *out);
+hipError_t polar_r1_counts_read_head(unsigned long long *out);
 #endif
 
 extern "C" {
@@ -16,6 +18,7 @@
     else if (s == "sc_no_fold") k.sc_no_fold = value != 0;
     else if (s == "no_tables") k.no_tables = value != 0;
     else if (s == "no_head") k.no_head = value != 0;
+    else if (s == "no_r1") k.no_r1 = value != 0;
     else if (s == "head_min_b") { if (value < 0) return fail(POLAR_E_ARG, "head_min_b must be >= 0 (0 = default)"); k.head_min_b = value; }
     else if (s == "no_fuse_front") k.no_fuse_front = value != 0;
     else if (s == "no_prefix") h->prefix_on = (value == 0);
@@ -86,6 +89,11 @@
         }
         return bad;
     }
+    if (s == "r1_committed" || s == "r1_discarded") {
+        unsigned long long c[2] = {0, 0};
+        if ((h->last_head_phi ? polar_r1_counts_read_head(c) : polar_r1_counts_read_ed32(c)) != hipSuccess) return -2;
+        return (long)c[s == "r1_discarded" ? 1 : 0];
+    }
 #endif
     if (s == "last_rounds") return h->last_rounds;
     if (s == "last_round_max_per_device") return h->last_round_max_per_device;
@@ -127,4 +135,16 @@
     return e == hipSuccess ? (long)count : -(long)e - 1;
 }
 
+long polar_debug_ctl_words(polar_code_t *h, uint32_t *words, long cap, int marked) {
+    if (!h) return -1;
+    DevGuard dg_;
+    if (ensure_device(h, dg_)) return -1;
+    const long n = std::min<long>(h->N, cap);
+    if (words && n > 0) {
+        const hipError_t e = hipMemcpy(words, marked ? h->d_ctl_r1.p : h->d_ctl.p, (size_t)n * sizeof(uint32_t), hipMemcpyDeviceToHost);
+        if (e != hipSuccess) return -(long)e - 1;
+    }
+    return h->N;
 }
+
+}
diff --git a/polar_amd/csrc/polar_decode.cpp b/polar_amd/csrc/polar_decode.cpp
--- a/polar_amd/csrc/polar_decode.cpp
+++ b/polar_amd/csrc/polar_decode.cpp
@@ -241,7 +241,7 @@
     p.prefix_q = 0; p.prefix_len = 0; p.pre = nullptr;
     p.llr = nullptr; p.llr_fmt = POLAR_LLR_F64; p.p0 = nullptr; p.out = nullptr; p.pm_out = nullptr;
     p.frozen = h->d_frozen.p; p.info_rank = h->d_info_rank.p; p.crc_mask = h->d_crc_mask.p; p.tabs = h->d_tabs.p;
-    p.ctl = h->d_ctl.p; p.work = h->d_work.p; p.llr_scr = h->d_llr_scr.p; p.c_scr = h->d_c_scr.p; p.hist_scr = h->d_hist_scr.p;
+    p.ctl = h->knobs.no_r1 ? h->d_ctl.p : h->d_ctl_r1.p; p.work = h->d_work.p; p.llr_scr = h->d_llr_scr.p; p.c_scr = h->d_c_scr.p; p.hist_scr = h->d_hist_scr.p;
     p.flags = nullptr; p.cw_list = nullptr; p.cw_count = nullptr; p.n_dev = nullptr; p.tab_scr = nullptr; p.var_scr = nullptr;
 }
 
diff --git a/polar_amd/csrc/polar_handle.cpp b/polar_amd/csrc/polar_handle.cpp
--- a/polar_amd/csrc/polar_handle.cpp
+++ b/polar_amd/csrc/polar_handle.cpp
@@ -154,6 +154,23 @@
         for (int i = 0; i < N; ++i)
             if (!h->frozen[i] && om[i] < 1e-3) { h->ctl[i] |= 0x100u; ++h->weak_leaves; }
     }
+    h->ctl_r1 = h->ctl;
+    if (h->n >= 4) {
+        std::vector<int> tu((size_t)N + 1, 0);
+        for (int i = 0; i < N; ++i) tu[i + 1] = tu[i] + (h->frozen[i] ? 0 : 1);
+        auto rate1 = [&](int i0, int Z) {
+            if (i0 + Z > N) return false;
+            for (int i = i0; i < i0 + Z; ++i) {
+                if (h->frozen[i] || (h->ctl[i] & 0x100u)) return false;
+                if (i < i0 + Z - 1 && (tu[i] & 31) == 31) return false;
+            }
+            return true;
+        };
+        for (int i = 0; i < N; i += 4) {
+            if ((i & 7) == 0 && rate1(i, 8)) { h->ctl_r1[i] |= 3u << 9; h->ctl_r1[i + 4] |= 2u << 9; i += 4; continue; }
+            if (rate1(i, 4)) h->ctl_r1[i] |= 2u << 9;
+        }
+    }
     h->crc_mask.assign((size_t)crc * h->W, 0u);
     for (int i = 0; i < crc; ++i) {
         uint32_t *m = &h->crc_mask[(size_t)i * h->W];
@@ -190,6 +207,7 @@
     int rc;
     if ((rc = upload(h->d_frozen, h->frozen))) return rc;
     if ((rc = upload(h->d_ctl, h->ctl))) return rc;
+    if ((rc = upload(h->d_ctl_r1, h->ctl_r1))) return rc;
     if ((rc = upload(h->d_sc_ops, h->sc_ops))) return rc;
     if ((rc = upload(h->d_sc_lat_ops, h->sc_lat_ops))) return rc;
     if ((rc = upload(h->d_order, h->order))) return rc;
@@ -218,6 +236,7 @@
     h->knobs.sc_no_fold = on("POLAR_SC_NO_FOLD");
     h->knobs.no_tables = on("POLAR_NO_TABLES");
     h->knobs.no_head = on("POLAR_NO_HEAD");
+    h->knobs.no_r1 = on("POLAR_NO_R1");
     h->knobs.no_rccl = on("POLAR_NO_RCCL");
     h->knobs.force_rccl = on("POLAR_FORCE_RCCL");
     return POLAR_OK;
@@ -309,7 +328,7 @@
         if (h->dev_ready && hipGetDevice(&cur) == hipSuccess && cur != h->device) dg_.prev = cur;
     }
     if (h->dev_ready) (void)hipSetDevice(h->device);
-    h->d_frozen.release(); h->d_ctl.release(); h->d_crcm.release(); h->d_order.release(); h->d_info_rank.release();
+    h->d_frozen.release(); h->d_ctl.release(); h->d_ctl_r1.release(); h->d_crcm.release(); h->d_order.release(); h->d_info_rank.release();
     h->d_crc_mask.release(); h->d_tabs.release(); h->d_pre.release(); h->d_llr_scr.release(); h->d_c_scr.release(); h->d_hist_scr.release();
     h->d_in.release(); h->d_f32.release(); h->d_out.release(); h->d_bytes_a.release(); h->d_bytes_b.release();
     h->d_counter.release(); h->d_sel.release(); h->d_work.release();
diff --git a/polar_amd/csrc/polar_host.h b/polar_amd/csrc/polar_host.h
--- a/polar_amd/csrc/polar_host.h
+++ b/polar_amd/csrc/polar_host.h
@@ -201,6 +201,7 @@
     std::vector<uint32_t> crc_mask;
     std::vector<uint8_t> sched;
     std::vector<uint32_t> ctl;
+    std::vector<uint32_t> ctl_r1;
     int weak_leaves = 0;
     std::vector<uint32_t> sc_ops;
     std::vector<uint32_t> sc_lat_ops;
@@ -210,7 +211,7 @@
     size_t lds_per_block = 0;
     DevBuf<uint8_t> d_frozen, d_crcm;
     DevBuf<uint16_t> d_order, d_info_rank;
-    DevBuf<uint32_t> d_crc_mask, d_ctl, d_sc_ops, d_sc_lat_ops, d_var_scr;
+    DevBuf<uint32_t> d_crc_mask, d_ctl, d_ctl_r1, d_sc_ops, d_sc_lat_ops, d_var_scr;
     DevBuf<double> d_tab_scr;
     DevBuf<unsigned long long> d_head_rec;
     int last_head_phi = 0;
@@ -248,6 +249,7 @@
         bool sc_no_fold = false;
         bool no_tables = false;
         bool no_head = false;
+        bool no_r1 = false;
         long head_min_b = 0;
         bool no_fuse_front = false;
         bool no_rccl = false;
diff --git a/polar_amd/csrc/polar_kernels.hip b/polar_amd/csrc/polar_kernels.hip
--- a/polar_amd/csrc/polar_kernels.hip
+++ b/polar_amd/csrc/polar_kernels.hip
@@ -7,14 +7,27 @@
 #include "polar_edom.h"
 
 #ifdef POLAR_PROFILE
-#define PROF_DECL u64 prof_acc[24] = {0,0,0,0,0,0,0,0,0,0,0,0,0,0,0,0,0,0,0,0,0,0,0,0}; u64 prof_t = __builtin_readcyclecounter();
+#define PROF_DECL u64 prof_acc[32] = {0,0,0,0,0,0,0,0,0,0,0,0,0,0,0,0,0,0,0,0,0,0,0,0,0,0,0,0,0,0,0,0}; u64 prof_t = __builtin_readcyclecounter();
 #define PROF(i) { u64 t_ = __builtin_readcyclecounter(); prof_acc[i] += t_ - prof_t; prof_t = t_; }
-#define PROF_OUT if (lane == 0 && p.pm_out) { for (int i_ = 0; i_ < 24; ++i_) atomicAdd((u64 *)p.pm_out + i_, prof_acc[i_]); }
+#define PROF_OUT if (lane == 0 && p.pm_out) { for (int i_ = 0; i_ < 32; ++i_) atomicAdd((u64 *)p.pm_out + i_, prof_acc[i_]); }
 #define PROF_CNT(i, v) { prof_acc[i] += (u64)(v); }
 #define PROF_HEAD_DECL const int prof_head_phi = p.pm_out ? (int)((const u64 *)p.pm_out)[32] : 0; const u64 prof_head_t0 = prof_t; bool prof_head_open = prof_head_phi > 0;
 #define PROF_HEAD(phi_) if (prof_head_open && (phi_) >= prof_head_phi) { prof_acc[22] += __builtin_readcyclecounter() - prof_head_t0; prof_head_open = false; }
 #define PROF_HEAD_END prof_acc[23] += __builtin_readcyclecounter() - prof_head_t0;
+#define PROF_R1_DECL int prof_r1_left = 0; bool prof_r1_open = false; u64 prof_r1_t0 = 0; const bool prof_r1_off = p.pm_out && ((const u64 *)p.pm_out)[33] != 0; (void)prof_r1_off;
+#define PROF_R1_TOP { if (prof_r1_open) { prof_acc[24] += prof_t - prof_r1_t0; prof_r1_open = false; } \
+                      if (prof_r1_left > 0) { prof_r1_t0 = prof_t; prof_r1_open = true; --prof_r1_left; } }
+#define PROF_R1_LEAF(ctl_, fast_) { const int rb_ = (int)((ctl_) >> 9) & 3; \
+                      if (prof_r1_open) { if (!(fast_)) prof_acc[27] += 1; } \
+                      else if (rb_) { if (fast_) { prof_acc[25] += 1; prof_r1_left = (1 << rb_) - 1; } else prof_acc[26] += 1; } }
+#define PROF_R1_COMMIT prof_r1_left = 0;
+#define PROF_R1_END if (prof_r1_open) { prof_acc[24] += __builtin_readcyclecounter() - prof_r1_t0; prof_r1_open = false; }
 #else
+#define PROF_R1_DECL constexpr bool prof_r1_off = false; (void)prof_r1_off;
+#define PROF_R1_TOP
+#define PROF_R1_LEAF(ctl_, fast_)
+#define PROF_R1_COMMIT
+#define PROF_R1_END
 #define PROF_HEAD_DECL
 #define PROF_HEAD(phi_)
 #define PROF_HEAD_END
@@ -73,6 +86,23 @@
 #endif
 #ifndef POLAR_HEAD
 #define POLAR_HEAD 0
+#endif
+#if defined(POLAR_ED_TU) && (POLAR_ED_TU == 2 || POLAR_ED_TU == 6) && !defined(POLAR_MARGIN)
+#define POLAR_R1 1
+#else
+#define POLAR_R1 0
+#endif
+#if POLAR_R1 && defined(POLAR_TEST_HOOKS)
+__device__ unsigned long long polar_r1_counts_dev[2];
+#define R1_CNT_DECL unsigned r1_cnt_c = 0, r1_cnt_d = 0;
+#define R1_CNT_COMMIT ++r1_cnt_c;
+#define R1_CNT_DISCARD ++r1_cnt_d;
+#define R1_CNT_OUT if (lane == 0) { atomicAdd(&polar_r1_counts_dev[0], (unsigned long long)r1_cnt_c); atomicAdd(&polar_r1_counts_dev[1], (unsigned long long)r1_cnt_d); }
+#else
+#define R1_CNT_DECL
+#define R1_CNT_COMMIT
+#define R1_CNT_DISCARD
+#define R1_CNT_OUT
 #endif
 template <int GS, int LDS_LOG, int PIPE, bool ED, int NL = 0, int LAT = 0>
 __global__ __launch_bounds__(PIPE ? 64 : 256, PIPE ? 2 : OCC) void scl_decode_llr_kernel(POLAR_KPARAMS p) {
@@ -133,6 +163,7 @@
     double *tab_w = tbl ? p.tab_scr + (size_t)wave_id * G * (size_t)(3 * N) : nullptr;
     uint32_t *g_v = tbl ? p.var_scr + (size_t)wave_id * (size_t)(S2 / 8) * 64 : nullptr;
 
+    R1_CNT_DECL
     for (long g0 = (long)wave_id * G; g0 < Bv;) {
         const long cwi = g0 + grp;
         const bool valid = (cwi < Bv);
@@ -250,6 +281,7 @@
 
         PROF_DECL
         PROF_HEAD_DECL
+        PROF_R1_DECL
 #ifdef POLAR_MARGIN
         double mingap = __builtin_inf();
 #endif
@@ -273,6 +305,7 @@
 #endif
             PROF_HEAD(phi)
             PROF(0)
+            PROF_R1_TOP
             const uint32_t ctl = ctl_next;
             auto update_c = [&](int S, uint32_t X, int ph) {
                 LANE_CTX
@@ -356,10 +389,14 @@
                     ctl_next = (uint32_t)__builtin_amdgcn_readlane((int)ctlv, nphi & 63);
                 } else ctl_next = ctlp[nphi < N ? nphi : 0];
             }
+#if POLAR_R1
+            bool r1_done = false;
+#endif
             const int lam_stop = n - zb;
 #include "polar_scl_visits.inc"
 #include "polar_scl_leaf.inc"
         }
+        PROF_R1_END
         PROF_HEAD_END
         PROF_OUT
 
@@ -414,6 +451,7 @@
             g0 += (long)nwaves * G;
         }
     }
+    R1_CNT_OUT
 }
 
 template <bool ED>
@@ -772,7 +810,17 @@
     return hipGetLastError();
 }
 #elif POLAR_ED_TU == 6
+#ifdef POLAR_TEST_HOOKS
+static hipError_t r1_counts_zero(hipStream_t st) {
+    static const unsigned long long z[2] = {0, 0};
+    return hipMemcpyToSymbolAsync(HIP_SYMBOL(polar_r1_counts_dev), z, sizeof z, 0, hipMemcpyHostToDevice, st);
+}
+hipError_t polar_r1_counts_read_head(unsigned long long *out) { return hipMemcpyFromSymbol(out, HIP_SYMBOL(polar_r1_counts_dev), 2 * sizeof(unsigned long long)); }
+#endif
 hipError_t polar_launch_decode_head_import(const PolarHeadParams &p, int grid, hipStream_t st) {
+#ifdef POLAR_TEST_HOOKS
+    if (hipError_t e = r1_counts_zero(st)) return e;
+#endif
     if (!p.head_rec || p.L < 17 || p.L > 32 || p.head_phi <= 0 || p.head_phi >= p.N || grid < 4 || (grid & 3)) return hipErrorInvalidValue;
     const size_t lds = polar_decode_lds_bytes(3, 0);
 #ifndef POLAR_NO_FIXED_N
@@ -784,7 +832,16 @@
     return hipGetLastError();
 }
 #elif POLAR_ED_TU == 2
+#ifdef POLAR_TEST_HOOKS
+hipError_t polar_r1_counts_read_ed32(unsigned long long *out) { return hipMemcpyFromSymbol(out, HIP_SYMBOL(polar_r1_counts_dev), 2 * sizeof(unsigned long long)); }
+#endif
 hipError_t polar_launch_decode_llr_ed1_gs32(const PolarDecodeParams &p, int lds_log, int pipe, int grid, hipStream_t st) {
+#ifdef POLAR_TEST_HOOKS
+    {
+        static const unsigned long long z[2] = {0, 0};
+        if (hipError_t e = hipMemcpyToSymbolAsync(HIP_SYMBOL(polar_r1_counts_dev), z, sizeof z, 0, hipMemcpyHostToDevice, st)) return e;
+    }
+#endif
     return launch_gs<32, true>(p, lds_log, pipe, grid, st);
 }
 #elif POLAR_ED_TU == 1
diff --git a/polar_amd/csrc/polar_multi.cpp b/polar_amd/csrc/polar_multi.cpp
--- a/polar_amd/csrc/polar_multi.cpp
+++ b/polar_amd/csrc/polar_multi.cpp
@@ -40,7 +40,7 @@
     polar_code *c = new polar_code;
     c->n = h->n; c->N = h->N; c->K = h->K; c->crc = h->crc; c->eps = h->eps;
     c->frozen = h->frozen; c->order = h->order; c->bitrev = h->bitrev; c->crcm = h->crcm;
-    c->W = h->W; c->info_rank = h->info_rank; c->crc_mask = h->crc_mask; c->sched = h->sched; c->ctl = h->ctl;
+    c->W = h->W; c->info_rank = h->info_rank; c->crc_mask = h->crc_mask; c->sched = h->sched; c->ctl = h->ctl; c->ctl_r1 = h->ctl_r1;
     c->sc_ops = h->sc_ops; c->sc_lat_ops = h->sc_lat_ops; c->sc_fold = h->sc_fold; c->weak_leaves = h->weak_leaves;
     c->device = dev;
     c->waves_per_cu = h->waves_per_cu; c->lds_log = h->lds_log; c->pipe = h->pipe; c->prefix_on = h->prefix_on; c->mode = h->mode;
diff --git a/polar_amd/csrc/polar_scl_leaf.inc b/polar_amd/csrc/polar_scl_leaf.inc
--- a/polar_amd/csrc/polar_scl_leaf.inc
+++ b/polar_amd/csrc/polar_scl_leaf.inc
@@ -112,6 +112,7 @@
                     fast = wave_all((nact == 0) || (nact == L && gmax < bmin));
                 }
                 PROF_CNT(8, 1)
+                PROF_R1_LEAF(ctl, fast)
                 PROF(16)
                 if (fast) {
                     PROF_CNT(9, 1)
@@ -128,6 +129,68 @@
                         hword |= ubit << (t & 31);
                     }
                     PROF(17)
+#if POLAR_R1
+                    if constexpr (ED && !LAT && GS == 32) {
+                    if ((ctl & 0x600u) && !prof_r1_off) {
+                        PROF_CNT(29, 1)
+                        const uint32_t ctl_r1 = ctlp[phi + 4 < N ? phi + 4 : 0];
+                        const double *yq = lds_llr + (size_t)1 * 64 + lane, *xq = lds_llr + (size_t)3 * 64 + lane;
+                        double lf[3] = {0.0, 0.0, 0.0};
+                        if (active) {
+                            const double y0 = yq[0], y1 = yq[64], x0 = xq[0], x1 = xq[64], x2 = xq[128], x3 = xq[192];
+                            auto gss = [&](double a_, double b_) { return g_node_e(a_, b_, (unsigned)(__double2hiint(a_) ^ __double2hiint(b_)), tb); };
+                            const double z0 = gss(x0, x2), z1 = gss(x1, x3);
+                            lf[0] = gss(y0, y1);
+                            lf[1] = FN(z0, z1);
+                            lf[2] = gss(z0, z1);
+                        }
+                        double pmq = pm;
+                        u64 m_lt = ~0ull, m_one = __builtin_amdgcn_fcmp(fabs(leaf), 1.0, 1);
+                        uint32_t uq = 0;
+#pragma unroll
+                        for (int i_ = 0; i_ < 3; ++i_) {
+                            bool ng1; double al1, sn1, sp1;
+                            leaf_terms<ED>(lf[i_], active, actw, tb, ng1, al1, sn1, sp1);
+                            const double gq = pmq + sn1, bq = (pmq + al1) * 0.99999999999909050530;
+                            unsigned gh_ = active ? (unsigned)__double2hiint(gq) : 0u, bh_ = active ? (unsigned)__double2hiint(bq) : 0xFFFFFFFFu;
+                            group_max_min_u32<GS>(gh_, bh_);
+                            m_lt &= __builtin_amdgcn_uicmp(gh_, bh_, 36);
+                            m_one |= __builtin_amdgcn_fcmp(fabs(lf[i_]), 1.0, 1);
+                            pmq = gq;
+                            uq |= (ng1 ? 1u : 0u) << i_;
+                        }
+                        const u64 m_okq = __builtin_amdgcn_sicmp(nact, 0, 32) | (__builtin_amdgcn_sicmp(nact, L, 32) & m_lt);
+                        const bool pass = ((m_okq | ~group_result_rows<GS>()) == ~0ull) && (m_one & actw) == 0;
+                        if (pass) {
+                            PROF_CNT(30, 1)
+                            PROF_CNT(8, 3)
+                            PROF_CNT(9, 3)
+                            PROF_R1_COMMIT
+                            const uint32_t u1 = uq & 1u, u2 = (uq >> 1) & 1u, u3 = uq >> 2;
+                            if (active) {
+                                pm = pmq;
+                                hword |= (u1 << ((t + 1) & 31)) | (u2 << ((t + 2) & 31)) | (u3 << ((t + 3) & 31));
+                            }
+                            const uint32_t X = (ubit ^ u1 ^ u2 ^ u3) | ((u1 ^ u3) << 1) | ((u2 ^ u3) << 2) | (u3 << 3);
+                            const int nu = phi >> 2;
+                            if ((nu & 1) == 0) {
+                                if (active) clsmall = (clsmall & ~(0xFull << 4)) | ((u64)X << 4);
+                            } else {
+                                update_c(4, X, nu);
+                            }
+                            wave_mem_fence();
+                            t += 3;
+                            phi += 3;
+                            ctl_next = ctl_r1;
+                            r1_done = true;
+                            R1_CNT_COMMIT
+                        } else {
+                            R1_CNT_DISCARD
+                        }
+                        PROF(28)
+                    }
+                    }
+#endif
                 } else {
                 double pf0 = __builtin_nan(""), pf1 = __builtin_nan("");
                 if (active) {
@@ -364,6 +427,10 @@
             }
 
             PROF(frozen ? 5 : 6)
+#if POLAR_R1
+            if (r1_done) {
+            } else
+#endif
             if ((phi & 1) == 0) {
                 if (active) clsmall = (clsmall & ~2ull) | ((u64)ubit << 1);
             } else {
```

New measurement: 1.107 million (median of 6 runs). 1.04x the previous value.
